# snap-stanford/KGWAS

Hardware: AMD Instinct MI355X
Metric: edges aggregated/sec (full fast-mode KG minibatch training; epoch time in config) (higher is better)
Workload: dtype f32

## Files before the change

include/kgwas_hip.h:

```cpp
#ifndef KGWAS_HIP_H
#define KGWAS_HIP_H

#include <stdint.h>

#ifdef __cplusplus
extern "C" {
#endif

#define KGW_VERSION      125
#define KGW_MAX_TYPES    8
#define KGW_MAX_RELS     64
#define KGW_MAX_LAYERS   4
#define KGW_CHUNK        128
#define KGW_TILE         1024
#define KGW_C            128

#define KGW_F_RAW_WEIGHTS 1
#define KGW_F_DUV_PIECES  4
#define KGW_F_RELU_INPUT  2

#define KGW_OK           0
#define KGW_E_NULL      -1
#define KGW_E_RANGE     -2
#define KGW_E_UNSUPPORTED -3
// ... 186 lines not shown

int64_t kgw_scatter_relu_rows_workspace_floats(int64_t n_rows);
int kgw_scatter_relu_rows(const float* g, const int32_t* g2l, const float* h, int64_t n_rows, float* dz,
                          float* colsum, float* workspace, kgw_stream_t stream);

int kgw_edge_alpha(const KgwLayerArgs* args, float* alpha_out, kgw_stream_t stream);

enum { KGW_GRAD_DIRECT = 0, KGW_GRAD_TN = 1, KGW_GRAD_TN_COLSUM = 2, KGW_GRAD_MLP2_W = 3, KGW_GRAD_MLP2_B = 4, KGW_GRAD_G3T = 5 };
typedef struct KgwGradSrc {
    const float* ws;
    int32_t kind, nblk;
    int32_t M, N, MT, NT, gy, gz;
    int32_t K1, c_transposed;
    void* packed;
    int32_t flip, pad_;
} KgwGradSrc;

int64_t kgw_tn_gemm_workspace_floats(int64_t rows, int32_t M, int32_t N);
typedef struct KgwTnJob {
    const float* A; int64_t lda; const float* B; int64_t ldb;
    int64_t rows;
    float* C; int64_t ldc;
    float* colsum_a; int64_t colsum_ld;
    float* workspace; int64_t workspace_floats;
    const int32_t* rows_dev;
    int32_t M, N, c_transposed, colsum_repeat;
} KgwTnJob;
int kgw_tn_gemm_multi(int32_t n_jobs, const KgwTnJob* jobs, kgw_stream_t stream);
int kgw_tn_gemm(const float* A, int64_t lda, int32_t M, const float* B, int64_t ldb, int32_t N,
                int64_t rows, float* C, int64_t ldc, float* colsum_a, float* workspace,
                int64_t workspace_floats, kgw_stream_t stream);
int kgw_tn_gemm_ex(const float* A, int64_t lda, int32_t M, const float* B, int64_t ldb, int32_t N,
                   int64_t rows, float* C, int64_t ldc, int32_t c_transposed, float* colsum_a,
                   int32_t colsum_repeat, int64_t colsum_ld, float* workspace, int64_t workspace_floats,
                   const int32_t* rows_dev, kgw_stream_t stream);

int kgw_tn_gemm_partial(const float* A, int64_t lda, int32_t M, const float* B, int64_t ldb, int32_t N,
                        int64_t rows, float* C, int64_t ldc, int32_t c_transposed, float* colsum_a,
                        float* workspace, int64_t workspace_floats, const int32_t* rows_dev, KgwGradSrc* src,
                        kgw_stream_t stream);
int kgw_tn_gemm_multi_partial(int32_t n_jobs, const KgwTnJob* jobs, KgwGradSrc* src, kgw_stream_t stream);
int kgw_tn_split(int on);
int64_t kgw_tn_direct_rows(int64_t rows);

typedef struct KgwReadoutFold {
    const float* scratch; const double* terms; float* dw_lin; float* db_lin; double* loss;
    int32_t nb, n;
} KgwReadoutFold;

typedef struct KgwTnReducePlan { int32_t valid; int32_t blocks ; int32_t reserved[2]; int64_t opaque[96]; } KgwTnReducePlan;
int kgw_tn_reduce_launch(const KgwTnReducePlan* plan, kgw_stream_t stream);
int kgw_tn_gemm_partial_ride(const float* A, int64_t lda, int32_t M, const float* B, int64_t ldb, int32_t N, int64_t rows,
                             float* C, int64_t ldc, int32_t c_transposed, float* colsum_a, float* workspace,
                             int64_t workspace_floats, const int32_t* rows_dev, KgwGradSrc* src, const KgwTnReducePlan* ride_in,
                             kgw_stream_t stream);

int kgw_linear(const float* X, int64_t ldx, const float* W, int64_t ldw, const float* bias,
               const float* mask, int64_t ldm, float* Y, int64_t ldy, int64_t rows, int32_t K, int32_t N,
               int32_t relu, int32_t w_is_kn, const int32_t* rows_dev, kgw_stream_t stream);

int kgw_mlp2_fwd(const float* X, int64_t ldx, int32_t K1, const float* W1, int64_t ldw1, const float* b1, const float* W2,
                 int64_t ldw2, const float* b2, float* H1, int64_t ldh1, float* H2, int64_t ldh2, int64_t rows,
                 const int32_t* rows_dev, const int32_t* ids, float* Xg, int64_t ldxg, kgw_stream_t stream);

int kgw_mlp2w_fwd(int32_t n_jobs, const float* const* src, const int32_t* const* ids, const int64_t* n_rows, int64_t ldx,
                  const float* W1, int64_t ldw1, const float* b1, const float* W2, int64_t ldw2, const float* b2, float* Xg,
                  float* H1, float* H2, int64_t ldo, kgw_stream_t stream);

int64_t kgw_mlp2_bwd_first_workspace_floats(int64_t rows);
int kgw_mlp2_bwd_first(const float* dH2, int64_t ldd, const float* W2, int64_t ldw2, const float* H1, int64_t ldh1,
                       const float* X, int64_t ldx, int32_t K1, int64_t rows, const int32_t* rows_dev, float* dW1,
                       int64_t ldw1, float* db1, float* workspace, int64_t workspace_floats, const int32_t* in_ids, float* dZ,
                       int64_t ldz, kgw_stream_t stream);

int kgw_mlp2_bwd_first_partial(const float* dH2, int64_t ldd, const float* W2, int64_t ldw2, const float* H1, int64_t ldh1,
                               const float* X, int64_t ldx, int32_t K1, int64_t rows, const int32_t* rows_dev, float* dW1,
                               int64_t ldw1, float* db1, float* workspace, int64_t workspace_floats, const int32_t* in_ids,
                               float* dZ, int64_t ldz, KgwGradSrc* src, kgw_stream_t stream);
int kgw_mlp2_bwd_first_packed(const float* dH2, int64_t ldd, const float* W2, int64_t ldw2, const float* H1, int64_t ldh1,
                              const float* X, int64_t ldx, int32_t K1, int64_t rows, float* dW1, int64_t ldw1, float* db1,
                              float* workspace, int64_t workspace_floats, const int32_t* in_ids, float* dZ, int64_t ldz,
                              void* packed, int32_t flip, KgwGradSrc* src, kgw_stream_t stream);

int64_t kgw_gemm3_packed_bytes(int64_t K);
int64_t kgw_gemm3_workspace_floats(int64_t M, int64_t K);
int kgw_gemm3_pack(const float* S, int64_t lds, int64_t K, int64_t k_valid, int32_t s_is_kn, void* packed, kgw_stream_t stream);
int kgw_gemm3(const float* A, int64_t lda, int64_t M, int64_t K, const void* packed, float* workspace, int64_t workspace_floats,
              const float* bias, int32_t relu, float* out, int64_t ldo, int32_t transpose_out, const int32_t* row_map,
              float* out_rows, int64_t ld_rows, int64_t out_rows_n, const int32_t* out_rows_real, kgw_stream_t stream);

int64_t kgw_linear_splitk_workspace_floats(int64_t rows, int32_t K, int32_t N);
int kgw_linear_splitk(const float* X, int64_t ldx, const float* W, int64_t ldw, const float* bias, float* Y,
                      int64_t ldy, int64_t rows, int32_t K, int32_t N, int32_t relu, int32_t w_is_kn,
                      float* workspace, int64_t workspace_floats, const int32_t* rows_dev, kgw_stream_t stream);
int kgw_linear_splitk_ind(const float* X, int64_t ldx, const float* W, int64_t ldw, const float* bias, float* Y,
                          int64_t ldy, int64_t rows, int32_t K, int32_t relu, const float* seg_stat, const float* gamma,
                          float* workspace, int64_t workspace_floats, const int32_t* rows_dev, kgw_stream_t stream);
int kgw_ind_colsum(const float* seg_stat, const float* dY, int64_t ldy, int64_t rows, int32_t R, float* dgamma,
                   kgw_stream_t stream);
typedef struct KgwSplitKJob {
    const float* X; int64_t ldx;
    const float* W; int64_t ldw;
    const float* bias;
    float* Y; int64_t ldy;
    int64_t rows;
    const float* seg_stat;
    const float* gamma;
    float* dgamma;
    int32_t K, N, relu, w_is_kn;
} KgwSplitKJob;
int kgw_linear_splitk_multi(int32_t n_jobs, const KgwSplitKJob* jobs, kgw_stream_t stream);
int kgw_ind_colsum_multi(int32_t n_jobs, const KgwSplitKJob* jobs, kgw_stream_t stream);

int kgw_transform_bwd(int32_t n_tn, const KgwTnJob* tn_jobs, int32_t n_sk, const KgwSplitKJob* sk_jobs, int32_t n_cs,
                      const KgwSplitKJob* cs_jobs, kgw_stream_t stream);
int kgw_transform_bwd_ex(int32_t n_tn, const KgwTnJob* tn_jobs, int32_t n_sk, const KgwSplitKJob* sk_jobs, int32_t n_cs,
                         const KgwSplitKJob* cs_jobs, const KgwTnReducePlan* ride_in, KgwTnReducePlan* defer_out,
                         const KgwReadoutFold* fold_in , kgw_stream_t stream);

int kgw_adam(int32_t n_tensors, float* const* params, const float* const* grads, float* const* exp_avg,
             float* const* exp_avg_sq, const int64_t* numel, int32_t* step_dev, float lr, float beta1,
             float beta2, float eps, float weight_decay, kgw_stream_t stream);
int kgw_adam_notick(int32_t n_tensors, float* const* params, const float* const* grads, float* const* exp_avg,
                    float* const* exp_avg_sq, const int64_t* numel, int32_t* step_dev, float lr, float beta1,
                    float beta2, float eps, float weight_decay, kgw_stream_t stream);

int kgw_gemm3_partial(const float* A, int64_t lda, int64_t M, int64_t K, const void* packed, float* workspace,
                      int64_t workspace_floats, float* out, int64_t ldo, KgwGradSrc* src, kgw_stream_t stream);
int kgw_gemm3_flip(void);

enum { KGW_ADAM_FUSED_MAX = 40, KGW_ADAM_FUSED_SRC = 12, KGW_ADAM_FUSED_COUNTERS = 65 * 32 };
int kgw_adam_fused(int32_t n_tensors, float* const* params, float* const* grads, float* const* exp_avg,
                   float* const* exp_avg_sq, const int64_t* numel, const KgwGradSrc* src, int32_t* step_dev, float lr,
                   float beta1, float beta2, float eps, float weight_decay, const KgwBatchMeta* meta_dev, int32_t n_layers,
                   int32_t n_hops, int64_t* stats, int32_t* done_counters, kgw_stream_t stream);

int kgw_grad_finish(int32_t n_tensors, float* const* dst, float* const* grads, const int64_t* numel, const KgwGradSrc* src,
                    kgw_stream_t stream);

int kgw_relvec_fwd(int32_t n_rels_total, const int32_t* live_of_rel, const int32_t* bip_pos, const float* w_src_t,
                   const float* w_dst_t, const float* att_src, const float* att_dst, float* U_full, float* V,
                   int32_t v_by_rel, int32_t n_live, const float* bias, const int32_t* blk_of_live, int32_t n_blk,
                   float* bias_sum, float* zero_buf, int64_t zero_floats, kgw_stream_t stream);
int kgw_relvec_bwd(int32_t n_live, const int32_t* rel_ids, const int32_t* bip_pos, const float* w_src_t,
                   const float* w_dst_t, const float* att_src, const float* att_dst, const float* dU_full,
                   const float* dV, float* dw_src_t, float* dw_dst_t, float* datt_src, float* datt_dst,
                   int32_t v_by_rel, kgw_stream_t stream);
typedef struct KgwRelvecJob {
    int32_t n_rels_total, n_live, n_blk;
    int32_t duv_pieces;
    const int32_t* live_of_rel; const int32_t* rel_ids; const int32_t* bip_pos;
    const float* w_src_t; const float* w_dst_t; const float* att_src; const float* att_dst;
    float* U_full; float* V; const float* bias; const int32_t* blk_of_live; float* bias_sum;
    float* zero_buf; int64_t zero_floats;
    const float* dU_full; const float* dV; const float* dw_src_acc;
    float* dw_src_t; float* dw_dst_t; float* datt_src; float* datt_dst;
} KgwRelvecJob;
int kgw_relvec_fwd_multi(int32_t n_jobs, const KgwRelvecJob* jobs, kgw_stream_t stream);
int kgw_relvec_bwd_multi(int32_t n_jobs, const KgwRelvecJob* jobs, kgw_stream_t stream);
int kgw_relvec_bwd_acc(int32_t n_live, const int32_t* rel_ids, const int32_t* bip_pos, const float* w_src_t,
                       const float* w_dst_t, const float* att_src, const float* att_dst, const float* dU_full,
                       const float* dV, const float* dw_src_acc, float* dw_src_t, float* dw_dst_t, float* datt_src,
                       float* datt_dst, int32_t v_by_rel, kgw_stream_t stream);

typedef struct KgwFoldArgs {
    int32_t n, n_rels, n_mlp;
// ... 55 lines not shown
```

kgwas_amd/_lib.py:

```python
from __future__ import annotations

import ctypes as C
import os

KGW_MAX_TYPES = 8
KGW_MAX_RELS = 64
KGW_MAX_LAYERS = 4
KGW_CHUNK = 128
KGW_TILE = 1024
KGW_C = 128
PART_STRIDE = 132

_HERE = os.path.dirname(os.path.abspath(__file__))
LIB_PATH = os.environ.get('KGW_LIB_PATH') or os.path.join(_HERE, 'csrc', 'libkgwas_hip.so')


class KgwGraph(C.Structure):
    _fields_ = [
        ('n_types', C.c_int32), ('n_rels', C.c_int32), ('n_layers', C.c_int32), ('n_hops', C.c_int32),
        ('n_nodes', C.c_int32 * KGW_MAX_TYPES),
        ('node_base', C.c_int32 * (KGW_MAX_TYPES + 1)),
        ('R_dst', C.c_int32 * KGW_MAX_TYPES),
        ('R_src', C.c_int32 * KGW_MAX_TYPES),
        ('rel_src', C.c_int32 * KGW_MAX_RELS),
# ... 57 lines not shown
    ]


class KgwLayerArgs(C.Structure):
    _fields_ = [
        ('layer', C.c_int32), ('n_chunks', C.c_int32), ('n_multi_hops', C.c_int32), ('n_src_rows', C.c_int32),
        ('neg_slope', C.c_float), ('inv_temp', C.c_float), ('flags', C.c_int32), ('pad_', C.c_int32),
        ('graph_host', C.c_void_p), ('meta_host', C.c_void_p), ('meta_dev', C.c_void_p),
        ('chunks', C.c_void_p), ('multi', C.c_void_p), ('multi_cap', C.c_int64),
        ('col_local', C.c_void_p), ('H', C.c_void_p), ('a_dst', C.c_void_p), ('V', C.c_void_p), ('U', C.c_void_p),
        ('Z', C.c_void_p), ('stat', C.c_void_p), ('e_edge', C.c_void_p), ('part', C.c_void_p),
        ('dZ', C.c_void_p), ('adp', C.c_void_p), ('da_dst', C.c_void_p), ('part_da', C.c_void_p),
        ('t_ptr', C.c_void_p), ('t_edge', C.c_void_p), ('t_zrow', C.c_void_p),
        ('dH', C.c_void_p), ('ev_before', C.c_void_p), ('ev_after', C.c_void_p), ('da_src', C.c_void_p),
        ('logit_bias', C.c_void_p), ('partial_rels', C.c_uint64),
        ('t_rel', C.c_void_p), ('oct_flags', C.c_void_p), ('rel_sums', C.c_void_p),
        ('part_du', C.c_void_p), ('seg_chptr', C.c_void_p), ('duv_ws', C.c_void_p), ('dU', C.c_void_p), ('dV', C.c_void_p),
    ]


class KgwTnJob(C.Structure):
    _fields_ = [('A', C.c_void_p), ('lda', C.c_int64), ('B', C.c_void_p), ('ldb', C.c_int64), ('rows', C.c_int64),
                ('C', C.c_void_p), ('ldc', C.c_int64), ('colsum_a', C.c_void_p), ('colsum_ld', C.c_int64),
                ('workspace', C.c_void_p), ('workspace_floats', C.c_int64), ('rows_dev', C.c_void_p),
                ('M', C.c_int32), ('N', C.c_int32), ('c_transposed', C.c_int32), ('colsum_repeat', C.c_int32)]


class KgwGradSrc(C.Structure):
    _fields_ = [('ws', C.c_void_p), ('kind', C.c_int32), ('nblk', C.c_int32), ('M', C.c_int32), ('N', C.c_int32), ('MT', C.c_int32),
                ('NT', C.c_int32), ('gy', C.c_int32), ('gz', C.c_int32), ('K1', C.c_int32), ('c_transposed', C.c_int32),
                ('packed', C.c_void_p), ('flip', C.c_int32), ('pad_', C.c_int32)]


KGW_SEGCOPY_MAX = 40


class KgwSegCopy(C.Structure):
    _fields_ = [('n', C.c_int32), ('to_slot', C.c_int32), ('ptr', C.c_void_p * KGW_SEGCOPY_MAX), ('units', C.c_int64 * KGW_SEGCOPY_MAX),
                ('slot_off', C.c_int64 * KGW_SEGCOPY_MAX), ('slots', C.c_void_p), ('slot_stride', C.c_int64), ('slot_index', C.c_void_p)]


ADAM_FUSED_MAX, ADAM_FUSED_SRC, ADAM_FUSED_COUNTERS = 40, 12, 65 * 32


class KgwReadoutFold(C.Structure):
    _fields_ = [('scratch', C.c_void_p), ('terms', C.c_void_p), ('dw_lin', C.c_void_p), ('db_lin', C.c_void_p), ('loss', C.c_void_p),
                ('nb', C.c_int32), ('n', C.c_int32)]


class KgwTnReducePlan(C.Structure):
    _fields_ = [('valid', C.c_int32), ('blocks', C.c_int32), ('reserved', C.c_int32 * 2), ('opaque', C.c_int64 * 96)]


class KgwSplitKJob(C.Structure):
    _fields_ = [('X', C.c_void_p), ('ldx', C.c_int64), ('W', C.c_void_p), ('ldw', C.c_int64), ('bias', C.c_void_p),
                ('Y', C.c_void_p), ('ldy', C.c_int64), ('rows', C.c_int64), ('seg_stat', C.c_void_p), ('gamma', C.c_void_p),
                ('dgamma', C.c_void_p), ('K', C.c_int32), ('N', C.c_int32), ('relu', C.c_int32), ('w_is_kn', C.c_int32)]


class KgwRelvecJob(C.Structure):
    _fields_ = [('n_rels_total', C.c_int32), ('n_live', C.c_int32), ('n_blk', C.c_int32), ('duv_pieces', C.c_int32),
                ('live_of_rel', C.c_void_p), ('rel_ids', C.c_void_p), ('bip_pos', C.c_void_p),
                ('w_src_t', C.c_void_p), ('w_dst_t', C.c_void_p), ('att_src', C.c_void_p), ('att_dst', C.c_void_p),
                ('U_full', C.c_void_p), ('V', C.c_void_p), ('bias', C.c_void_p), ('blk_of_live', C.c_void_p), ('bias_sum', C.c_void_p),
                ('zero_buf', C.c_void_p), ('zero_floats', C.c_int64),
                ('dU_full', C.c_void_p), ('dV', C.c_void_p), ('dw_src_acc', C.c_void_p),
                ('dw_src_t', C.c_void_p), ('dw_dst_t', C.c_void_p), ('datt_src', C.c_void_p), ('datt_dst', C.c_void_p)]


class KgwFoldArgs(C.Structure):
    _fields_ = [('n', C.c_int32), ('n_rels', C.c_int32), ('n_mlp', C.c_int32), ('duv_pieces', C.c_int32),
                ('rel_ids_host', C.c_void_p), ('src_mlp_host', C.c_void_p), ('dst_mlp_host', C.c_void_p),
                ('w_src_t', C.c_void_p), ('fc_weight', C.c_void_p * 4), ('fc_bias', C.c_void_p * 4),
                ('U', C.c_void_p), ('V', C.c_void_p),
                ('Up', C.c_void_p), ('Vp', C.c_void_p), ('kappa', C.c_void_p), ('Wp', C.c_void_p), ('gamma', C.c_void_p),
                ('dUp', C.c_void_p), ('dVp', C.c_void_p), ('dkappa', C.c_void_p), ('dWp', C.c_void_p), ('dgamma', C.c_void_p),
                ('dU', C.c_void_p), ('dV', C.c_void_p), ('dws', C.c_void_p),
                ('d_fc_weight', C.c_void_p * 4), ('d_fc_bias', C.c_void_p * 4)]


EXPORTS = ['kgw_version', 'kgw_status_string', 'kgw_struct_sizes', 'kgw_sample_batch', 'kgw_sample_batch_parts', 'kgw_sample_batch_fanout', 'kgw_sampler_scan_ints', 'kgw_segments_copy',
           'kgw_softmax_pack', 'kgw_softmax_merge', 'kgw_scatter_rows', 'kgw_linear_splitk', 'kgw_linear_splitk_workspace_floats', 'kgw_linear_splitk_ind', 'kgw_ind_colsum', 'kgw_linear_splitk_multi', 'kgw_ind_colsum_multi', 'kgw_fold_fwd', 'kgw_fold_bwd', 'kgw_relation_sums',
           'kgw_gat_aggregate_fwd', 'kgw_gat_aggregate_bwd_dst', 'kgw_gat_aggregate_bwd_src',
           'kgw_gather_rows', 'kgw_gather_rows_multi', 'kgw_scatter_relu_rows', 'kgw_scatter_relu_rows_workspace_floats', 'kgw_edge_alpha', 'kgw_debug_reduce', 'kgw_debug_reduce8', 'kgw_tn_gemm', 'kgw_tn_gemm_ex', 'kgw_tn_gemm_multi', 'kgw_tn_gemm_workspace_floats', 'kgw_tn_gemm_partial', 'kgw_tn_gemm_multi_partial', 'kgw_tn_split', 'kgw_tn_direct_rows', 'kgw_param_tail', 'kgw_tn_reduce_launch', 'kgw_tn_gemm_partial_ride', 'kgw_transform_bwd_ex', 'kgw_mlp2_bwd_first_partial', 'kgw_mlp2_bwd_first_packed', 'kgw_adam_fused', 'kgw_gemm3_partial', 'kgw_gemm3_flip', 'kgw_transform_bwd', 'kgw_grad_finish',
           'kgw_linear', 'kgw_mlp2_fwd', 'kgw_mlp2w_fwd', 'kgw_mlp2_bwd_first', 'kgw_mlp2_bwd_first_workspace_floats', 'kgw_gemm3', 'kgw_gemm3_riders', 'kgw_gemm3_rider_blocks', 'kgw_gemm3_pack', 'kgw_gemm3_packed_bytes', 'kgw_gemm3_workspace_floats', 'kgw_adam', 'kgw_adam_notick', 'kgw_relvec_fwd', 'kgw_relvec_bwd', 'kgw_relvec_bwd_acc', 'kgw_relvec_fwd_multi', 'kgw_relvec_bwd_multi', 'kgw_wmse_fwd', 'kgw_wmse_bwd', 'kgw_readout_wmse_fwd', 'kgw_readout_wmse_bwd', 'kgw_readout_wmse_train', 'kgw_readout_wmse_train_parts', 'kgw_readout_train_fold', 'kgw_accumulate_stats', 'kgw_accumulate_stats_tick']

_lib = None


class KgwasHipError(RuntimeError):
    pass


def lib():
    global _lib
    if _lib is not None:
        return _lib
    if not os.path.exists(LIB_PATH):
        raise KgwasHipError(
            f'{LIB_PATH} not found: build it with `python -c "import __graft_entry__ as g; g.build()"` '
            '(hipcc --offload-arch=gfx950).  kgwas_amd has no CPU fallback.')
    L = C.CDLL(LIB_PATH)
    L.kgw_version.restype = C.c_int
    L.kgw_status_string.restype = C.c_char_p
    L.kgw_status_string.argtypes = [C.c_int]
    L.kgw_struct_sizes.argtypes = [C.POINTER(C.c_int64), C.c_int]
    sizes = (C.c_int64 * 7)()
    L.kgw_struct_sizes(sizes, 7)
    mine = [C.sizeof(KgwGraph), C.sizeof(KgwBatchMeta), C.sizeof(KgwChunk), C.sizeof(KgwBatchBuf),
            C.sizeof(KgwLayerArgs), C.sizeof(KgwTnJob), C.sizeof(KgwGradSrc)]
    if list(sizes) != mine:
        raise KgwasHipError(f'ABI struct size mismatch: library {list(sizes)} vs binding {mine}')
    L.kgw_sample_batch.argtypes = [C.POINTER(KgwGraph), C.POINTER(KgwBatchBuf), C.c_void_p, C.c_int32,
                                   C.c_int32, C.c_int32, C.c_void_p]
    L.kgw_sample_batch_parts.argtypes = [C.POINTER(KgwGraph), C.POINTER(KgwBatchBuf), C.c_void_p, C.c_int32,
                                         C.c_int32, C.c_int32, C.c_int32, C.c_int32, C.c_void_p]
    if hasattr(L, 'kgw_sample_batch_fanout'):
        L.kgw_sample_batch_fanout.argtypes = [C.POINTER(KgwGraph), C.POINTER(KgwBatchBuf), C.c_void_p, C.c_int32, C.c_int32,
                                              C.POINTER(C.c_int32), C.c_void_p, C.c_void_p]
    L.kgw_sampler_scan_ints.argtypes = [C.c_int64, C.c_int64, C.c_int64]
    L.kgw_sampler_scan_ints.restype = C.c_int64
    L.kgw_segments_copy.argtypes = [C.POINTER(KgwSegCopy), C.c_int32, C.c_void_p]
    L.kgw_softmax_pack.argtypes = [C.c_void_p, C.c_void_p, C.c_void_p, C.c_int64, C.c_void_p, C.c_void_p]
    L.kgw_softmax_merge.argtypes = [C.c_void_p, C.c_int32, C.c_void_p, C.c_int64, C.c_void_p, C.c_void_p, C.c_void_p]
    L.kgw_scatter_rows.argtypes = [C.c_void_p, C.c_void_p, C.c_int64, C.c_int32, C.c_void_p, C.c_void_p]
    for name in ('kgw_gat_aggregate_fwd', 'kgw_gat_aggregate_bwd_dst', 'kgw_gat_aggregate_bwd_src'):
        getattr(L, name).argtypes = [C.POINTER(KgwLayerArgs), C.c_void_p]
    L.kgw_gather_rows.argtypes = [C.c_void_p, C.c_void_p, C.c_int64, C.c_int32, C.c_void_p, C.c_void_p]
    L.kgw_tn_gemm_multi.argtypes = [C.c_int32, C.POINTER(KgwTnJob), C.c_void_p]
    L.kgw_scatter_relu_rows_workspace_floats.restype = C.c_int64
    L.kgw_scatter_relu_rows_workspace_floats.argtypes = [C.c_int64]
    L.kgw_scatter_relu_rows.argtypes = [C.c_void_p, C.c_void_p, C.c_void_p, C.c_int64, C.c_void_p, C.c_void_p, C.c_void_p, C.c_void_p]
    L.kgw_gather_rows_multi.argtypes = [C.c_int32, C.POINTER(C.c_void_p), C.POINTER(C.c_void_p), C.POINTER(C.c_int64), C.c_int32,
                                        C.POINTER(C.c_void_p), C.c_void_p]
    L.kgw_edge_alpha.argtypes = [C.POINTER(KgwLayerArgs), C.c_void_p, C.c_void_p]
    L.kgw_debug_reduce.argtypes = [C.c_void_p] * 5
    L.kgw_debug_reduce8.argtypes = [C.c_void_p] * 3
    L.kgw_tn_gemm_workspace_floats.restype = C.c_int64
    L.kgw_tn_gemm_workspace_floats.argtypes = [C.c_int64, C.c_int32, C.c_int32]
    L.kgw_linear.argtypes = [C.c_void_p, C.c_int64, C.c_void_p, C.c_int64, C.c_void_p, C.c_void_p, C.c_int64,
                             C.c_void_p, C.c_int64, C.c_int64, C.c_int32, C.c_int32, C.c_int32, C.c_int32, C.c_void_p,
                             C.c_void_p]
    L.kgw_mlp2_fwd.argtypes = [C.c_void_p, C.c_int64, C.c_int32, C.c_void_p, C.c_int64, C.c_void_p, C.c_void_p, C.c_int64, C.c_void_p,
                               C.c_void_p, C.c_int64, C.c_void_p, C.c_int64, C.c_int64, C.c_void_p, C.c_void_p, C.c_void_p, C.c_int64,
                               C.c_void_p]
    L.kgw_mlp2w_fwd.argtypes = [C.c_int32, C.c_void_p, C.c_void_p, C.c_void_p, C.c_int64, C.c_void_p, C.c_int64, C.c_void_p, C.c_void_p,
                                C.c_int64, C.c_void_p, C.c_void_p, C.c_void_p, C.c_void_p, C.c_int64, C.c_void_p]
    L.kgw_gemm3_packed_bytes.restype = C.c_int64
    L.kgw_gemm3_packed_bytes.argtypes = [C.c_int64]
    L.kgw_gemm3_workspace_floats.restype = C.c_int64
    L.kgw_gemm3_workspace_floats.argtypes = [C.c_int64, C.c_int64]
    L.kgw_gemm3_pack.argtypes = [C.c_void_p, C.c_int64, C.c_int64, C.c_int64, C.c_int32, C.c_void_p, C.c_void_p]
    L.kgw_gemm3.argtypes = [C.c_void_p, C.c_int64, C.c_int64, C.c_int64, C.c_void_p, C.c_void_p, C.c_int64, C.c_void_p, C.c_int32,
                            C.c_void_p, C.c_int64, C.c_int32, C.c_void_p, C.c_void_p, C.c_int64, C.c_int64, C.c_void_p, C.c_void_p]
    L.kgw_gemm3_riders.argtypes = L.kgw_gemm3.argtypes[:-1] + [C.c_int32, C.c_void_p, C.c_void_p, C.c_int32, C.c_void_p]
    L.kgw_gemm3_rider_blocks.argtypes = [C.c_int64, C.c_int64]
    L.kgw_mlp2_bwd_first_workspace_floats.restype = C.c_int64
    L.kgw_mlp2_bwd_first_workspace_floats.argtypes = [C.c_int64]
    L.kgw_mlp2_bwd_first.argtypes = [C.c_void_p, C.c_int64, C.c_void_p, C.c_int64, C.c_void_p, C.c_int64, C.c_void_p, C.c_int64, C.c_int32,
                                     C.c_int64, C.c_void_p, C.c_void_p, C.c_int64, C.c_void_p, C.c_void_p, C.c_int64, C.c_void_p, C.c_void_p,
                                     C.c_int64, C.c_void_p]
    L.kgw_linear_splitk_workspace_floats.restype = C.c_int64
    L.kgw_linear_splitk_workspace_floats.argtypes = [C.c_int64, C.c_int32, C.c_int32]
    L.kgw_linear_splitk.argtypes = [C.c_void_p, C.c_int64, C.c_void_p, C.c_int64, C.c_void_p, C.c_void_p, C.c_int64, C.c_int64,
                                    C.c_int32, C.c_int32, C.c_int32, C.c_int32, C.c_void_p, C.c_int64, C.c_void_p, C.c_void_p]
    L.kgw_linear_splitk_ind.argtypes = [C.c_void_p, C.c_int64, C.c_void_p, C.c_int64, C.c_void_p, C.c_void_p, C.c_int64, C.c_int64,
                                        C.c_int32, C.c_int32, C.c_void_p, C.c_void_p, C.c_void_p, C.c_int64, C.c_void_p, C.c_void_p]
    L.kgw_ind_colsum.argtypes = [C.c_void_p, C.c_void_p, C.c_int64, C.c_int64, C.c_int32, C.c_void_p, C.c_void_p]
    L.kgw_linear_splitk_multi.argtypes = [C.c_int32, C.POINTER(KgwSplitKJob), C.c_void_p]
    L.kgw_ind_colsum_multi.argtypes = [C.c_int32, C.POINTER(KgwSplitKJob), C.c_void_p]
    L.kgw_relation_sums.argtypes = [C.POINTER(KgwLayerArgs), C.c_void_p, C.c_void_p, C.c_void_p]
    L.kgw_fold_fwd.argtypes = [C.POINTER(KgwFoldArgs), C.c_void_p]
    L.kgw_fold_bwd.argtypes = [C.POINTER(KgwFoldArgs), C.c_void_p]
    L.kgw_adam.argtypes = [C.c_int32, C.c_void_p, C.c_void_p, C.c_void_p, C.c_void_p, C.c_void_p, C.c_void_p,
                           C.c_float, C.c_float, C.c_float, C.c_float, C.c_float, C.c_void_p]
    L.kgw_adam_notick.argtypes = L.kgw_adam.argtypes
    L.kgw_relvec_fwd.argtypes = [C.c_int32] + [C.c_void_p] * 8 + [C.c_int32, C.c_int32, C.c_void_p, C.c_void_p, C.c_int32,
                                 C.c_void_p, C.c_void_p, C.c_int64, C.c_void_p]
    L.kgw_relvec_fwd_multi.argtypes = [C.c_int32, C.POINTER(KgwRelvecJob), C.c_void_p]
    L.kgw_relvec_bwd_multi.argtypes = [C.c_int32, C.POINTER(KgwRelvecJob), C.c_void_p]
    L.kgw_relvec_bwd.argtypes = [C.c_int32] + [C.c_void_p] * 12 + [C.c_int32, C.c_void_p]
    L.kgw_relvec_bwd_acc.argtypes = [C.c_int32] + [C.c_void_p] * 13 + [C.c_int32, C.c_void_p]
    L.kgw_tn_gemm.argtypes = [C.c_void_p, C.c_int64, C.c_int32, C.c_void_p, C.c_int64, C.c_int32, C.c_int64,
                              C.c_void_p, C.c_int64, C.c_void_p, C.c_void_p, C.c_int64, C.c_void_p]
    L.kgw_tn_gemm_ex.argtypes = [C.c_void_p, C.c_int64, C.c_int32, C.c_void_p, C.c_int64, C.c_int32, C.c_int64,
                                 C.c_void_p, C.c_int64, C.c_int32, C.c_void_p, C.c_int32, C.c_int64, C.c_void_p,
                                 C.c_int64, C.c_void_p, C.c_void_p]
    L.kgw_tn_gemm_partial.argtypes = [C.c_void_p, C.c_int64, C.c_int32, C.c_void_p, C.c_int64, C.c_int32, C.c_int64,
                                      C.c_void_p, C.c_int64, C.c_int32, C.c_void_p, C.c_void_p, C.c_int64, C.c_void_p,
                                      C.POINTER(KgwGradSrc), C.c_void_p]
    L.kgw_tn_gemm_multi_partial.argtypes = [C.c_int32, C.POINTER(KgwTnJob), C.POINTER(KgwGradSrc), C.c_void_p]
    L.kgw_param_tail.argtypes = [C.c_int32, C.c_void_p, C.c_void_p, C.c_void_p, C.c_int32, C.c_void_p, C.c_int32, C.c_void_p]
    L.kgw_mlp2_bwd_first_partial.argtypes = L.kgw_mlp2_bwd_first.argtypes[:-1] + [C.POINTER(KgwGradSrc), C.c_void_p]
    L.kgw_mlp2_bwd_first_packed.argtypes = [C.c_void_p, C.c_int64, C.c_void_p, C.c_int64, C.c_void_p, C.c_int64, C.c_void_p, C.c_int64, C.c_int32,
                                            C.c_int64, C.c_void_p, C.c_int64, C.c_void_p, C.c_void_p, C.c_int64, C.c_void_p, C.c_void_p,
                                            C.c_int64, C.c_void_p, C.c_int32, C.c_void_p, C.c_void_p]
    L.kgw_adam_fused.argtypes = [C.c_int32, C.c_void_p, C.c_void_p, C.c_void_p, C.c_void_p, C.c_void_p, C.POINTER(KgwGradSrc), C.c_void_p,
                                 C.c_float, C.c_float, C.c_float, C.c_float, C.c_float, C.c_void_p, C.c_int32, C.c_int32, C.c_void_p,
                                 C.c_void_p, C.c_void_p]
    L.kgw_gemm3_partial.argtypes = [C.c_void_p, C.c_int64, C.c_int64, C.c_int64, C.c_void_p, C.c_void_p, C.c_int64, C.c_void_p, C.c_int64,
                                    C.POINTER(KgwGradSrc), C.c_void_p]
    L.kgw_gemm3_flip.restype = C.c_int
    L.kgw_grad_finish.argtypes = [C.c_int32, C.c_void_p, C.c_void_p, C.c_void_p, C.POINTER(KgwGradSrc), C.c_void_p]
    L.kgw_transform_bwd.argtypes = [C.c_int32, C.POINTER(KgwTnJob), C.c_int32, C.POINTER(KgwSplitKJob), C.c_int32, C.POINTER(KgwSplitKJob),
                                    C.c_void_p]
    L.kgw_transform_bwd_ex.argtypes = L.kgw_transform_bwd.argtypes[:-1] + [C.c_void_p, C.c_void_p, C.c_void_p, C.c_void_p]
    L.kgw_tn_reduce_launch.argtypes = [C.c_void_p, C.c_void_p]
    L.kgw_tn_direct_rows.restype = C.c_int64
    L.kgw_tn_direct_rows.argtypes = [C.c_int64]
    L.kgw_tn_gemm_partial_ride.argtypes = L.kgw_tn_gemm_partial.argtypes[:-1] + [C.c_void_p, C.c_void_p]
    L.kgw_wmse_fwd.argtypes = [C.c_void_p] * 4 + [C.c_int32, C.c_void_p, C.c_void_p]
    L.kgw_wmse_bwd.argtypes = [C.c_void_p] * 4 + [C.c_int32, C.c_void_p, C.c_void_p, C.c_void_p]
    L.kgw_readout_wmse_fwd.argtypes = [C.c_void_p] * 6 + [C.c_int32, C.c_int32] + [C.c_void_p] * 4
    L.kgw_readout_wmse_bwd.argtypes = [C.c_void_p] * 6 + [C.c_int32, C.c_int64, C.c_int32] + [C.c_void_p] * 6
    L.kgw_readout_wmse_train.argtypes = [C.c_void_p] * 6 + [C.c_int32, C.c_int64, C.c_int32] + [C.c_void_p] * 8
    L.kgw_readout_wmse_train_parts.argtypes = [C.c_void_p] * 6 + [C.c_int32, C.c_int64, C.c_int32] + [C.c_void_p] * 9
    L.kgw_readout_train_fold.argtypes = [C.c_void_p, C.c_void_p]
    L.kgw_accumulate_stats.argtypes = [C.c_void_p, C.c_int32, C.c_int32, C.c_void_p, C.c_void_p]
    L.kgw_accumulate_stats_tick.argtypes = [C.c_void_p, C.c_int32, C.c_int32, C.c_void_p, C.c_void_p, C.c_void_p]
    _lib = L
    return L


KGW_E_UNSUPPORTED = -3


def check(status: int, what: str):
    if status != 0:
        msg = lib().kgw_status_string(int(status))
        raise KgwasHipError(f'{what} failed: status {status} ({msg.decode() if msg else "?"})')


def stream_ptr():
    import torch
    return C.c_void_p(torch.cuda.current_stream().cuda_stream)
```

kgwas_amd/csrc/kgw_dense_linear.h:

```cpp
#pragma once

namespace {

constexpr int LBM = 128, LBN = 128, LBK = 32, LPAD = 33;

struct LinArgs {
    const float* X; int64_t ldx;
    const float* W; int64_t ldw;
    const float* bias;
    const float* mask;
    int64_t ldm;
    float* Y; int64_t ldy;
    int64_t rows; int K, N;
    int relu, w_kn;
    const int32_t* rows_dev;
};

__device__ __forceinline__ int64_t lin_rows_eff(const LinArgs& a) {
    if (!a.rows_dev) return a.rows;
    const int64_t r = *a.rows_dev;
    return r < 0 ? 0 : (r < a.rows ? r : a.rows);
}

__device__ __forceinline__ void lin_zero_padding(const LinArgs& a, int64_t rows_eff, int64_t tid, int64_t nthreads) {
// ... 38 lines not shown
            {
                const int row = idx >> 3, kq = (idx & 7) * 4;
                const int64_t r = r0 + row;
                const bool ok = (r < a.rows) && (k0 + kq < a.K);
                const float* p = a.X + (ok ? r : 0) * a.ldx + (ok ? k0 + kq : 0);
                const float4 v = *(const float4*)p;
                xr[j] = ok ? v : make_float4(0.f, 0.f, 0.f, 0.f);
            }
            if (!a.w_kn) {
                const int n = idx >> 3, kq = (idx & 7) * 4;
                const bool ok = (n0 + n < a.N) && (k0 + kq < a.K);
                const float* p = a.W + (int64_t)(ok ? n0 + n : 0) * a.ldw + (ok ? k0 + kq : 0);
                const float4 v = *(const float4*)p;
                wr[j] = ok ? v : make_float4(0.f, 0.f, 0.f, 0.f);
            } else {
                const int k = idx >> 5, nq = (idx & 31) * 4;
                const bool ok = (k0 + k < a.K) && (n0 + nq < a.N);
                const float* p = a.W + (int64_t)(ok ? k0 + k : 0) * a.ldw + (ok ? n0 + nq : 0);
                const float4 v = *(const float4*)p;
                wr[j] = ok ? v : make_float4(0.f, 0.f, 0.f, 0.f);
            }
        }
    };
    auto stage = [&]() {
#pragma unroll
        for (int j = 0; j < 4; ++j) {
            const int idx = tid + 256 * j;
            {
                const int row = idx >> 3, kq = (idx & 7) * 4;
                float* d = Xs + row * LPAD + kq;
                d[0] = xr[j].x; d[1] = xr[j].y; d[2] = xr[j].z; d[3] = xr[j].w;
            }
            if (!a.w_kn) {
                const int n = idx >> 3, kq = (idx & 7) * 4;
                float* d = Ws + n * LPAD + kq;
                d[0] = wr[j].x; d[1] = wr[j].y; d[2] = wr[j].z; d[3] = wr[j].w;
            } else {
                const int k = idx >> 5, nq = (idx & 31) * 4;
                Ws[(nq + 0) * LPAD + k] = wr[j].x; Ws[(nq + 1) * LPAD + k] = wr[j].y;
                Ws[(nq + 2) * LPAD + k] = wr[j].z; Ws[(nq + 3) * LPAD + k] = wr[j].w;
            }
        }
    };

    fetch(0);
    for (int k0 = 0; k0 < a.K; k0 += LBK) {
        __syncthreads();
        stage();
        __syncthreads();
        if (k0 + LBK < a.K) fetch(k0 + LBK);
        const float* xa = Xs + (wave * 32 + li) * LPAD + lk;
        const float* wb = Ws + li * LPAD + lk;
#pragma unroll
        for (int kp = 0; kp < LBK / 2; ++kp) {
            const float av = xa[2 * kp];
#pragma unroll
            for (int t = 0; t < 4; ++t)
                acc[t] = __builtin_amdgcn_mfma_f32_32x32x2f32(av, wb[t * 32 * LPAD + 2 * kp], acc[t], 0, 0, 0);
        }
    }
#pragma unroll
    for (int t = 0; t < 4; ++t) {
        const int col = n0 + t * 32 + li;
        if (col >= a.N) continue;
        const float bv = a.bias ? a.bias[col] : 0.f;
#pragma unroll
        for (int e = 0; e < 16; ++e) {
            const int64_t r = r0 + wave * 32 + (e & 3) + 8 * (e >> 2) + 4 * lk;
            if (r >= a.rows) continue;
            float v = acc[t][e] + bv;
            if (a.relu) v = fmaxf(v, 0.f);
            if (a.mask) v = (a.mask[r * a.ldm + col] > 0.f) ? v : 0.f;
            a.Y[r * a.ldy + col] = v;
        }
    }
}

}

namespace {

constexpr int WST = 132;

typedef float f32x4 __attribute__((ext_vector_type(4)));

template <int KC, bool WKN, int RT>
__global__ void __launch_bounds__(512) __attribute__((amdgpu_waves_per_eu(2, 2))) k_linear_wres(LinArgs a_) {
    extern __shared__ __attribute__((aligned(16))) float lds[];
    LinArgs a = a_;
    {
        const int64_t re = lin_rows_eff(a_);
        lin_zero_padding(a_, re, (int64_t)blockIdx.x * 512 + threadIdx.x, (int64_t)gridDim.x * 512);
        a.rows = re;
        if ((int64_t)blockIdx.x * RT >= re) return;
    }
    constexpr int XST = KC + 4;
    float* Wl = lds;
    float* Xs = lds + 128 * WST;
    constexpr int WRG = RT / 32, WCG = 8 / WRG, CT = 4 / WCG;
    const int tid = threadIdx.x, lane = tid & 63, wave = tid >> 6;
    const int li = lane & 31, lk = lane >> 5;
    const int nch = (a.K + KC - 1) / KC;
    const int64_t ntiles = (a.rows + RT - 1) / RT;
    constexpr int F4 = RT * KC / 4 / 512;
    f32x4 xr[F4];
#define KGW_FETCH(TILE, CH)                                                                            \
    _Pragma("unroll") for (int j = 0; j < F4; ++j) {                                                   \
        const int idx = tid + 512 * j;                                                                 \
        const int row = idx / (KC / 4), kq = (idx % (KC / 4)) * 4;                                     \
        int64_t r = (TILE) * RT + row;                                                                 \
        if (r >= a.rows) r = a.rows - 1;                      \
        int k = (CH) * KC + kq;                                                                        \
        if (k > a.K - 4) k = a.K - 4;                       \
        xr[j] = *(const f32x4*)(a.X + r * a.ldx + k);                                                   \
    }
    int64_t tile = blockIdx.x;
    if (tile < ntiles) { KGW_FETCH(tile, 0) }
    {
        f32x4 wv[8];
#pragma unroll
        for (int it = 0; it < 8; ++it) {
            const int idx = tid + 512 * it;
            wv[it] = f32x4{0.f, 0.f, 0.f, 0.f};
            if (!WKN) {
                const int n = idx >> 5, k4 = (idx & 31) * 4;
                if (n < a.N && k4 < a.K) wv[it] = *(const f32x4*)(a.W + (int64_t)n * a.ldw + k4);
            } else {
                const int k = idx >> 5, n4 = (idx & 31) * 4;
                if (k < a.K && n4 < a.N) wv[it] = *(const f32x4*)(a.W + (int64_t)k * a.ldw + n4);
            }
        }
#pragma unroll
        for (int it = 0; it < 8; ++it) {
            const int idx = tid + 512 * it;
            if (!WKN) {
                *(f32x4*)(Wl + (idx >> 5) * WST + (idx & 31) * 4) = wv[it];
            } else {
                const int k = idx >> 5, n4 = (idx & 31) * 4;
                Wl[(n4 + 0) * WST + k] = wv[it].x; Wl[(n4 + 1) * WST + k] = wv[it].y;
                Wl[(n4 + 2) * WST + k] = wv[it].z; Wl[(n4 + 3) * WST + k] = wv[it].w;
            }
        }
    }
    const int rg = wave % WRG, cg = wave / WRG;
    const float* wb = Wl + (cg * CT * 32 + li) * WST + lk * (KC / 2);
    float* slice = Xs + rg * 32 * XST;
    const float* xa = slice + li * XST + lk * (KC / 2);
    constexpr int Q = KC / 8;
    const float relu_lo = a.relu ? 0.f : -__builtin_inff();
    for (; tile < ntiles; tile += gridDim.x) {
        f32x16 acc[CT];
#pragma unroll
        for (int t = 0; t < CT; ++t)
#pragma unroll
            for (int e = 0; e < 16; ++e) acc[t][e] = 0.f;
        for (int ch = 0; ch < nch; ++ch) {
            __syncthreads();
#pragma unroll
            for (int j = 0; j < F4; ++j) {
                const int idx = tid + 512 * j;
                *(f32x4*)(Xs + (idx / (KC / 4)) * XST + (idx % (KC / 4)) * 4) = xr[j];
            }
            __syncthreads();
            {
                const bool same = ch + 1 < nch;
                const int64_t nt = same ? tile : tile + gridDim.x;
                const int nc = same ? ch + 1 : 0;
// ... 163 lines not shown
        }
        const int64_t row = (int64_t)tile * 32 + li;
        const bool live = row < a.rows;
        const float* mp = nullptr;
        if (MASK) mp = a.mask + (live ? row : a.rows - 1) * a.ldm + 4 * lk;
        unsigned mb[2] = {0xffffffffu, 0xffffffffu};
        f32x4 mv[2][4];
        f32x4 b3n = *(const f32x4*)w3;
#define KGW_MASK_FETCH(T)                                                                                 \
        _Pragma("unroll") for (int g = 0; g < 4; ++g) mv[(T) & 1][g] = *(const f32x4*)(mp + (T) * 32 + 8 * g);
#define KGW_MASK_BITS(T)                                                                                  \
        _Pragma("unroll") for (int g = 0; g < 4; ++g) {                                                  \
            const int b0 = ((T) & 1) * 16 + 4 * g;                                                        \
            if (!(mv[(T) & 1][g].x > 0.f)) mb[(T) >> 1] &= ~(1u << (b0 + 0));                             \
            if (!(mv[(T) & 1][g].y > 0.f)) mb[(T) >> 1] &= ~(1u << (b0 + 1));                             \
            if (!(mv[(T) & 1][g].z > 0.f)) mb[(T) >> 1] &= ~(1u << (b0 + 2));                             \
            if (!(mv[(T) & 1][g].w > 0.f)) mb[(T) >> 1] &= ~(1u << (b0 + 3));                             \
        }
#pragma unroll
        for (int q = 0; q < 16; ++q) {
            if (MASK) {
                if (q == 0) { KGW_MASK_FETCH(0) }
                if (q == 1) { KGW_MASK_FETCH(1) }
                if (q == 5) { KGW_MASK_BITS(0) }
                if (q == 6) { KGW_MASK_BITS(1) KGW_MASK_FETCH(2) }
                if (q == 7) { KGW_MASK_FETCH(3) }
                if (q == 11) { KGW_MASK_BITS(2) }
                if (q == 12) { KGW_MASK_BITS(3) }
            }
            const f32x4 b3 = b3n;
            if (q + 1 < 16) b3n = *(const f32x4*)(w3 + 4 * (q + 1));
#define KGW_WREG_STEP(C)                                                                                  \
            _Pragma("unroll") for (int t = 0; t < 3; ++t)                                                \
                acc[t] = __builtin_amdgcn_mfma_f32_32x32x2f32(bw[t][q].C, xa[q].C, acc[t], 0, 0, 0);      \
            acc[3] = __builtin_amdgcn_mfma_f32_32x32x2f32(b3.C, xa[q].C, acc[3], 0, 0, 0);
            KGW_WREG_STEP(x) KGW_WREG_STEP(y) KGW_WREG_STEP(z) KGW_WREG_STEP(w)
#undef KGW_WREG_STEP
            if (q == 7) {
                __builtin_amdgcn_sched_barrier(0);
#pragma unroll
                for (int qq = 0; qq < 8; ++qq) xa[qq] = *(const f32x4*)(xn + 4 * qq);
                __builtin_amdgcn_sched_barrier(0);
            }
        }
#undef KGW_MASK_FETCH
#undef KGW_MASK_BITS
        if (live) {
            float* yp = a.Y + row * a.ldy + 4 * lk;
#pragma unroll
            for (int t = 0; t < 4; ++t) {
#pragma unroll
                for (int g = 0; g < 4; ++g) {
                    const f32x4 b4 = *(const f32x4*)(bl + t * 32 + 8 * g);
                    f32x4 v;
                    v.x = acc[t][4 * g + 0] + b4.x; v.y = acc[t][4 * g + 1] + b4.y;
                    v.z = acc[t][4 * g + 2] + b4.z; v.w = acc[t][4 * g + 3] + b4.w;
                    v.x = fmaxf(v.x, lo); v.y = fmaxf(v.y, lo); v.z = fmaxf(v.z, lo); v.w = fmaxf(v.w, lo);
                    if (MASK) {
                        const unsigned m4 = mb[t >> 1] >> (((t & 1) << 4) + 4 * g);
                        v.x = (m4 & 1u) ? v.x : 0.f; v.y = (m4 & 2u) ? v.y : 0.f;
                        v.z = (m4 & 4u) ? v.z : 0.f; v.w = (m4 & 8u) ? v.w : 0.f;
                    }
                    *(f32x4*)(yp + t * 32 + 8 * g) = v;
                }
            }
        }
        __builtin_amdgcn_sched_barrier(0);
#pragma unroll
        for (int qq = 8; qq < 16; ++qq) xa[qq] = *(const f32x4*)(xn + 4 * qq);
        __builtin_amdgcn_sched_barrier(0);
    }
}

struct Mlp2Args {
    const float* X; int64_t ldx;
    const float* W1; int64_t ldw1; const float* b1;
    const float* W2; int64_t ldw2; const float* b2;
    float* H1; int64_t ldh1;
    float* H2; int64_t ldh2;
    int64_t rows; int K1;
    const int32_t* rows_dev;
    const int32_t* ids;
    float* Xg; int64_t ldxg;
};

__global__ void __launch_bounds__(256) __attribute__((amdgpu_waves_per_eu(1, 1))) k_mlp2_fwd(Mlp2Args a) {
    extern __shared__ __attribute__((aligned(16))) float lds[];
    float* Wl = lds;
    float* W1l = lds + 128 * WST + 128;
    const int tid = threadIdx.x, lane = tid & 63, wave = tid >> 6;
    const int li = lane & 31, lk = lane >> 5;
    int64_t rows = a.rows;
    if (a.rows_dev) { const int64_t r = *a.rows_dev; rows = r < 0 ? 0 : (r < a.rows ? r : a.rows); }
    {
        const int64_t npad = a.rows - rows;
        for (int64_t q = (int64_t)blockIdx.x * 256 + tid; q < npad * 32; q += (int64_t)gridDim.x * 256) {
            const int64_t r = rows + q / 32; const int c4 = (int)(q % 32) * 4;
            *(float4*)(a.H2 + r * a.ldh2 + c4) = make_float4(0.f, 0.f, 0.f, 0.f);
            if (a.H1) *(float4*)(a.H1 + r * a.ldh1 + c4) = make_float4(0.f, 0.f, 0.f, 0.f);
        }
        if ((int64_t)blockIdx.x * 4 * 32 >= rows) return;
    }
    const int ntiles = (int)((rows + 31) / 32);
    const int nw = (int)gridDim.x * 4;
    int tile = (int)blockIdx.x * 4 + wave;
    const int K1 = a.K1;
    auto fetch_x = [&](int t, f32x4 (&x)[3]) {
        int64_t r = (int64_t)(t < ntiles ? t : ntiles - 1) * 32 + li;
        if (r >= rows) r = rows - 1;
        const float* xp = a.X + (a.ids ? (int64_t)a.ids[r] : r) * a.ldx;
#pragma unroll
        for (int c = 0; c < 3; ++c) {
            const int k4 = 12 * lk + 4 * c;
            if (k4 + 4 <= K1) x[c] = *(const f32x4*)(xp + k4);
            else x[c] = f32x4{k4 == K1 ? 1.f : 0.f, 0.f, 0.f, 0.f};
        }
    };
    f32x4 xn[3];
    fetch_x(tile, xn);
    {
        f32x4 wv[16];
#pragma unroll
        for (int it = 0; it < 16; ++it) {
            const int idx = tid + 256 * it;
            wv[it] = *(const f32x4*)(a.W2 + (int64_t)(idx >> 5) * a.ldw2 + (idx & 31) * 4);
        }
#pragma unroll
        for (int it = 0; it < 16; ++it) {
            const int idx = tid + 256 * it;
            *(f32x4*)(Wl + (idx >> 5) * WST + (idx & 31) * 4) = wv[it];
        }
        for (int idx = tid; idx < 128 * 24; idx += 256) {
            const int n = idx / 24, k = idx % 24;
            W1l[idx] = k < K1 ? a.W1[(int64_t)n * a.ldw1 + k] : (k == K1 ? (a.b1 ? a.b1[n] : 0.f) : 0.f);
        }
    }
    if (tid < 128) Wl[128 * WST + tid] = a.b2 ? a.b2[tid] : 0.f;
    __syncthreads();
    f32x4 bw[3][16];
#pragma unroll
    for (int t = 0; t < 3; ++t)
#pragma unroll
        for (int q = 0; q < 16; ++q) bw[t][q] = *(const f32x4*)(Wl + (t * 32 + li) * WST + 32 * (q >> 2) + 8 * (q & 3) + 4 * lk);
    const float* w3 = Wl + (96 + li) * WST + 4 * lk;
    f32x4 w1[4][3];
#pragma unroll
    for (int t = 0; t < 4; ++t)
#pragma unroll
        for (int c = 0; c < 3; ++c) w1[t][c] = *(const f32x4*)(W1l + (t * 32 + li) * 24 + 12 * lk + 4 * c);
    const float* bl = Wl + 128 * WST + 4 * lk;
    for (; tile < ntiles; tile += nw) {
        f32x4 x[3] = {xn[0], xn[1], xn[2]};
        fetch_x(tile + nw, xn);
        f32x16 acc[4];
#pragma unroll
        for (int t = 0; t < 4; ++t)
#pragma unroll
            for (int e = 0; e < 16; ++e) acc[t][e] = 0.f;
#pragma unroll
        for (int c = 0; c < 3; ++c) {
#define KGW_MLP_STEP(C)                                                                                   \
            _Pragma("unroll") for (int t = 0; t < 4; ++t)                                                \
                acc[t] = __builtin_amdgcn_mfma_f32_32x32x2f32(w1[t][c].C, x[c].C, acc[t], 0, 0, 0);
            KGW_MLP_STEP(x) KGW_MLP_STEP(y) KGW_MLP_STEP(z) KGW_MLP_STEP(w)
#undef KGW_MLP_STEP
        }
        const int64_t row = (int64_t)tile * 32 + li;
        const bool live = row < rows;
        if (a.Xg && live) {
#pragma unroll
            for (int c = 0; c < 3; ++c)
                if (12 * lk + 4 * c + 4 <= K1) *(f32x4*)(a.Xg + row * a.ldxg + 12 * lk + 4 * c) = x[c];
        }
        f32x4 xa[16];
#pragma unroll
        for (int t = 0; t < 4; ++t)
#pragma unroll
            for (int g = 0; g < 4; ++g) {
                f32x4 v;
                v.x = fmaxf(acc[t][4 * g + 0], 0.f); v.y = fmaxf(acc[t][4 * g + 1], 0.f);
                v.z = fmaxf(acc[t][4 * g + 2], 0.f); v.w = fmaxf(acc[t][4 * g + 3], 0.f);
                xa[4 * t + g] = v;
            }
        if (a.H1 && live) {
            float* hp = a.H1 + row * a.ldh1 + 4 * lk;
#pragma unroll
            for (int q = 0; q < 16; ++q) *(f32x4*)(hp + 32 * (q >> 2) + 8 * (q & 3)) = xa[q];
        }
#pragma unroll
        for (int t = 0; t < 4; ++t)
#pragma unroll
            for (int e = 0; e < 16; ++e) acc[t][e] = 0.f;
        f32x4 b3n = *(const f32x4*)w3;
#pragma unroll
        for (int q = 0; q < 16; ++q) {
            const f32x4 b3 = b3n;
            if (q + 1 < 16) b3n = *(const f32x4*)(w3 + 32 * ((q + 1) >> 2) + 8 * ((q + 1) & 3));
#define KGW_MLP_STEP(C)                                                                                   \
            _Pragma("unroll") for (int t = 0; t < 3; ++t)                                                \
                acc[t] = __builtin_amdgcn_mfma_f32_32x32x2f32(bw[t][q].C, xa[q].C, acc[t], 0, 0, 0);      \
            acc[3] = __builtin_amdgcn_mfma_f32_32x32x2f32(b3.C, xa[q].C, acc[3], 0, 0, 0);
            KGW_MLP_STEP(x) KGW_MLP_STEP(y) KGW_MLP_STEP(z) KGW_MLP_STEP(w)
#undef KGW_MLP_STEP
        }
        if (live) {
            float* yp = a.H2 + row * a.ldh2 + 4 * lk;
#pragma unroll
            for (int t = 0; t < 4; ++t) {
#pragma unroll
                for (int g = 0; g < 4; ++g) {
                    const f32x4 b4 = *(const f32x4*)(bl + t * 32 + 8 * g);
                    f32x4 v;
                    v.x = fmaxf(acc[t][4 * g + 0] + b4.x, 0.f); v.y = fmaxf(acc[t][4 * g + 1] + b4.y, 0.f);
                    v.z = fmaxf(acc[t][4 * g + 2] + b4.z, 0.f); v.w = fmaxf(acc[t][4 * g + 3] + b4.w, 0.f);
                    *(f32x4*)(yp + t * 32 + 8 * g) = v;
                }
            }
        }
    }
}

static constexpr int M3_W2_U4 = 8 * 3 * 4 * 64;

__global__ void __launch_bounds__(512, 1) k_mlp2_fwd3(Mlp2Args a) {
    extern __shared__ __attribute__((aligned(16))) float lds[];
    uint4* W2p = (uint4*)lds;
    float* W1l = lds + M3_W2_U4 * 4;
    float* bl = W1l + 128 * 24;
    const int tid = threadIdx.x, lane = tid & 63, wave = tid >> 6;
    const int li = lane & 31, lk = lane >> 5;
    int64_t rows = a.rows;
    if (a.rows_dev) { const int64_t r = *a.rows_dev; rows = r < 0 ? 0 : (r < a.rows ? r : a.rows); }
    {
        const int64_t npad = a.rows - rows;
        for (int64_t q = (int64_t)blockIdx.x * 512 + tid; q < npad * 32; q += (int64_t)gridDim.x * 512) {
            const int64_t r = rows + q / 32; const int c4 = (int)(q % 32) * 4;
            *(float4*)(a.H2 + r * a.ldh2 + c4) = make_float4(0.f, 0.f, 0.f, 0.f);
            if (a.H1) *(float4*)(a.H1 + r * a.ldh1 + c4) = make_float4(0.f, 0.f, 0.f, 0.f);
        }
        if ((int64_t)blockIdx.x * 8 * 32 >= rows) return;
    }
    const int ntiles = (int)((rows + 31) / 32);
    const int nw = (int)gridDim.x * 8;
    int tile = (int)blockIdx.x * 8 + wave;
    const int K1 = a.K1;
    auto fetch_x = [&](int t, f32x4 (&x)[3]) {
        int64_t r = (int64_t)(t < ntiles ? t : ntiles - 1) * 32 + li;
        if (r >= rows) r = rows - 1;
        const float* xp = a.X + (a.ids ? (int64_t)a.ids[r] : r) * a.ldx;
#pragma unroll
        for (int c = 0; c < 3; ++c) {
            const int k4 = 12 * lk + 4 * c;
            if (k4 + 4 <= K1) x[c] = *(const f32x4*)(xp + k4);
            else x[c] = f32x4{k4 == K1 ? 1.f : 0.f, 0.f, 0.f, 0.f};
        }
    };
    f32x4 xn[3];
    fetch_x(tile, xn);
    for (int idx = tid; idx < 8 * 4 * 64; idx += 512) {
        const int ln = idx & 63, ot = (idx >> 6) & 3, s_ = idx >> 8;
        const float* wp = a.W2 + (int64_t)(32 * ot + (ln & 31)) * a.ldw2 + 32 * (s_ >> 1) + 16 * (s_ & 1) + 4 * (ln >> 5);
        const f32x4 u = *(const f32x4*)wp, v = *(const f32x4*)(wp + 8);
        const float x[8] = {u.x, u.y, u.z, u.w, v.x, v.y, v.z, v.w};
        uint4 p1, p2, p3;
        kgw_split3x8(x, p1, p2, p3);
        uint4* o = W2p + ((s_ * 3) * 4 + ot) * 64 + ln;
        o[0] = p1; o[4 * 64] = p2; o[8 * 64] = p3;
    }
    for (int idx = tid; idx < 128 * 24; idx += 512) {
        const int n = idx / 24, k = idx % 24;
        W1l[idx] = k < K1 ? a.W1[(int64_t)n * a.ldw1 + k] : (k == K1 ? (a.b1 ? a.b1[n] : 0.f) : 0.f);
    }
    if (tid < 128) bl[tid] = a.b2 ? a.b2[tid] : 0.f;
    __syncthreads();
    const float* w1p = W1l + li * 24 + 12 * lk;
    const uint4* w2p = W2p + lane;
    const float* blp = bl + 4 * lk;
    for (; tile < ntiles; tile += nw) {
        f32x4 x[3] = {xn[0], xn[1], xn[2]};
        fetch_x(tile + nw, xn);
        f32x16 acc[4];
#pragma unroll
        for (int t = 0; t < 4; ++t)
#pragma unroll
            for (int e = 0; e < 16; ++e) acc[t][e] = 0.f;
#pragma unroll
        for (int c = 0; c < 3; ++c) {
            f32x4 w[4];
#pragma unroll
            for (int t = 0; t < 4; ++t) w[t] = *(const f32x4*)(w1p + t * 32 * 24 + 4 * c);
#define KGW_MLP_STEP(C)                                                                                   \
            _Pragma("unroll") for (int t = 0; t < 4; ++t)                                                \
                acc[t] = __builtin_amdgcn_mfma_f32_32x32x2f32(w[t].C, x[c].C, acc[t], 0, 0, 0);
            KGW_MLP_STEP(x) KGW_MLP_STEP(y) KGW_MLP_STEP(z) KGW_MLP_STEP(w)
#undef KGW_MLP_STEP
        }
        const int64_t row = (int64_t)tile * 32 + li;
        const bool live = row < rows;
        if (a.Xg && live) {
#pragma unroll
            for (int c = 0; c < 3; ++c)
                if (12 * lk + 4 * c + 4 <= K1) *(f32x4*)(a.Xg + row * a.ldxg + 12 * lk + 4 * c) = x[c];
        }
        f32x4 xa[16];
#pragma unroll
        for (int t = 0; t < 4; ++t)
#pragma unroll
            for (int g = 0; g < 4; ++g) {
                f32x4 v;
                v.x = fmaxf(acc[t][4 * g + 0], 0.f); v.y = fmaxf(acc[t][4 * g + 1], 0.f);
                v.z = fmaxf(acc[t][4 * g + 2], 0.f); v.w = fmaxf(acc[t][4 * g + 3], 0.f);
                xa[4 * t + g] = v;
            }
        if (a.H1 && live) {
            float* hp = a.H1 + row * a.ldh1 + 4 * lk;
#pragma unroll
            for (int q = 0; q < 16; ++q) *(f32x4*)(hp + 32 * (q >> 2) + 8 * (q & 3)) = xa[q];
        }
#pragma unroll
        for (int t = 0; t < 4; ++t)
#pragma unroll
            for (int e = 0; e < 16; ++e) acc[t][e] = 0.f;
#pragma unroll
        for (int s_ = 0; s_ < 8; ++s_) {
            const f32x4 u = xa[2 * s_], v = xa[2 * s_ + 1];
            const float h[8] = {u.x, u.y, u.z, u.w, v.x, v.y, v.z, v.w};
            uint4 p1, p2, p3;
            kgw_split3x8(h, p1, p2, p3);
            const kgw_bf8 hb[3] = {__builtin_bit_cast(kgw_bf8, p1), __builtin_bit_cast(kgw_bf8, p2), __builtin_bit_cast(kgw_bf8, p3)};
            kgw_bf8 wa[3][4];
#pragma unroll
            for (int p = 0; p < 3; ++p)
#pragma unroll
                for (int ot = 0; ot < 4; ++ot) wa[p][ot] = __builtin_bit_cast(kgw_bf8, w2p[((s_ * 3 + p) * 4 + ot) * 64]);
            constexpr int TW[6] = {0, 2, 1, 0, 1, 0}, TH[6] = {2, 0, 1, 1, 0, 0};
#pragma unroll
            for (int t6 = 0; t6 < 6; ++t6)
#pragma unroll
                for (int ot = 0; ot < 4; ++ot)
                    acc[ot] = __builtin_amdgcn_mfma_f32_32x32x16_bf16(wa[TW[t6]][ot], hb[TH[t6]], acc[ot], 0, 0, 0);
        }
        if (live) {
            float* yp = a.H2 + row * a.ldh2 + 4 * lk;
#pragma unroll
            for (int t = 0; t < 4; ++t) {
#pragma unroll
                for (int g = 0; g < 4; ++g) {
                    const f32x4 b4 = *(const f32x4*)(blp + t * 32 + 8 * g);
                    f32x4 v;
                    v.x = fmaxf(acc[t][4 * g + 0] + b4.x, 0.f); v.y = fmaxf(acc[t][4 * g + 1] + b4.y, 0.f);
                    v.z = fmaxf(acc[t][4 * g + 2] + b4.z, 0.f); v.w = fmaxf(acc[t][4 * g + 3] + b4.w, 0.f);
                    *(f32x4*)(yp + t * 32 + 8 * g) = v;
                }
            }
        }
    }
}

struct Mlp2wArgs {
    const float* src[4]; const int32_t* ids[4]; int64_t row0[5];
    int n_jobs; int64_t ldx;
    const float* W1; int64_t ldw1; const float* b1;
    const float* W2; int64_t ldw2; const float* b2;
    float* Xg; float* H1; float* H2; int64_t ldo;
    int64_t rows;
};

__global__ void __launch_bounds__(256) __attribute__((amdgpu_waves_per_eu(1, 1))) k_mlp2w_fwd(Mlp2wArgs a) {
    extern __shared__ __attribute__((aligned(16))) float lds[];
    float* W1l = lds;
    float* W2l = lds + 128 * WST;
    float* bl = lds + 2 * 128 * WST;
    const int tid = threadIdx.x, lane = tid & 63, wave = tid >> 6;
    const int li = lane & 31, lk = lane >> 5;
    const int64_t tile = (int64_t)blockIdx.x * 2 + (wave >> 1);
    const int half = wave & 1, t0 = half * 2;
    const int64_t row = tile * 32 + li;
    const bool live = row < a.rows;
    const int64_t rc = live ? row : a.rows - 1;
    f32x4 xa[16];
    {
        int j = 0;
        while (j + 1 < a.n_jobs && rc >= a.row0[j + 1]) ++j;
        const float* xp = a.src[j] + (int64_t)a.ids[j][rc - a.row0[j]] * a.ldx + lk * 64;
#pragma unroll
        for (int q = 0; q < 16; ++q) xa[q] = *(const f32x4*)(xp + 4 * q);
    }
    {
        f32x4 wv[16];
#pragma unroll
        for (int it = 0; it < 16; ++it) {
            const int idx = tid + 256 * it;
            wv[it] = *(const f32x4*)(a.W1 + (int64_t)(idx >> 5) * a.ldw1 + (idx & 31) * 4);
        }
#pragma unroll
        for (int it = 0; it < 16; ++it) {
            const int idx = tid + 256 * it;
            *(f32x4*)(W1l + (idx >> 5) * WST + (idx & 31) * 4) = wv[it];
        }
#pragma unroll
        for (int it = 0; it < 16; ++it) {
// ... 38 lines not shown
#undef KGW_MLPW_STEP
    }
    f32x4 xh[8];
#pragma unroll
    for (int t = 0; t < 2; ++t)
#pragma unroll
        for (int g = 0; g < 4; ++g) {
            const f32x4 b4 = *(const f32x4*)(bl + (t0 + t) * 32 + 8 * g + 4 * lk);
            f32x4 v;
            v.x = fmaxf(acc[t][4 * g + 0] + b4.x, 0.f); v.y = fmaxf(acc[t][4 * g + 1] + b4.y, 0.f);
            v.z = fmaxf(acc[t][4 * g + 2] + b4.z, 0.f); v.w = fmaxf(acc[t][4 * g + 3] + b4.w, 0.f);
            xh[4 * t + g] = v;
        }
    if (live) {
        float* hp = a.H1 + row * a.ldo + 4 * lk;
#pragma unroll
        for (int q = 0; q < 8; ++q) *(f32x4*)(hp + 32 * (t0 + (q >> 2)) + 8 * (q & 3)) = xh[q];
    }
    __syncthreads();
    {
        f32x4* ex = (f32x4*)W1l;
#pragma unroll
        for (int q = 0; q < 8; ++q) ex[(wave * 8 + q) * 64 + lane] = xh[q];
    }
    __syncthreads();
    {
        const f32x4* ex = (const f32x4*)W1l + ((wave ^ 1) * 8) * 64 + lane;
#pragma unroll
        for (int q = 0; q < 8; ++q) {
            const f32x4 pq = ex[q * 64];
            xa[q] = half ? pq : xh[q];
            xa[8 + q] = half ? xh[q] : pq;
        }
    }
    f32x16 ac2[2];
#pragma unroll
    for (int t = 0; t < 2; ++t)
#pragma unroll
        for (int e = 0; e < 16; ++e) ac2[t][e] = 0.f;
    const float* w2p = W2l + (t0 * 32 + li) * WST + 4 * lk;
    f32x4 vn[2];
#pragma unroll
    for (int t = 0; t < 2; ++t) vn[t] = *(const f32x4*)(w2p + t * 32 * WST);
#pragma unroll
    for (int q = 0; q < 16; ++q) {
        f32x4 w[2];
#pragma unroll
        for (int t = 0; t < 2; ++t) w[t] = vn[t];
        if (q + 1 < 16) {
#pragma unroll
            for (int t = 0; t < 2; ++t) vn[t] = *(const f32x4*)(w2p + t * 32 * WST + 32 * ((q + 1) >> 2) + 8 * ((q + 1) & 3));
        }
#define KGW_MLPW_STEP(C)                                                                                  \
        _Pragma("unroll") for (int t = 0; t < 2; ++t)                                                    \
            ac2[t] = __builtin_amdgcn_mfma_f32_32x32x2f32(w[t].C, xa[q].C, ac2[t], 0, 0, 0);
        KGW_MLPW_STEP(x) KGW_MLPW_STEP(y) KGW_MLPW_STEP(z) KGW_MLPW_STEP(w)
#undef KGW_MLPW_STEP
    }
    if (live) {
        float* yp = a.H2 + row * a.ldo + 4 * lk;
#pragma unroll
        for (int t = 0; t < 2; ++t)
#pragma unroll
            for (int g = 0; g < 4; ++g) {
                const f32x4 b4 = *(const f32x4*)(bl + 128 + (t0 + t) * 32 + 8 * g + 4 * lk);
                f32x4 v;
                v.x = fmaxf(ac2[t][4 * g + 0] + b4.x, 0.f); v.y = fmaxf(ac2[t][4 * g + 1] + b4.y, 0.f);
                v.z = fmaxf(ac2[t][4 * g + 2] + b4.z, 0.f); v.w = fmaxf(ac2[t][4 * g + 3] + b4.w, 0.f);
                *(f32x4*)(yp + (t0 + t) * 32 + 8 * g) = v;
            }
    }
}

struct Mlp2BwdArgs {
    const float* dH2; int64_t ldd;
    const float* W2; int64_t ldw;
    const float* H1; int64_t ldm;
    const float* X; int64_t ldx;
    float* part;
    int64_t rows; int K1;
    const int32_t* rows_dev;
    const int32_t* in_ids;
    float* dZ; int64_t ldz;
    uint4* packed; int flip;
};

constexpr int TST = 132;

__global__ void __launch_bounds__(256) __attribute__((amdgpu_waves_per_eu(1, 1))) k_mlp2_bwd_first(Mlp2BwdArgs a) {
    extern __shared__ __attribute__((aligned(16))) float lds[];
    float* Wl = lds;
    float* Tl = lds + 128 * WST;
    const int tid = threadIdx.x, lane = tid & 63, wave = tid >> 6;
    const int li = lane & 31, lk = lane >> 5;
    int64_t rows = a.rows;
    if (a.rows_dev) { const int64_t r = *a.rows_dev; rows = r < 0 ? 0 : (r < a.rows ? r : a.rows); }
    const int ntiles = (int)((rows + 31) / 32);
    const int nw = (int)gridDim.x * 4;
    float* Tw = Tl + wave * 32 * TST;
    {
        f32x4 wv[16];
#pragma unroll
        for (int it = 0; it < 16; ++it) {
            const int idx = tid + 256 * it;
            wv[it] = *(const f32x4*)(a.W2 + (int64_t)(idx & 127) * a.ldw + (idx >> 7) * 4);
        }
#pragma unroll
        for (int it = 0; it < 16; ++it) {
            const int idx = tid + 256 * it;
            const int k = idx & 127, n4 = (idx >> 7) * 4;
            Wl[(n4 + 0) * WST + k] = wv[it].x; Wl[(n4 + 1) * WST + k] = wv[it].y;
            Wl[(n4 + 2) * WST + k] = wv[it].z; Wl[(n4 + 3) * WST + k] = wv[it].w;
        }
    }
    __syncthreads();
    f32x4 bw[2][16];
#pragma unroll
    for (int t = 0; t < 2; ++t)
#pragma unroll
        for (int q = 0; q < 16; ++q) bw[t][q] = *(const f32x4*)(Wl + (t * 32 + li) * WST + lk * 64 + 4 * q);
    const float* w2 = Wl + (64 + li) * WST + lk * 64;
    const float* w3 = Wl + (96 + li) * WST + lk * 64;
    f32x16 accw[4];
#pragma unroll
    for (int t = 0; t < 4; ++t)
#pragma unroll
        for (int e = 0; e < 16; ++e) accw[t][e] = 0.f;
    const int K1 = a.K1;
    int tile = (int)blockIdx.x * 4 + wave;
    f32x4 xa[16];
    int src_cur;
    {
        int64_t r = (int64_t)(tile < ntiles ? tile : ntiles - 1) * 32 + li;
        if (r >= rows) r = rows - 1;
        src_cur = a.in_ids ? a.in_ids[r] : 0;
        const float* xp = a.dH2 + (a.in_ids ? (int64_t)(src_cur < 0 ? 0 : src_cur) : r) * a.ldd + lk * 64;
#pragma unroll
        for (int q = 0; q < 16; ++q) xa[q] = *(const f32x4*)(xp + 4 * q);
    }
    for (; tile < ntiles; tile += nw) {
        const int64_t r0 = (int64_t)tile * 32;
        const int64_t row = r0 + li;
        const bool live = row < rows && src_cur >= 0;
        const int64_t rc = row < rows ? row : rows - 1;
        const float* xn;
        {
            int nt = tile + nw;
            if (nt >= ntiles) nt = ntiles - 1;
            int64_t r = (int64_t)nt * 32 + li;
            if (r >= rows) r = rows - 1;
            src_cur = a.in_ids ? a.in_ids[r] : 0;
            xn = a.dH2 + (a.in_ids ? (int64_t)(src_cur < 0 ? 0 : src_cur) : r) * a.ldd + lk * 64;
        }
        float xs[16];
#pragma unroll
        for (int s2 = 0; s2 < 16; ++s2) {
            const int64_t rr = r0 + 2 * s2 + lk;
            float v = 0.f;
            if (rr < rows) v = li < K1 ? a.X[rr * a.ldx + li] : (li == K1 ? 1.f : 0.f);
            xs[s2] = v;
        }
        const float* mp = a.H1 + rc * a.ldm + 4 * lk;
        unsigned mb[2] = {0u, 0u};
        f32x4 mv[4];
#define KGW_MLPB_MFETCH(T)                                                                                \
        _Pragma("unroll") for (int g = 0; g < 4; ++g) mv[g] = *(const f32x4*)(mp + (T) * 32 + 8 * g);
#define KGW_MLPB_MBITS(T)                                                                                 \
        _Pragma("unroll") for (int g = 0; g < 4; ++g) {                                                  \
            const int b0 = ((T) & 1) * 16 + 4 * g;                                                        \
            mb[(T) >> 1] |= (mv[g].x > 0.f ? 1u : 0u) << (b0 + 0);                                        \
            mb[(T) >> 1] |= (mv[g].y > 0.f ? 1u : 0u) << (b0 + 1);                                        \
            mb[(T) >> 1] |= (mv[g].z > 0.f ? 1u : 0u) << (b0 + 2);                                        \
            mb[(T) >> 1] |= (mv[g].w > 0.f ? 1u : 0u) << (b0 + 3);                                        \
        }
        f32x16 acc[4];
#pragma unroll
        for (int t = 0; t < 4; ++t)
#pragma unroll
            for (int e = 0; e < 16; ++e) acc[t][e] = 0.f;
        f32x4 b2n = *(const f32x4*)w2, b3n = *(const f32x4*)w3;
#pragma unroll
        for (int q = 0; q < 16; ++q) {
            if (q == 0) { KGW_MLPB_MFETCH(0) }
            if (q == 3) { KGW_MLPB_MBITS(0) KGW_MLPB_MFETCH(1) }
            if (q == 6) { KGW_MLPB_MBITS(1) KGW_MLPB_MFETCH(2) }
            if (q == 10) { KGW_MLPB_MBITS(2) KGW_MLPB_MFETCH(3) }
            if (q == 14) { KGW_MLPB_MBITS(3) }
            const f32x4 b2 = b2n, b3 = b3n;
            if (q + 1 < 16) { b2n = *(const f32x4*)(w2 + 4 * (q + 1)); b3n = *(const f32x4*)(w3 + 4 * (q + 1)); }
#define KGW_MLPB_STEP(C)                                                                                  \
            acc[0] = __builtin_amdgcn_mfma_f32_32x32x2f32(bw[0][q].C, xa[q].C, acc[0], 0, 0, 0);          \
            acc[1] = __builtin_amdgcn_mfma_f32_32x32x2f32(bw[1][q].C, xa[q].C, acc[1], 0, 0, 0);          \
            acc[2] = __builtin_amdgcn_mfma_f32_32x32x2f32(b2.C, xa[q].C, acc[2], 0, 0, 0);                \
            acc[3] = __builtin_amdgcn_mfma_f32_32x32x2f32(b3.C, xa[q].C, acc[3], 0, 0, 0);
            KGW_MLPB_STEP(x) KGW_MLPB_STEP(y) KGW_MLPB_STEP(z) KGW_MLPB_STEP(w)
#undef KGW_MLPB_STEP
            if (q == 7) {
                __builtin_amdgcn_sched_barrier(0);
#pragma unroll
                for (int qq = 0; qq < 8; ++qq) xa[qq] = *(const f32x4*)(xn + 4 * qq);
                __builtin_amdgcn_sched_barrier(0);
            }
        }
#undef KGW_MLPB_MFETCH
#undef KGW_MLPB_MBITS
        if (!live) { mb[0] = 0u; mb[1] = 0u; }
        __builtin_amdgcn_sched_barrier(0);
#pragma unroll
        for (int qq = 8; qq < 16; ++qq) xa[qq] = *(const f32x4*)(xn + 4 * qq);
        __builtin_amdgcn_sched_barrier(0);
#pragma unroll
        for (int t = 0; t < 4; ++t)
#pragma unroll
            for (int g = 0; g < 4; ++g) {
                const unsigned m4 = mb[t >> 1] >> (((t & 1) << 4) + 4 * g);
                f32x4 v;
                v.x = (m4 & 1u) ? acc[t][4 * g + 0] : 0.f; v.y = (m4 & 2u) ? acc[t][4 * g + 1] : 0.f;
                v.z = (m4 & 4u) ? acc[t][4 * g + 2] : 0.f; v.w = (m4 & 8u) ? acc[t][4 * g + 3] : 0.f;
                *(f32x4*)(Tw + li * TST + t * 32 + 8 * g + 4 * lk) = v;
                if (a.dZ && row < rows) *(f32x4*)(a.dZ + row * a.ldz + t * 32 + 8 * g + 4 * lk) = v;
            }
        __asm__ volatile("s_waitcnt lgkmcnt(0)" ::: "memory");
#pragma unroll
        for (int s2 = 0; s2 < 16; ++s2) {
            const float* tp = Tw + (2 * s2 + lk) * TST + li;
#pragma unroll
            for (int t = 0; t < 4; ++t)
                accw[t] = __builtin_amdgcn_mfma_f32_32x32x2f32(xs[s2], tp[t * 32], accw[t], 0, 0, 0);
        }
        __asm__ volatile("s_waitcnt lgkmcnt(0)" ::: "memory");
    }
    __syncthreads();
    float* R = Tl;
#pragma unroll
    for (int t = 0; t < 4; ++t)
#pragma unroll
        for (int e = 0; e < 16; ++e) R[wave * 4096 + (t * 16 + e) * 64 + lane] = accw[t][e];
    __syncthreads();
    for (int f = tid; f < 4096; f += 256)
        a.part[(int64_t)blockIdx.x * 4096 + f] = (R[f] + R[4096 + f]) + (R[2 * 4096 + f] + R[3 * 4096 + f]);
}

constexpr int TS2 = 68;

template <bool PACK>
__global__ void __launch_bounds__(256) __attribute__((amdgpu_waves_per_eu(1, 1))) k_mlp2_bwd_first3(Mlp2BwdArgs a) {
    extern __shared__ __attribute__((aligned(16))) float lds[];
    uint4* W2p = (uint4*)lds;
    float* Tl = lds + M3_W2_U4 * 4;
    const int tid = threadIdx.x, lane = tid & 63, wave = tid >> 6;
    const int li = lane & 31, lk = lane >> 5;
    const unsigned sgn = (li & 1) ? 0x80000000u : 0u;
    int64_t rows = a.rows;
    if (a.rows_dev) { const int64_t r = *a.rows_dev; rows = r < 0 ? 0 : (r < a.rows ? r : a.rows); }
    const int ntiles = (int)((rows + 31) / 32);
    const int nw = (int)gridDim.x * 4;
    float* Tw = Tl + wave * 32 * TS2;
    for (int idx = tid; idx < 8 * 4 * 64; idx += 256) {
        const int ln = idx & 63, jt = (idx >> 6) & 3, s_ = idx >> 8;
        const float* wp = a.W2 + (int64_t)(64 * (ln >> 5) + 8 * s_) * a.ldw + 32 * jt + (ln & 31);
        float x[8];
#pragma unroll
        for (int i = 0; i < 8; ++i) x[i] = wp[(int64_t)i * a.ldw];
        uint4 p1, p2, p3;
        kgw_split3x8(x, p1, p2, p3);
        uint4* o = W2p + ((s_ * 3) * 4 + jt) * 64 + ln;
        o[0] = p1; o[4 * 64] = p2; o[8 * 64] = p3;
    }
    __syncthreads();
    const uint4* w2p = W2p + lane;
    f32x16 accw[4];
#pragma unroll
    for (int t = 0; t < 4; ++t)
#pragma unroll
        for (int e = 0; e < 16; ++e) accw[t][e] = 0.f;
    const int K1 = a.K1;
    int tile = (int)blockIdx.x * 4 + wave;
    f32x4 xa[16];
    int src_cur;
    {
        int64_t r = (int64_t)(tile < ntiles ? tile : ntiles - 1) * 32 + li;
        if (r >= rows) r = rows - 1;
        src_cur = a.in_ids ? a.in_ids[r] : 0;
        const float* xp = a.dH2 + (a.in_ids ? (int64_t)(src_cur < 0 ? 0 : src_cur) : r) * a.ldd + lk * 64;
#pragma unroll
        for (int q = 0; q < 16; ++q) xa[q] = *(const f32x4*)(xp + 4 * q);
    }
#define KGW_MLPB_BITS(MV, MB)                                                                            \
    _Pragma("unroll") for (int t_ = 0; t_ < 4; ++t_) _Pragma("unroll") for (int g = 0; g < 4; ++g) {    \
        const int b0 = (t_ & 1) * 16 + 4 * g;                                                            \
        MB[t_ >> 1] |= (MV[t_][g].x > 0.f ? 1u : 0u) << (b0 + 0);                                        \
        MB[t_ >> 1] |= (MV[t_][g].y > 0.f ? 1u : 0u) << (b0 + 1);                                        \
        MB[t_ >> 1] |= (MV[t_][g].z > 0.f ? 1u : 0u) << (b0 + 2);                                        \
        MB[t_ >> 1] |= (MV[t_][g].w > 0.f ? 1u : 0u) << (b0 + 3);                                        \
    }
    unsigned mb[2] = {0u, 0u};
    {
        int64_t r = (int64_t)(tile < ntiles ? tile : ntiles - 1) * 32 + li;
        if (r >= rows) r = rows - 1;
        const float* mp = a.H1 + r * a.ldm + 4 * lk;
        f32x4 mv[4][4];
#pragma unroll
        for (int t_ = 0; t_ < 4; ++t_)
#pragma unroll
            for (int g = 0; g < 4; ++g) mv[t_][g] = *(const f32x4*)(mp + t_ * 32 + 8 * g);
        KGW_MLPB_BITS(mv, mb)
    }
    for (; tile < ntiles; tile += nw) {
        const int64_t r0 = (int64_t)tile * 32;
        const int64_t row = r0 + li;
        const bool live = row < rows && src_cur >= 0;
        const int64_t rc = row < rows ? row : rows - 1;
        const float* xn;
        {
            int nt = tile + nw;
            if (nt >= ntiles) nt = ntiles - 1;
            int64_t r = (int64_t)nt * 32 + li;
            if (r >= rows) r = rows - 1;
            src_cur = a.in_ids ? a.in_ids[r] : 0;
            xn = a.dH2 + (a.in_ids ? (int64_t)(src_cur < 0 ? 0 : src_cur) : r) * a.ldd + lk * 64;
        }
        float xs[16];
#pragma unroll
        for (int s2 = 0; s2 < 16; ++s2) {
            const int64_t rr = r0 + 2 * s2 + lk;
            float v = 0.f;
            if (rr < rows) v = li < K1 ? a.X[rr * a.ldx + li] : (li == K1 ? 1.f : 0.f);
            xs[s2] = v;
        }
        f32x4 mvn[4][4];
        {
            int nt = tile + nw;
            if (nt >= ntiles) nt = ntiles - 1;
            int64_t r = (int64_t)nt * 32 + li;
            if (r >= rows) r = rows - 1;
            const float* mpn = a.H1 + r * a.ldm + 4 * lk;
#pragma unroll
            for (int t_ = 0; t_ < 4; ++t_)
#pragma unroll
                for (int g = 0; g < 4; ++g) mvn[t_][g] = *(const f32x4*)(mpn + t_ * 32 + 8 * g);
        }
        f32x16 acc[4];
#pragma unroll
        for (int t = 0; t < 4; ++t)
#pragma unroll
            for (int e = 0; e < 16; ++e) acc[t][e] = 0.f;
#pragma unroll
        for (int s_ = 0; s_ < 8; ++s_) {
            const f32x4 u = xa[2 * s_], v = xa[2 * s_ + 1];
            const float h[8] = {kgw_fxor(u.x, sgn), kgw_fxor(u.y, sgn), kgw_fxor(u.z, sgn), kgw_fxor(u.w, sgn),
                                kgw_fxor(v.x, sgn), kgw_fxor(v.y, sgn), kgw_fxor(v.z, sgn), kgw_fxor(v.w, sgn)};
            uint4 p1, p2, p3;
            kgw_split3x8(h, p1, p2, p3);
            const kgw_bf8 hb[3] = {__builtin_bit_cast(kgw_bf8, p1), __builtin_bit_cast(kgw_bf8, p2), __builtin_bit_cast(kgw_bf8, p3)};
            kgw_bf8 wa[3][4];
#pragma unroll
            for (int p = 0; p < 3; ++p)
#pragma unroll
                for (int jt = 0; jt < 4; ++jt) wa[p][jt] = __builtin_bit_cast(kgw_bf8, w2p[((s_ * 3 + p) * 4 + jt) * 64]);
            constexpr int TW[6] = {0, 2, 1, 0, 1, 0}, TH[6] = {2, 0, 1, 1, 0, 0};
#pragma unroll
            for (int t6 = 0; t6 < 6; ++t6)
#pragma unroll
                for (int jt = 0; jt < 4; ++jt)
                    acc[jt] = __builtin_amdgcn_mfma_f32_32x32x16_bf16(wa[TW[t6]][jt], hb[TH[t6]], acc[jt], 0, 0, 0);
            if (s_ == 3) {
                __builtin_amdgcn_sched_barrier(0);
#pragma unroll
                for (int qq = 0; qq < 8; ++qq) xa[qq] = *(const f32x4*)(xn + 4 * qq);
                __builtin_amdgcn_sched_barrier(0);
            }
        }
        if (!live) { mb[0] = 0u; mb[1] = 0u; }
        __builtin_amdgcn_sched_barrier(0);
#pragma unroll
        for (int qq = 8; qq < 16; ++qq) xa[qq] = *(const f32x4*)(xn + 4 * qq);
        __builtin_amdgcn_sched_barrier(0);
#pragma unroll
        for (int hh = 0; hh < 2; ++hh) {
#pragma unroll
            for (int t = 2 * hh; t < 2 * hh + 2; ++t)
#pragma unroll
                for (int g = 0; g < 4; ++g) {
                    const unsigned m4 = mb[t >> 1] >> (((t & 1) << 4) + 4 * g);
                    f32x4 v;
                    v.x = (m4 & 1u) ? kgw_fxor(acc[t][4 * g + 0], sgn) : 0.f; v.y = (m4 & 2u) ? kgw_fxor(acc[t][4 * g + 1], sgn) : 0.f;
                    v.z = (m4 & 4u) ? kgw_fxor(acc[t][4 * g + 2], sgn) : 0.f; v.w = (m4 & 8u) ? kgw_fxor(acc[t][4 * g + 3], sgn) : 0.f;
                    *(f32x4*)(Tw + li * TS2 + (t - 2 * hh) * 32 + 8 * g + 4 * lk) = v;
                    if (a.dZ && row < rows) *(f32x4*)(a.dZ + row * a.ldz + t * 32 + 8 * g + 4 * lk) = v;
                }
            __asm__ volatile("s_waitcnt lgkmcnt(0)" ::: "memory");
            if (PACK) {
                const bool neg = a.flip && ((tile / a.flip) & 1);
#pragma unroll
                for (int it = 0; it < 4; ++it) {
                    const int ntl = it & 1, j = it >> 1;
                    const float* tp = Tw + (16 * j + 8 * lk) * TS2 + 32 * ntl + li;
                    float x[8];
#pragma unroll
                    for (int i = 0; i < 8; ++i) x[i] = neg ? -tp[i * TS2] : tp[i * TS2];
                    uint4 p1, p2, p3;
                    kgw_split3x8(x, p1, p2, p3);
                    uint4* o = a.packed + (((int64_t)tile * 2 + j) * 3 * 4 + (2 * hh + ntl)) * 64 + lane;
                    o[0] = p1; o[4 * 64] = p2; o[8 * 64] = p3;
                }
            }
#pragma unroll
            for (int s2 = 0; s2 < 16; ++s2) {
                const float* tp = Tw + (2 * s2 + lk) * TS2 + li;
#pragma unroll
                for (int t = 0; t < 2; ++t)
                    accw[2 * hh + t] = __builtin_amdgcn_mfma_f32_32x32x2f32(xs[s2], tp[t * 32], accw[2 * hh + t], 0, 0, 0);
            }
            __asm__ volatile("s_waitcnt lgkmcnt(0)" ::: "memory");
        }
        mb[0] = 0u; mb[1] = 0u;
        KGW_MLPB_BITS(mvn, mb)
    }
#undef KGW_MLPB_BITS
    __syncthreads();
    float* R = lds;
#pragma unroll
    for (int t = 0; t < 4; ++t)
#pragma unroll
        for (int e = 0; e < 16; ++e) R[wave * 4096 + (t * 16 + e) * 64 + lane] = accw[t][e];
    __syncthreads();
    for (int f = tid; f < 4096; f += 256)
        a.part[(int64_t)blockIdx.x * 4096 + f] = (R[f] + R[4096 + f]) + (R[2 * 4096 + f] + R[3 * 4096 + f]);
}

__global__ void __launch_bounds__(1024) k_mlp2_bwd_fold(const float* __restrict__ part, int nblk, int K1, float* __restrict__ dW1,
                                                        int64_t ldw, float* __restrict__ db1) {
    __shared__ float sm[1024];
    const int fl = threadIdx.x & 63, g = threadIdx.x >> 6;
    const int f = blockIdx.x * 64 + fl;
    float s4[4] = {0.f, 0.f, 0.f, 0.f};
    int q = 0;
    for (int b = g; b < nblk; b += 16, ++q) s4[q & 3] += part[(int64_t)b * 4096 + f];
    sm[threadIdx.x] = (s4[0] + s4[1]) + (s4[2] + s4[3]);
    __syncthreads();
    if (g == 0) {
        float sv = 0.f;
#pragma unroll
        for (int k = 0; k < 16; k += 4) sv += (sm[k * 64 + fl] + sm[(k + 1) * 64 + fl]) + (sm[(k + 2) * 64 + fl] + sm[(k + 3) * 64 + fl]);
        const int lane = f & 63, e = (f >> 6) & 15, t = f >> 10;
        const int k = (e & 3) + 8 * (e >> 2) + 4 * (lane >> 5), col = 32 * t + (lane & 31);
        if (k < K1) dW1[(int64_t)col * ldw + k] = sv;
        else if (k == K1) db1[col] = sv;
    }
}

template <bool WKN, bool MASK>
__global__ void __launch_bounds__(256) __attribute__((amdgpu_waves_per_eu(2, 2))) k_linear_wreg_half(LinArgs a_) {
    extern __shared__ __attribute__((aligned(16))) float lds[];
    LinArgs a = a_;
    {
        const int64_t re = lin_rows_eff(a_);
        lin_zero_padding(a_, re, (int64_t)blockIdx.x * 256 + threadIdx.x, (int64_t)gridDim.x * 256);
        a.rows = re;
        if ((int64_t)blockIdx.x * 2 * 32 >= re) return;
    }
    float* Wl = lds;
    const int tid = threadIdx.x, lane = tid & 63, wave = tid >> 6;
    const int li = lane & 31, lk = lane >> 5;
    const int64_t tile = (int64_t)blockIdx.x * 2 + (wave >> 1);
    const int t0 = (wave & 1) * 2;
    const int64_t row = tile * 32 + li;
    const bool live = row < a.rows;
    const int64_t rc = live ? row : a.rows - 1;
    f32x4 xa[16];
    {
        const float* xp = a.X + rc * a.ldx + lk * 64;
#pragma unroll
        for (int q = 0; q < 16; ++q) xa[q] = *(const f32x4*)(xp + 4 * q);
    }
    f32x4 mv[2][4];
    if (MASK) {
        const float* mp = a.mask + rc * a.ldm + 4 * lk;
#pragma unroll
        for (int t = 0; t < 2; ++t)
#pragma unroll
            for (int g = 0; g < 4; ++g) mv[t][g] = *(const f32x4*)(mp + (t0 + t) * 32 + 8 * g);
    }
    {
        f32x4 wv[16];
#pragma unroll
        for (int it = 0; it < 16; ++it) {
            const int idx = tid + 256 * it;
            if (!WKN) wv[it] = *(const f32x4*)(a.W + (int64_t)(idx >> 5) * a.ldw + (idx & 31) * 4);
            else wv[it] = *(const f32x4*)(a.W + (int64_t)(idx & 127) * a.ldw + (idx >> 7) * 4);
        }
#pragma unroll
        for (int it = 0; it < 16; ++it) {
            const int idx = tid + 256 * it;
            if (!WKN) {
                *(f32x4*)(Wl + (idx >> 5) * WST + (idx & 31) * 4) = wv[it];
            } else {
                const int k = idx & 127, n4 = (idx >> 7) * 4;
                Wl[(n4 + 0) * WST + k] = wv[it].x; Wl[(n4 + 1) * WST + k] = wv[it].y;
                Wl[(n4 + 2) * WST + k] = wv[it].z; Wl[(n4 + 3) * WST + k] = wv[it].w;
// ... 42 lines not shown
                *(f32x4*)(yp + (t0 + t) * 32 + 8 * g) = v;
            }
        }
    }
}

template <bool WKN>
int launch_wreg(const LinArgs& a, hipStream_t st) {
    const size_t lds = (size_t)(128 * WST + 128) * sizeof(float);
    static KgwPerDevice attr_once;
    if (attr_once.need()) {
        KGW_HIP(hipFuncSetAttribute((const void*)k_linear_wreg<WKN, false>, hipFuncAttributeMaxDynamicSharedMemorySize, (int)lds));
        KGW_HIP(hipFuncSetAttribute((const void*)k_linear_wreg<WKN, true>, hipFuncAttributeMaxDynamicSharedMemorySize, (int)lds));
    }
    const int64_t ntiles = (a.rows + 31) / 32;
    const int64_t half_max = 1024;
    if (ntiles <= half_max) {
        static KgwPerDevice attr_half;
        if (attr_half.need()) {
            KGW_HIP(hipFuncSetAttribute((const void*)k_linear_wreg_half<WKN, false>, hipFuncAttributeMaxDynamicSharedMemorySize, (int)lds));
            KGW_HIP(hipFuncSetAttribute((const void*)k_linear_wreg_half<WKN, true>, hipFuncAttributeMaxDynamicSharedMemorySize, (int)lds));
        }
        const int grid = (int)((ntiles + 1) / 2);
        if (a.mask) k_linear_wreg_half<WKN, true><<<grid, 256, lds, st>>>(a);
        else k_linear_wreg_half<WKN, false><<<grid, 256, lds, st>>>(a);
        KGW_LAUNCH_CHECK();
        return KGW_OK;
    }
    const int64_t nblk = (ntiles + 3) / 4;
    const int grid = (int)(nblk < 256 ? nblk : 256);
    if (a.mask) k_linear_wreg<WKN, true><<<grid, 256, lds, st>>>(a);
    else k_linear_wreg<WKN, false><<<grid, 256, lds, st>>>(a);
    KGW_LAUNCH_CHECK();
    return KGW_OK;
}

template <int KC, bool WKN, int RT>
int launch_wres(const LinArgs& a, hipStream_t st) {
    const size_t lds = (size_t)(128 * WST + RT * (KC + 4)) * sizeof(float);
    auto kern = k_linear_wres<KC, WKN, RT>;
    static KgwPerDevice attr_once;
    if (attr_once.need()) {
        KGW_HIP(hipFuncSetAttribute((const void*)kern, hipFuncAttributeMaxDynamicSharedMemorySize, (int)lds));
    }
    int64_t ntiles = (a.rows + RT - 1) / RT;
    int grid = (int)(ntiles < 256 ? ntiles : 256);
    kern<<<grid, 512, lds, st>>>(a);
    KGW_LAUNCH_CHECK();
    return KGW_OK;
}

}

extern "C" int kgw_linear(const float* X, int64_t ldx, const float* W, int64_t ldw, const float* bias,
                          const float* mask, int64_t ldm, float* Y, int64_t ldy, int64_t rows, int32_t K,
                          int32_t N, int32_t relu, int32_t w_is_kn, const int32_t* rows_dev, kgw_stream_t stream_) {
    if (rows == 0) return KGW_OK;
    if (!X || !W || !Y) return KGW_E_NULL;
    if (rows < 0 || K <= 0 || N <= 0) return KGW_E_RANGE;
    if ((K & 3) || (ldx & 3) || (ldw & 3) || !aligned16(X) || !aligned16(W)) return KGW_E_UNSUPPORTED;
    if (w_is_kn && (N & 3)) return KGW_E_UNSUPPORTED;
    LinArgs a{X, ldx, W, ldw, bias, mask, ldm, Y, ldy, rows, K, N, relu, w_is_kn, rows_dev};
    const int64_t wres_min = 4096;
    const int64_t wres_tall = 32768;
    if (K <= 128 && N <= 128 && rows >= wres_min && (N & 3) == 0 && (ldy & 3) == 0 && aligned16(Y) && aligned16(bias) &&
        (!mask || ((ldm & 3) == 0 && aligned16(mask)))) {
        hipStream_t st = (hipStream_t)stream_;
        const int64_t wreg_min = 4096;
        if (K == 128 && N == 128 && rows >= wreg_min)
            return w_is_kn ? launch_wreg<true>(a, st) : launch_wreg<false>(a, st);
        if (rows >= wres_tall) {
            if (w_is_kn) return K <= 32 ? launch_wres<32, true, 256>(a, st) : launch_wres<64, true, 256>(a, st);
            return K <= 32 ? launch_wres<32, false, 256>(a, st) : launch_wres<64, false, 256>(a, st);
        }
        if (w_is_kn) return K <= 32 ? launch_wres<32, true, 64>(a, st) : launch_wres<64, true, 64>(a, st);
        return K <= 32 ? launch_wres<32, false, 64>(a, st) : launch_wres<64, false, 64>(a, st);
    }
    dim3 grid((unsigned)((rows + LBM - 1) / LBM), (unsigned)((N + LBN - 1) / LBN));
    k_linear<<<grid, 256, 0, (hipStream_t)stream_>>>(a);
    KGW_LAUNCH_CHECK();
    return KGW_OK;
}

extern "C" int kgw_mlp2_fwd(const float* X, int64_t ldx, int32_t K1, const float* W1, int64_t ldw1, const float* b1,
                            const float* W2, int64_t ldw2, const float* b2, float* H1, int64_t ldh1, float* H2, int64_t ldh2,
                            int64_t rows, const int32_t* rows_dev, const int32_t* ids, float* Xg, int64_t ldxg,
                            kgw_stream_t stream_) {
    if (rows == 0) return KGW_OK;
    if (!X || !W1 || !W2 || !H2) return KGW_E_NULL;
    if (Xg && ((ldxg & 3) || !aligned16(Xg))) return KGW_E_UNSUPPORTED;
    if (rows < 0 || K1 <= 0) return KGW_E_RANGE;
    if (K1 > 20 || (K1 & 3) || (ldx & 3) || (ldw2 & 3) || (ldh2 & 3) || (H1 && (ldh1 & 3)) || !aligned16(X) || !aligned16(W2) ||
        !aligned16(H2) || (H1 && !aligned16(H1)))
        return KGW_E_UNSUPPORTED;
    Mlp2Args a{X, ldx, W1, ldw1, b1, W2, ldw2, b2, H1, ldh1, H2, ldh2, rows, K1, rows_dev, ids, Xg, ldxg};
    const size_t lds = (size_t)(128 * WST + 128 + 128 * 24) * sizeof(float);
    static KgwPerDevice attr_once;
    if (attr_once.need()) {
        KGW_HIP(hipFuncSetAttribute((const void*)k_mlp2_fwd, hipFuncAttributeMaxDynamicSharedMemorySize, (int)lds));
    }
    static const bool split3 = !(getenv("KGW_MLP2_SPLIT") && getenv("KGW_MLP2_SPLIT")[0] == '0');
    if (split3) {
        const size_t lds3 = (size_t)M3_W2_U4 * 16 + (size_t)(128 * 24 + 128) * sizeof(float);
        static KgwPerDevice attr3_set;
        if (attr3_set.need()) {
            KGW_HIP(hipFuncSetAttribute((const void*)k_mlp2_fwd3, hipFuncAttributeMaxDynamicSharedMemorySize, (int)lds3));
        }
        const int64_t nblk3 = ((rows + 31) / 32 + 7) / 8;
        k_mlp2_fwd3<<<(int)(nblk3 < 256 ? nblk3 : 256), 512, lds3, (hipStream_t)stream_>>>(a);
        KGW_LAUNCH_CHECK();
        return KGW_OK;
    }
    const int64_t nblk = ((rows + 31) / 32 + 3) / 4;
    k_mlp2_fwd<<<(int)(nblk < 256 ? nblk : 256), 256, lds, (hipStream_t)stream_>>>(a);
    KGW_LAUNCH_CHECK();
    return KGW_OK;
}

extern "C" int kgw_mlp2w_fwd(int32_t n_jobs, const float* const* src, const int32_t* const* ids, const int64_t* n_rows,
                             int64_t ldx, const float* W1, int64_t ldw1, const float* b1, const float* W2, int64_t ldw2,
                             const float* b2, float* Xg, float* H1, float* H2, int64_t ldo, kgw_stream_t stream_) {
    if (n_jobs <= 0) return KGW_OK;
    if (n_jobs > 4) return KGW_E_RANGE;
    if (!src || !ids || !n_rows || !W1 || !W2 || !Xg || !H1 || !H2) return KGW_E_NULL;
    if ((ldx & 3) || (ldw1 & 3) || (ldw2 & 3) || (ldo & 3) || !aligned16(W1) || !aligned16(W2) || !aligned16(Xg) || !aligned16(H1) ||
        !aligned16(H2))
        return KGW_E_UNSUPPORTED;
    Mlp2wArgs a{};
    a.n_jobs = n_jobs; a.ldx = ldx;
    a.row0[0] = 0;
    for (int j = 0; j < n_jobs; ++j) {
        if (!src[j] || !ids[j] || n_rows[j] < 0) return KGW_E_NULL;
        if (!aligned16(src[j])) return KGW_E_UNSUPPORTED;
        a.src[j] = src[j]; a.ids[j] = ids[j]; a.row0[j + 1] = a.row0[j] + n_rows[j];
    }
    a.rows = a.row0[n_jobs];
    if (a.rows == 0) return KGW_OK;
    a.W1 = W1; a.ldw1 = ldw1; a.b1 = b1; a.W2 = W2; a.ldw2 = ldw2; a.b2 = b2;
    a.Xg = Xg; a.H1 = H1; a.H2 = H2; a.ldo = ldo;
    const size_t lds = (size_t)(2 * 128 * WST + 256) * sizeof(float);
    static KgwPerDevice attr_once;
    if (attr_once.need()) {
        KGW_HIP(hipFuncSetAttribute((const void*)k_mlp2w_fwd, hipFuncAttributeMaxDynamicSharedMemorySize, (int)lds));
    }
    const int64_t ntiles = (a.rows + 31) / 32;
    k_mlp2w_fwd<<<(unsigned)((ntiles + 1) / 2), 256, lds, (hipStream_t)stream_>>>(a);
    KGW_LAUNCH_CHECK();
    return KGW_OK;
}

extern "C" int64_t kgw_mlp2_bwd_first_workspace_floats(int64_t rows) {
    int64_t nblk = ((rows + 31) / 32 + 3) / 4;
    if (nblk > 256) nblk = 256;
    if (nblk < 1) nblk = 1;
    return nblk * 4096;
}

static int mlp2_bwd_first(const float* dH2, int64_t ldd, const float* W2, int64_t ldw2, const float* H1, int64_t ldh1,
                          const float* X, int64_t ldx, int32_t K1, int64_t rows, const int32_t* rows_dev, float* dW1,
                          int64_t ldw1, float* db1, float* workspace, int64_t workspace_floats, const int32_t* in_ids,
                          float* dZ, int64_t ldz, kgw_stream_t stream_, KgwGradSrc* defer, void* packed = nullptr, int flip = 0) {
    if (!dH2 || !W2 || !H1 || !db1 || !workspace) return KGW_E_NULL;
    if (defer && K1 > 0 && ldw1 != K1) return KGW_E_UNSUPPORTED;
    if (rows <= 0 || K1 < 0) return KGW_E_RANGE;
    if (K1 > 0 && (!X || !dW1)) return KGW_E_NULL;
    if (dZ && ((ldz & 3) || !aligned16(dZ))) return KGW_E_UNSUPPORTED;
    if (K1 > 31 || (ldd & 3) || (ldw2 & 3) || (ldh1 & 3) || !aligned16(dH2) || !aligned16(W2) || !aligned16(H1)) return KGW_E_UNSUPPORTED;
    int64_t nblk = ((rows + 31) / 32 + 3) / 4;
    if (nblk > 256) nblk = 256;
    if (workspace_floats < nblk * 4096) return KGW_E_RANGE;
    Mlp2BwdArgs a{dH2, ldd, W2, ldw2, H1, ldh1, X, ldx, workspace, rows, K1, rows_dev, in_ids, dZ, ldz, (uint4*)packed, flip};
    const size_t lds = (size_t)(128 * WST + 4 * 32 * TST) * sizeof(float);
    static KgwPerDevice attr_once;
    if (attr_once.need()) {
        KGW_HIP(hipFuncSetAttribute((const void*)k_mlp2_bwd_first, hipFuncAttributeMaxDynamicSharedMemorySize, (int)lds));
    }
    hipStream_t st = (hipStream_t)stream_;
    static const bool split3 = !(getenv("KGW_MLP2_SPLIT") && getenv("KGW_MLP2_SPLIT")[0] == '0');
    if (packed && (!split3 || rows_dev || ((uintptr_t)packed & 15))) return KGW_E_UNSUPPORTED;
    if (split3) {
        const size_t lds3 = (size_t)M3_W2_U4 * 16 + (size_t)(4 * 32 * TS2) * sizeof(float);
        static KgwPerDevice attr3_set;
        if (attr3_set.need()) {
            KGW_HIP(hipFuncSetAttribute((const void*)k_mlp2_bwd_first3<false>, hipFuncAttributeMaxDynamicSharedMemorySize, (int)lds3));
            KGW_HIP(hipFuncSetAttribute((const void*)k_mlp2_bwd_first3<true>, hipFuncAttributeMaxDynamicSharedMemorySize, (int)lds3));
        }
        if (packed) k_mlp2_bwd_first3<true><<<(int)nblk, 256, lds3, st>>>(a);
        else k_mlp2_bwd_first3<false><<<(int)nblk, 256, lds3, st>>>(a);
    } else {
        k_mlp2_bwd_first<<<(int)nblk, 256, lds, st>>>(a);
    }
    KGW_LAUNCH_CHECK();
    if (defer) {
        defer[0] = KgwGradSrc{};
        defer[1] = KgwGradSrc{};
        if (K1 > 0) { defer[0].ws = workspace; defer[0].kind = KGW_GRAD_MLP2_W; defer[0].nblk = (int)nblk; defer[0].K1 = K1; }
        defer[1].ws = workspace; defer[1].kind = KGW_GRAD_MLP2_B; defer[1].nblk = (int)nblk; defer[1].K1 = K1;
        return KGW_OK;
    }
    k_mlp2_bwd_fold<<<4096 / 64, 1024, 0, st>>>(workspace, (int)nblk, K1, dW1, ldw1, db1);
    KGW_LAUNCH_CHECK();
    return KGW_OK;
}

extern "C" int kgw_mlp2_bwd_first(const float* dH2, int64_t ldd, const float* W2, int64_t ldw2, const float* H1, int64_t ldh1,
                                  const float* X, int64_t ldx, int32_t K1, int64_t rows, const int32_t* rows_dev, float* dW1,
                                  int64_t ldw1, float* db1, float* workspace, int64_t workspace_floats, const int32_t* in_ids,
                                  float* dZ, int64_t ldz, kgw_stream_t stream_) {
    return mlp2_bwd_first(dH2, ldd, W2, ldw2, H1, ldh1, X, ldx, K1, rows, rows_dev, dW1, ldw1, db1, workspace, workspace_floats,
                          in_ids, dZ, ldz, stream_, nullptr);
}

extern "C" int kgw_mlp2_bwd_first_partial(const float* dH2, int64_t ldd, const float* W2, int64_t ldw2, const float* H1,
                                          int64_t ldh1, const float* X, int64_t ldx, int32_t K1, int64_t rows,
                                          const int32_t* rows_dev, float* dW1, int64_t ldw1, float* db1, float* workspace,
                                          int64_t workspace_floats, const int32_t* in_ids, float* dZ, int64_t ldz, KgwGradSrc* src,
                                          kgw_stream_t stream_) {
    if (!src) return KGW_E_NULL;
    return mlp2_bwd_first(dH2, ldd, W2, ldw2, H1, ldh1, X, ldx, K1, rows, rows_dev, dW1, ldw1, db1, workspace, workspace_floats,
                          in_ids, dZ, ldz, stream_, src);
}

extern "C" int kgw_mlp2_bwd_first_packed(const float* dH2, int64_t ldd, const float* W2, int64_t ldw2, const float* H1,
                                         int64_t ldh1, const float* X, int64_t ldx, int32_t K1, int64_t rows, float* dW1,
                                         int64_t ldw1, float* db1, float* workspace, int64_t workspace_floats,
                                         const int32_t* in_ids, float* dZ, int64_t ldz, void* packed, int32_t flip, KgwGradSrc* src,
                                         kgw_stream_t stream_) {
    if (!packed) return KGW_E_NULL;
    if (flip < 0 || (flip & (flip - 1))) return KGW_E_RANGE;
    return mlp2_bwd_first(dH2, ldd, W2, ldw2, H1, ldh1, X, ldx, K1, rows, nullptr, dW1, ldw1, db1, workspace, workspace_floats,
                          in_ids, dZ, ldz, stream_, src, packed, flip);
}
```

kgwas_amd/csrc/kgw_dense_tn.h:

```cpp
#pragma once

namespace {

typedef float f32x16 __attribute__((ext_vector_type(16)));

template <int V> struct VecLoad;
template <> struct VecLoad<1> {
    static __device__ __forceinline__ void ld(const float* p, bool ok, float (&o)[1]) { float v = *p; o[0] = ok ? v : 0.f; }
};
template <> struct VecLoad<2> {
    static __device__ __forceinline__ void ld(const float* p, bool ok, float (&o)[2]) {
        float2 v = *(const float2*)p; o[0] = ok ? v.x : 0.f; o[1] = ok ? v.y : 0.f; }
};
template <> struct VecLoad<4> {
    static __device__ __forceinline__ void ld(const float* p, bool ok, float (&o)[4]) {
        float4 v = *(const float4*)p;
        o[0] = ok ? v.x : 0.f; o[1] = ok ? v.y : 0.f; o[2] = ok ? v.z : 0.f; o[3] = ok ? v.w : 0.f; }
};

constexpr int TN_U = 4;

template <int MT, int NT>
struct Stage { float a[TN_U][MT]; float b[TN_U][NT]; };

template <int MT, int NT>
__device__ __forceinline__ void tn_load(Stage<MT, NT>& s, const float* pa, int64_t lda2, const float* pb, int64_t ldb2) {
#pragma unroll
    for (int u = 0; u < TN_U; ++u) {
        VecLoad<MT>::ld(pa + u * lda2, true, s.a[u]);
        VecLoad<NT>::ld(pb + u * ldb2, true, s.b[u]);
    }
}

template <int MT, int NT>
__device__ __forceinline__ void tn_mma(const Stage<MT, NT>& s, f32x16 (&acc)[MT][NT], float (&sa)[MT]) {
#pragma unroll
    for (int u = 0; u < TN_U; ++u) {
#pragma unroll
        for (int a = 0; a < MT; ++a) {
            sa[a] += s.a[u][a];
#pragma unroll
            for (int b = 0; b < NT; ++b)
                acc[a][b] = __builtin_amdgcn_mfma_f32_32x32x2f32(s.a[u][a], s.b[u][b], acc[a][b], 0, 0, 0);
        }
    }
}

static int g_tn_split = -1;
static bool tn_split_on() {
    if (g_tn_split < 0) g_tn_split = !(getenv("KGW_TN_SPLIT") && getenv("KGW_TN_SPLIT")[0] == '0');
    return g_tn_split != 0;
}

static int64_t g_tn_direct = -1;
static int64_t tn_direct_rows() {
    if (g_tn_direct < 0) g_tn_direct = getenv("KGW_TN_DIRECT_ROWS") ? atoll(getenv("KGW_TN_DIRECT_ROWS")) : 0;
    return g_tn_direct;
}

constexpr int TN_MAX_JOBS = 4;
struct TnJob {
    const float* A; const float* B; float* C; float* colsum; float* ws; float* ws_cs; const int32_t* rows_dev;
    int64_t lda, ldb, rows, rpw, c_rs, c_cs, cs_ld;
    int M, N, nblk, blk0, gy, gz, cs_rep, pad_;
};
struct TnJobs { TnJob j[TN_MAX_JOBS]; int n; };

struct TnStage3 { float2 a[8], b[8]; };
__device__ __forceinline__ void tn_mma3(const TnStage3& s, const unsigned sgn, f32x16 (&acc)[2][2], float (&sa)[2]) {
    float xa0[8], xa1[8], xb0[8], xb1[8];
#pragma unroll
    for (int j = 0; j < 8; ++j) {
        sa[0] += s.a[j].x; sa[1] += s.a[j].y;
        xa0[j] = kgw_fxor(s.a[j].x, sgn); xa1[j] = kgw_fxor(s.a[j].y, sgn);
        xb0[j] = s.b[j].x; xb1[j] = s.b[j].y;
    }
    uint4 pa0[3], pa1[3], pb0[3], pb1[3];
    kgw_split3x8(xa0, pa0[0], pa0[1], pa0[2]);
    kgw_split3x8(xa1, pa1[0], pa1[1], pa1[2]);
    kgw_split3x8(xb0, pb0[0], pb0[1], pb0[2]);
    kgw_split3x8(xb1, pb1[0], pb1[1], pb1[2]);
    constexpr int TA[6] = {0, 2, 1, 0, 1, 0}, TB[6] = {2, 0, 1, 1, 0, 0};
#pragma unroll
    for (int t6 = 0; t6 < 6; ++t6) {
        const kgw_bf8 a0 = __builtin_bit_cast(kgw_bf8, pa0[TA[t6]]), a1 = __builtin_bit_cast(kgw_bf8, pa1[TA[t6]]);
        const kgw_bf8 b0 = __builtin_bit_cast(kgw_bf8, pb0[TB[t6]]), b1 = __builtin_bit_cast(kgw_bf8, pb1[TB[t6]]);
        acc[0][0] = __builtin_amdgcn_mfma_f32_32x32x16_bf16(a0, b0, acc[0][0], 0, 0, 0);
        acc[0][1] = __builtin_amdgcn_mfma_f32_32x32x16_bf16(a0, b1, acc[0][1], 0, 0, 0);
        acc[1][0] = __builtin_amdgcn_mfma_f32_32x32x16_bf16(a1, b0, acc[1][0], 0, 0, 0);
        acc[1][1] = __builtin_amdgcn_mfma_f32_32x32x16_bf16(a1, b1, acc[1][1], 0, 0, 0);
    }
}

constexpr int TN3_FLIP = 4;
__device__ __forceinline__ void tn3_flip(unsigned& sgn, f32x16 (&acc)[2][2]) {
    sgn ^= 0x80000000u;
#pragma unroll
    for (int a = 0; a < 2; ++a)
#pragma unroll
        for (int b = 0; b < 2; ++b)
#pragma unroll
            for (int e = 0; e < 16; ++e) acc[a][b][e] = -acc[a][b][e];
}
__device__ __forceinline__ void tn_rows_split3(const float* __restrict__ A, const int64_t lda, const int cas, const float* __restrict__ B,
                                               const int64_t ldb, const int cbs, const int64_t r0, const int64_t r1, const int kg,
                                               unsigned& sgn, f32x16 (&acc)[2][2], float (&sa)[2]) {
    const int64_t nfull = (r1 - r0) / 16;
    const float* pa = A + (r0 + 8 * kg) * lda + cas;
    const float* pb = B + (r0 + 8 * kg) * ldb + cbs;
    if (nfull > 0) {
        TnStage3 cur, nxt;
#pragma unroll
        for (int j = 0; j < 8; ++j) { cur.a[j] = *(const float2*)(pa + j * lda); cur.b[j] = *(const float2*)(pb + j * ldb); }
        for (int64_t it = 1; it < nfull; ++it) {
            pa += 16 * lda; pb += 16 * ldb;
#pragma unroll
            for (int j = 0; j < 8; ++j) { nxt.a[j] = *(const float2*)(pa + j * lda); nxt.b[j] = *(const float2*)(pb + j * ldb); }
            tn_mma3(cur, sgn, acc, sa);
            if ((it & (TN3_FLIP - 1)) == 0) tn3_flip(sgn, acc);
            cur = nxt;
        }
        tn_mma3(cur, sgn, acc, sa);
    }
    const int64_t rt = r0 + nfull * 16;
    if (rt < r1) {
        TnStage3 t;
#pragma unroll
        for (int j = 0; j < 8; ++j) {
            const int64_t row = rt + 8 * kg + j;
            const bool ok = row < r1;
            const int64_t rc = ok ? row : (r1 - 1);
            const float2 va = *(const float2*)(A + rc * lda + cas), vb = *(const float2*)(B + rc * ldb + cbs);
            t.a[j] = ok ? va : make_float2(0.f, 0.f);
            t.b[j] = ok ? vb : make_float2(0.f, 0.f);
        }
        tn_mma3(t, sgn, acc, sa);
    }
}

template <int MT, int NT>
__device__ __forceinline__ void tn_gemm_block(const TnJob& T, const int bx, const int by, const int bz, float* lds) {
    const float* __restrict__ A = T.A;
    const float* __restrict__ B = T.B;
    const int64_t lda = T.lda, ldb = T.ldb;
    const int M = T.M, N = T.N;
    int64_t rows = T.rows, rows_per_wave = T.rpw;
    float* __restrict__ ws = T.ws;
    float* __restrict__ ws_colsum = T.ws_cs;
    const int nbx = T.nblk;
    const int lane = threadIdx.x & 63, wave = threadIdx.x >> 6;
    const int k = lane >> 5, i = lane & 31;
    const int m0 = by * 32 * MT, n0 = bz * 32 * NT;
    const int ca = m0 + MT * i, cb = n0 + NT * i;
    const int cas = ca < M ? ca : 0, cbs = cb < N ? cb : 0;
    const int64_t wg = (int64_t)bx * 4 + wave;
    if (T.rows_dev) {
        const int64_t re = min(rows, (int64_t)max(*T.rows_dev, 0));
        rows = re;
        rows_per_wave = ((re + (int64_t)nbx * 4 - 1) / ((int64_t)nbx * 4) + 1) & ~(int64_t)1;
    }
    const int64_t r0 = min(rows, wg * rows_per_wave);
    const int64_t r1 = min(rows, r0 + rows_per_wave);

    f32x16 acc[MT][NT];
#pragma unroll
    for (int a = 0; a < MT; ++a)
#pragma unroll
        for (int b = 0; b < NT; ++b)
#pragma unroll
            for (int e = 0; e < 16; ++e) acc[a][b][e] = 0.f;
    float sa[MT];
#pragma unroll
    for (int a = 0; a < MT; ++a) sa[a] = 0.f;

    unsigned flipm = 0u;
    bool split3 = false;
    if constexpr (MT == 2 && NT == 2) split3 = T.pad_ != 0;
    if (split3) {
        if constexpr (MT == 2 && NT == 2) {
            flipm = (wg & 1) ? 0x80000000u : 0u;
            if (r0 < r1) tn_rows_split3(A, lda, cas, B, ldb, cbs, r0, r1, k, flipm, acc, sa);
        }
    } else if (r0 < r1) {
        constexpr int STEP = 2 * TN_U;
        const int64_t nfull = (r1 - r0) / STEP;
        const float* pa = A + (r0 + k) * lda + cas;
        const float* pb = B + (r0 + k) * ldb + cbs;
        const int64_t lda2 = 2 * lda, ldb2 = 2 * ldb;
        if (nfull > 0) {
            Stage<MT, NT> cur, nxt;
            tn_load<MT, NT>(cur, pa, lda2, pb, ldb2);
            for (int64_t it = 1; it < nfull; ++it) {
                pa += STEP * lda; pb += STEP * ldb;
                tn_load<MT, NT>(nxt, pa, lda2, pb, ldb2);
                tn_mma<MT, NT>(cur, acc, sa);
                cur = nxt;
            }
            tn_mma<MT, NT>(cur, acc, sa);
            pa += STEP * lda; pb += STEP * ldb;
        }
        const int64_t rt = r0 + nfull * STEP;
        if (rt < r1) {
            Stage<MT, NT> t;
#pragma unroll
            for (int u = 0; u < TN_U; ++u) {
                const int64_t row = rt + 2 * u + k;
                const bool ok = row < r1;
                const int64_t rc = ok ? row : (r1 - 1);
                VecLoad<MT>::ld(A + rc * lda + cas, ok, t.a[u]);
                VecLoad<NT>::ld(B + rc * ldb + cbs, ok, t.b[u]);
            }
            tn_mma<MT, NT>(t, acc, sa);
        }
    }

    constexpr int FRAG = MT * NT * 16 * 64;
    float* reg0 = lds;
    float* reg1 = lds + FRAG;
    float* cs = lds + 2 * FRAG;
#pragma unroll
    for (int a = 0; a < MT; ++a) {
        const float t = sa[a] + kgw_xhalf(sa[a]);
        if (k == 0) cs[wave * 32 * MT + MT * i + a] = t;
    }
    if (wave >= 2) {
        float* dst = (wave == 2) ? reg0 : reg1;
#pragma unroll
        for (int a = 0; a < MT; ++a)
#pragma unroll
            for (int b = 0; b < NT; ++b) {
#pragma unroll
                for (int e = 0; e < 16; ++e) dst[((a * NT + b) * 16 + e) * 64 + lane] = kgw_fxor(acc[a][b][e], flipm);
                __builtin_amdgcn_sched_barrier(0);
            }
    }
    __syncthreads();
    if (wave < 2) {
        float* dst = (wave == 0) ? reg0 : reg1;
#pragma unroll
        for (int a = 0; a < MT; ++a)
#pragma unroll
            for (int b = 0; b < NT; ++b) {
#pragma unroll
                for (int e = 0; e < 16; ++e) {
                    const int idx = ((a * NT + b) * 16 + e) * 64 + lane;
                    dst[idx] = kgw_fxor(acc[a][b][e], flipm) + dst[idx];
                }
                __builtin_amdgcn_sched_barrier(0);
            }
    }
    __syncthreads();
    if (nbx == 1) {
        float* __restrict__ Cq = T.C;
        for (int f = threadIdx.x * 4; f < FRAG; f += 256 * 4) {
            const float4 x = *(const float4*)(reg0 + f), y = *(const float4*)(reg1 + f);
            const float v[4] = {x.x + y.x, x.y + y.y, x.z + y.z, x.w + y.w};
            const int e = (f >> 6) & 15, tb = (f >> 10) % NT, ta = (f >> 10) / NT;
#pragma unroll
            for (int q = 0; q < 4; ++q) {
                const int ln = (f & 63) + q;
                const int ti = (e & 3) + 8 * (e >> 2) + 4 * (ln >> 5), tj = ln & 31;
                const int m = m0 + MT * ti + ta, n = n0 + NT * tj + tb;
                if (m < M && n < N) Cq[(int64_t)m * T.c_rs + (int64_t)n * T.c_cs] = v[q];
            }
// ... 37 lines not shown
    if (by >= T.gy || bz >= T.gz) return;
    if (T.nblk == 1) return;
    const float* __restrict__ ws = T.ws;
    const float* __restrict__ ws_colsum = T.ws_cs;
    const int nblk = T.nblk, gy = T.gy, M = T.M, N = T.N, cs_rep = T.cs_rep;
    float* __restrict__ C = T.C;
    float* __restrict__ colsum = T.colsum;
    const int64_t c_rs = T.c_rs, c_cs = T.c_cs, cs_ld = T.cs_ld;
    const int m0 = by * 32 * MT, n0 = bz * 32 * NT;
    const int fl = threadIdx.x & 63, g = threadIdx.x >> 6;
    const int f = bx_ * 64 + fl;
    {
        const float* p = ws + ((int64_t)bz * gy + by) * nblk * FRAG + f;
        float s8[8] = {0.f, 0.f, 0.f, 0.f, 0.f, 0.f, 0.f, 0.f};
        int b = g;
        for (; b + 28 < nblk; b += 32) {
#pragma unroll
            for (int q = 0; q < 8; ++q) s8[q] += p[(int64_t)(b + 4 * q) * FRAG];
        }
        for (int q = 0; b < nblk; b += 4, ++q) s8[q & 7] += p[(int64_t)b * FRAG];
        sm[threadIdx.x] = ((s8[0] + s8[1]) + (s8[2] + s8[3])) + ((s8[4] + s8[5]) + (s8[6] + s8[7]));
    }
    __syncthreads();
    if (g == 0) {
        const float s = (sm[fl] + sm[64 + fl]) + (sm[128 + fl] + sm[192 + fl]);
        const int lane = f & 63, e = (f >> 6) & 15, tb = (f >> 10) % NT, ta = (f >> 10) / NT;
        const int ti = (e & 3) + 8 * (e >> 2) + 4 * (lane >> 5);
        const int tj = lane & 31;
        const int m = m0 + MT * ti + ta, n = n0 + NT * tj + tb;
        if (m < M && n < N) C[(int64_t)m * c_rs + (int64_t)n * c_cs] = s;
    }
    if (colsum && bz == 0 && bx_ == 0) {
        constexpr int NC = 32 * MT, NG = 256 / NC;
        __syncthreads();
        const int c = threadIdx.x % NC, gq = threadIdx.x / NC;
        const float* p = ws_colsum + (int64_t)by * nblk * NC + c;
        float s4[4] = {0.f, 0.f, 0.f, 0.f};
        int b = gq;
        for (; b + 3 * NG < nblk; b += 4 * NG) {
#pragma unroll
            for (int q = 0; q < 4; ++q) s4[q] += p[(int64_t)(b + q * NG) * NC];
        }
        for (int q = 0; b < nblk; b += NG, ++q) s4[q & 3] += p[(int64_t)b * NC];
        sm[threadIdx.x] = (s4[0] + s4[1]) + (s4[2] + s4[3]);
        __syncthreads();
        if (gq == 0) {
            float t = 0.f;
            for (int q = 0; q < NG; ++q) t += sm[q * NC + c];
            if (m0 + c < M)
                for (int q = 0; q < cs_rep; ++q) colsum[(int64_t)q * cs_ld + m0 + c] = t;
        }
    }
}

template <int MT, int NT>
__global__ void __launch_bounds__(256) k_tn_reduce(TnJobs J, int gz_max) {
    __shared__ float sm[256];
    tn_reduce_block<MT, NT>(J, gz_max, (int)blockIdx.x, (int)blockIdx.y, (int)blockIdx.z, sm);
}

struct TnReducePlan { int32_t valid, blocks, gy_max, gz_max; int32_t n, pad_[3]; TnJobs J; };
static_assert(sizeof(TnReducePlan) <= sizeof(KgwTnReducePlan), "KgwTnReducePlan holds a TnReducePlan");
constexpr int TN22_FRAG = 2 * 2 * 16 * 64;
inline int tn_reduce_plan_blocks(const TnReducePlan& R) { return R.valid ? (TN22_FRAG / 64) * R.gy_max * R.gz_max * R.n : 0; }
__device__ __forceinline__ void tn_reduce_plan_block(const TnJobs& J, int gy_max, int gz_max, int b, float* sm) {
    constexpr int NX = TN22_FRAG / 64;
    tn_reduce_block<2, 2>(J, gz_max, b % NX, (b / NX) % gy_max, b / (NX * gy_max), sm);
}

struct TnRideIdx { int n_rd, rd_gy, rd_gz, blk, gy_max, gz_max; };
__global__ void __launch_bounds__(256, 1) k_tn_gemm_ride(TnJobs J, TnJobs JR, TnRideIdx X) {
    extern __shared__ __attribute__((aligned(16))) float lds[];
    const int b = (int)blockIdx.x;
    if (b < X.n_rd) { tn_reduce_plan_block(JR, X.rd_gy, X.rd_gz, b, lds); return; }
    const int l = b - X.n_rd;
    const int bx = l % X.blk, by = (l / X.blk) % X.gy_max, bz = l / (X.blk * X.gy_max);
    int jq = 0;
    while (jq + 1 < J.n && bx >= J.j[jq + 1].blk0) ++jq;
    const TnJob& T = J.j[jq];
    if (by >= T.gy || bz >= T.gz) return;
    tn_gemm_block<2, 2>(T, bx - T.blk0, by, bz, lds);
}

struct TnDesc {
    const float* A; int64_t lda; int M; const float* B; int64_t ldb; int N; int64_t rows; float* C; int64_t ldc; bool c_t;
    float* colsum; int cs_rep; int64_t cs_ld; float* ws; int64_t ws_floats; const int32_t* rows_dev;
};

struct TnPlan { TnJobs J; int blk, gy_max, gz_max; bool all_direct; };
template <int MT, int NT>
int launch_tn_jobs(const TnDesc* d, int n, hipStream_t st, KgwGradSrc* defer = nullptr, TnPlan* plan = nullptr,
                   const TnReducePlan* ride = nullptr) {
    constexpr int FRAG = MT * NT * 16 * 64;
    TnJobs J{};
    J.n = n;
    int blk = 0, gy_max = 0, gz_max = 0;
    bool all_direct = true;
    for (int q = 0; q < n; ++q) {
        const TnDesc& D = d[q];
        TnJob& T = J.j[q];
        const int gy = (D.M + 32 * MT - 1) / (32 * MT), gz = (D.N + 32 * NT - 1) / (32 * NT);
        int64_t nblk = (D.rows + 4 * 64 - 1) / (4 * 64);
        const int64_t cap_small = 512;
        int64_t cap = ((MT * NT <= 4) ? cap_small : 256) / ((int64_t)gy * gz);
        if (cap < 1) cap = 1;
        if (nblk > cap) nblk = cap;
        if (nblk < 1) nblk = 1;
        const int64_t direct_max = tn_direct_rows();
        if (D.rows <= direct_max && (int64_t)gy * gz >= 16) nblk = 1;
        all_direct = all_direct && nblk == 1;
        int64_t rpw = (D.rows + nblk * 4 - 1) / (nblk * 4);
        rpw = (rpw + 1) & ~(int64_t)1;
        const int64_t need = nblk * gy * gz * FRAG + nblk * gy * 32 * MT;
        if (need > D.ws_floats) return KGW_E_RANGE;
        T.A = D.A; T.B = D.B; T.C = D.C; T.colsum = D.colsum; T.ws = D.ws;
        T.ws_cs = D.colsum ? D.ws + nblk * gy * gz * FRAG : nullptr;
        T.rows_dev = D.rows_dev;
        T.lda = D.lda; T.ldb = D.ldb; T.rows = D.rows; T.rpw = rpw;
        T.c_rs = D.c_t ? 1 : D.ldc; T.c_cs = D.c_t ? D.ldc : 1; T.cs_ld = D.cs_ld;
        T.M = D.M; T.N = D.N; T.nblk = (int)nblk; T.blk0 = blk; T.gy = gy; T.gz = gz; T.cs_rep = D.cs_rep;
        T.pad_ = (MT == 2 && NT == 2 && tn_split_on() && (D.lda & 1) == 0 && (D.ldb & 1) == 0) ? 1 : 0;
        if (defer) {
            if (D.ldc != (D.c_t ? D.M : D.N) || (D.colsum && D.cs_rep != 1)) return KGW_E_UNSUPPORTED;
            KgwGradSrc& W = defer[2 * q];
            KgwGradSrc& Bc = defer[2 * q + 1];
            W = KgwGradSrc{};
            Bc = KgwGradSrc{};
            if (nblk > 1) {
                W.kind = KGW_GRAD_TN; W.nblk = (int)nblk; W.ws = D.ws; W.M = D.M; W.N = D.N; W.MT = MT; W.NT = NT; W.gy = gy; W.gz = gz;
                W.c_transposed = D.c_t ? 1 : 0;
                if (D.colsum) {
                    Bc = W;
                    Bc.kind = KGW_GRAD_TN_COLSUM; Bc.ws = T.ws_cs;
                }
            }
        }
        blk += (int)nblk;
        gy_max = gy > gy_max ? gy : gy_max;
        gz_max = gz > gz_max ? gz : gz_max;
    }
    if (plan) { plan->J = J; plan->blk = blk; plan->gy_max = gy_max; plan->gz_max = gz_max; plan->all_direct = all_direct; return KGW_OK; }
    const size_t lds_bytes = (size_t)(2 * FRAG + 4 * 32 * MT) * sizeof(float);
    auto kern = k_tn_gemm<MT, NT>;
    static KgwPerDevice attr_once;
    if (lds_bytes > 64 * 1024 && attr_once.need()) {
        KGW_HIP(hipFuncSetAttribute((const void*)kern, hipFuncAttributeMaxDynamicSharedMemorySize, (int)lds_bytes));
    }
    if (ride && !ride->valid) ride = nullptr;
    bool rode = false;
    if constexpr (MT == 2 && NT == 2) {
        if (ride) {
            const TnRideIdx X{tn_reduce_plan_blocks(*ride), ride->gy_max, ride->gz_max, blk, gy_max, gz_max};
            static KgwPerDevice attr_ride;
            if (lds_bytes > 64 * 1024 && attr_ride.need()) {
                KGW_HIP(hipFuncSetAttribute((const void*)k_tn_gemm_ride, hipFuncAttributeMaxDynamicSharedMemorySize, (int)lds_bytes));
            }
            k_tn_gemm_ride<<<X.n_rd + blk * gy_max * gz_max, 256, lds_bytes, st>>>(J, ride->J, X);
            KGW_LAUNCH_CHECK();
            rode = true;
        }
    }
    if (!rode) {
        if (ride) {
            k_tn_reduce<2, 2><<<dim3(TN22_FRAG / 64, ride->gy_max, ride->gz_max * ride->n), 256, 0, st>>>(ride->J, ride->gz_max);
            KGW_LAUNCH_CHECK();
        }
        kern<<<dim3((unsigned)blk, gy_max, gz_max), 256, lds_bytes, st>>>(J);
        KGW_LAUNCH_CHECK();
    }
    if (all_direct || defer) return KGW_OK;
    k_tn_reduce<MT, NT><<<dim3(FRAG / 64, gy_max, gz_max * n), 256, 0, st>>>(J, gz_max);
    KGW_LAUNCH_CHECK();
    return KGW_OK;
}

template <int MT, int NT>
int launch_tn(const float* A, int64_t lda, int M, const float* B, int64_t ldb, int N, int64_t rows, float* C,
              int64_t ldc, bool c_t, float* colsum, int cs_rep, int64_t cs_ld, float* ws, int64_t ws_floats,
              const int32_t* rows_dev, hipStream_t st, KgwGradSrc* defer = nullptr, const TnReducePlan* ride = nullptr) {
    const TnDesc d{A, lda, M, B, ldb, N, rows, C, ldc, c_t, colsum, cs_rep, cs_ld, ws, ws_floats, rows_dev};
    return launch_tn_jobs<MT, NT>(&d, 1, st, defer, nullptr, ride);
}

inline bool aligned16(const void* p) { return ((uintptr_t)p & 15) == 0; }

}

extern "C" int64_t kgw_tn_direct_rows(int64_t rows) {
    const int64_t was = tn_direct_rows();
    if (rows >= 0) g_tn_direct = rows;
    return was;
}

extern "C" int kgw_tn_split(int on) {
    const int was = tn_split_on() ? 1 : 0;
    if (on >= 0) g_tn_split = on ? 1 : 0;
    return was;
}

extern "C" int64_t kgw_tn_gemm_workspace_floats(int64_t rows, int M, int N) {
    const int64_t gy1 = 4 * ((M + 127) / 128), gz1 = 4 * ((N + 127) / 128);
    int64_t nblk = (rows + 255) / 256;
    if (nblk > 1024) nblk = 1024;
    if (nblk < 1) nblk = 1;
    return nblk * gy1 * gz1 * 1024 + nblk * gy1 * 32 + 4096;
}

static int tn_gemm_ex(const float* A, int64_t lda, int32_t M, const float* B, int64_t ldb, int32_t N,
                      int64_t rows, float* C, int64_t ldc, int32_t c_transposed, float* colsum_a,
                      int32_t colsum_repeat, int64_t colsum_ld, float* workspace, int64_t workspace_floats,
                      const int32_t* rows_dev, kgw_stream_t stream_, KgwGradSrc* defer, const TnReducePlan* ride = nullptr) {
    if (!A || !B || !C || !workspace) return KGW_E_NULL;
    if (M <= 0 || N <= 0 || rows <= 0 || lda < M || ldb < N || ldc < (c_transposed ? M : N)) return KGW_E_RANGE;
    if (colsum_a && (colsum_repeat < 1 || (colsum_repeat > 1 && colsum_ld < M))) return KGW_E_RANGE;
    hipStream_t st = (hipStream_t)stream_;
    const bool ct = c_transposed != 0;
    const int rep = colsum_a ? colsum_repeat : 0;
    auto aligned8 = [](const void* p) { return ((uintptr_t)p & 7) == 0; };
    const bool a2 = (M % 2 == 0) && (lda % 2 == 0) && aligned8(A) && M >= 64;
    const bool b2 = (N % 2 == 0) && (ldb % 2 == 0) && aligned8(B) && N >= 64;
    const bool b4 = (N % 4 == 0) && (ldb % 4 == 0) && aligned16(B) && N >= 128;
#define KGW_TN_ARGS A, lda, M, B, ldb, N, rows, C, ldc, ct, colsum_a, rep, colsum_ld, workspace, workspace_floats, rows_dev, st, defer, ride
    if (a2 && b2) return launch_tn<2, 2>(KGW_TN_ARGS);
    if (a2)       return launch_tn<2, 1>(KGW_TN_ARGS);
    if (b4)       return launch_tn<1, 4>(KGW_TN_ARGS);
    if (b2)       return launch_tn<1, 2>(KGW_TN_ARGS);
    return launch_tn<1, 1>(KGW_TN_ARGS);
#undef KGW_TN_ARGS
}

extern "C" int kgw_tn_gemm_ex(const float* A, int64_t lda, int32_t M, const float* B, int64_t ldb, int32_t N,
                              int64_t rows, float* C, int64_t ldc, int32_t c_transposed, float* colsum_a,
                              int32_t colsum_repeat, int64_t colsum_ld, float* workspace, int64_t workspace_floats,
                              const int32_t* rows_dev, kgw_stream_t stream_) {
    return tn_gemm_ex(A, lda, M, B, ldb, N, rows, C, ldc, c_transposed, colsum_a, colsum_repeat, colsum_ld, workspace,
                      workspace_floats, rows_dev, stream_, nullptr);
}

extern "C" int kgw_tn_gemm_partial(const float* A, int64_t lda, int32_t M, const float* B, int64_t ldb, int32_t N,
                                   int64_t rows, float* C, int64_t ldc, int32_t c_transposed, float* colsum_a,
                                   float* workspace, int64_t workspace_floats, const int32_t* rows_dev, KgwGradSrc* src,
                                   kgw_stream_t stream_) {
    if (!src) return KGW_E_NULL;
    return tn_gemm_ex(A, lda, M, B, ldb, N, rows, C, ldc, c_transposed, colsum_a, 1, M, workspace, workspace_floats, rows_dev,
                      stream_, src);
}

extern "C" int kgw_tn_gemm_partial_ride(const float* A, int64_t lda, int32_t M, const float* B, int64_t ldb, int32_t N,
                                        int64_t rows, float* C, int64_t ldc, int32_t c_transposed, float* colsum_a,
                                        float* workspace, int64_t workspace_floats, const int32_t* rows_dev, KgwGradSrc* src,
                                        const KgwTnReducePlan* ride_in, kgw_stream_t stream_) {
    if (!src) return KGW_E_NULL;
    return tn_gemm_ex(A, lda, M, B, ldb, N, rows, C, ldc, c_transposed, colsum_a, 1, M, workspace, workspace_floats, rows_dev,
                      stream_, src, (const TnReducePlan*)ride_in);
}

static int tn_gemm_multi(int32_t n_jobs, const KgwTnJob* jobs, kgw_stream_t stream_, KgwGradSrc* defer) {
    if (n_jobs == 0) return KGW_OK;
    if (!jobs) return KGW_E_NULL;
    if (n_jobs < 0 || n_jobs > TN_MAX_JOBS) return KGW_E_RANGE;
    TnDesc d[TN_MAX_JOBS];
    auto aligned8 = [](const void* p) { return ((uintptr_t)p & 7) == 0; };
    for (int q = 0; q < n_jobs; ++q) {
        const KgwTnJob& j = jobs[q];
        if (!j.A || !j.B || !j.C || !j.workspace) return KGW_E_NULL;
        if (j.M <= 0 || j.N <= 0 || j.rows <= 0 || j.lda < j.M || j.ldb < j.N || j.ldc < (j.c_transposed ? j.M : j.N)) return KGW_E_RANGE;
        if (j.colsum_a && (j.colsum_repeat < 1 || (j.colsum_repeat > 1 && j.colsum_ld < j.M))) return KGW_E_RANGE;
        if ((j.M & 1) || (j.lda & 1) || !aligned8(j.A) || (j.N & 1) || (j.ldb & 1) || !aligned8(j.B)) return KGW_E_UNSUPPORTED;
        d[q] = TnDesc{j.A, j.lda, j.M, j.B, j.ldb, j.N, j.rows, j.C, j.ldc, j.c_transposed != 0, j.colsum_a,
                      j.colsum_a ? j.colsum_repeat : 0, j.colsum_ld, j.workspace, j.workspace_floats, j.rows_dev};
    }
    return launch_tn_jobs<2, 2>(d, n_jobs, (hipStream_t)stream_, defer);
}

extern "C" int kgw_tn_gemm_multi(int32_t n_jobs, const KgwTnJob* jobs, kgw_stream_t stream_) {
    return tn_gemm_multi(n_jobs, jobs, stream_, nullptr);
}

extern "C" int kgw_tn_gemm_multi_partial(int32_t n_jobs, const KgwTnJob* jobs, KgwGradSrc* src, kgw_stream_t stream_) {
    if (n_jobs > 0 && !src) return KGW_E_NULL;
    return tn_gemm_multi(n_jobs, jobs, stream_, src);
}

extern "C" int kgw_tn_gemm(const float* A, int64_t lda, int32_t M, const float* B, int64_t ldb, int32_t N,
                           int64_t rows, float* C, int64_t ldc, float* colsum_a, float* workspace,
                           int64_t workspace_floats, kgw_stream_t stream_) {
    return kgw_tn_gemm_ex(A, lda, M, B, ldb, N, rows, C, ldc, 0, colsum_a, 1, M, workspace, workspace_floats, nullptr, stream_);
}
```

kgwas_amd/ops.py:

```python
from __future__ import annotations

import ctypes as C
import os
import weakref
import sys

import torch

from . import _lib
from ._lib import KGW_C, PART_STRIDE, KgwLayerArgs


def _p(t):
    return t.data_ptr() if t is not None else 0


class _TunedLibraryGemm:

    def __init__(self):
        self.on = os.environ.get('KGW_TUNABLE_GEMM', '1') == '1'
        self._ready = False

    def __enter__(self):
        if not self.on:
# ... 462 lines not shown
    return torch.empty(zr * (KGW_C + 3) + (-(zr * (KGW_C + 3))) % 4, device=device)


def gat_aggregate(batch, layer: int, H: torch.Tensor, U: torch.Tensor, V: torch.Tensor,
                  neg_slope: float = 0.2, temperature: float = 1.0, raw_weights: bool = False,
                  relu_input: bool = False, zbuf: torch.Tensor = None, logit_bias: torch.Tensor = None):
    stat, e_edge, Z = _GatAggregate.apply(H, U, V, batch, layer, float(neg_slope), 1.0 / float(temperature), raw_weights,
                                          relu_input, zbuf, logit_bias)
    xchg = getattr(batch, 'exchange', None)
    if xchg is not None and xchg.staged and xchg.mask[layer] and Z.requires_grad:
        Zx = Z.detach().requires_grad_()
        xchg.cuts.append((layer, Z, Zx))
        Z = Zx
    return Z, stat, e_edge


gat_aggregate_flat = gat_aggregate


def edge_alpha(batch, layer: int, stat: torch.Tensor, e_edge: torch.Tensor, temperature: float = 1.0):
    a = _layer_args(batch, layer, 0.2, 1.0 / float(temperature))
    n_edges = int(batch.meta.n_edges[layer - 1])
    out = torch.zeros(max(n_edges, 1), device=e_edge.device)
    a.stat, a.e_edge = _p(stat), _p(e_edge)
    _lib.check(_lib.lib().kgw_edge_alpha(C.byref(a), C.c_void_p(out.data_ptr()), _lib.stream_ptr()), 'kgw_edge_alpha')
    return out[:n_edges]


_TN_MIN_ROWS = 1024


def tn_gemm(A: torch.Tensor, B: torch.Tensor, colsum: bool = False, out: torch.Tensor = None,
            transpose_out: bool = False, colsum_out: torch.Tensor = None, rows_dev: torch.Tensor = None, defer: bool = False):
    assert A.dim() == 2 and B.dim() == 2 and A.shape[0] == B.shape[0]
    assert A.dtype == torch.float32 and B.dtype == torch.float32
    if A.stride(1) != 1:
        A = A.contiguous()
    if B.stride(1) != 1:
        B = B.contiguous()
    rows, M = A.shape
    N = B.shape[1]
    dev = A.device
    if out is None:
        out = torch.empty((N, M) if transpose_out else (M, N), device=dev)
    assert out.shape == ((N, M) if transpose_out else (M, N)) and out.stride(1) == 1
    cs = None
    rep, cs_ld = 1, M
    if colsum_out is not None:
        assert colsum_out.dim() == 2 and colsum_out.shape[1] == M and colsum_out.stride(1) == 1
        cs, rep, cs_ld = colsum_out, colsum_out.shape[0], colsum_out.stride(0)
    elif colsum:
        cs = torch.empty(M, device=dev)
    if rows == 0:
        out.zero_()
        if cs is not None:
            cs.zero_()
        return (out, cs) if (colsum or colsum_out is not None) else out
    L = _lib.lib()
    nws = int(L.kgw_tn_gemm_workspace_floats(rows, M, N))
    ws = torch.empty(nws, device=dev)
    sink = GRAD_SINK
    if defer and sink is not None and colsum_out is None and out.is_contiguous():
        src = (_lib.KgwGradSrc * 2)()
        ride = sink.take_reduce()
        if ride is not None:
            _lib.check(L.kgw_tn_gemm_partial_ride(_p(A), A.stride(0), M, _p(B), B.stride(0), N, rows, _p(out), out.stride(0),
                                                  1 if transpose_out else 0, _p(cs), _p(ws), nws, _p(rows_dev), src, C.byref(ride[0]),
                                                  _lib.stream_ptr()), 'kgw_tn_gemm_partial_ride')
            sink.reduces_ridden += 1
        else:
            _lib.check(L.kgw_tn_gemm_partial(_p(A), A.stride(0), M, _p(B), B.stride(0), N, rows, _p(out), out.stride(0),
                                             1 if transpose_out else 0, _p(cs), _p(ws), nws, _p(rows_dev), src, _lib.stream_ptr()),
                       'kgw_tn_gemm_partial')
        sink.add(out, src[0], ws)
        if cs is not None:
            sink.add(cs, src[1], ws)
        return (out, cs) if colsum else out
    _lib.check(L.kgw_tn_gemm_ex(_p(A), A.stride(0), M, _p(B), B.stride(0), N, rows, _p(out), out.stride(0),
                                1 if transpose_out else 0, _p(cs), rep, cs_ld, _p(ws), nws, _p(rows_dev), _lib.stream_ptr()),
               'kgw_tn_gemm_ex')
    return (out, cs) if (colsum or colsum_out is not None) else out


def _tn_gemm_group(jobs) -> bool:
    if not (2 <= len(jobs) <= 4):
        return False
    for A, B, out, cs in jobs:
        if not (A.dtype == torch.float32 and B.dtype == torch.float32 and A.stride(1) == 1 and B.stride(1) == 1 and out.stride(1) == 1 and
                cs.stride(1) == 1 and A.shape[0] == B.shape[0] and A.shape[0] > 0 and A.shape[1] % 2 == 0 and B.shape[1] % 2 == 0 and
                A.shape[1] >= 64 and B.shape[1] >= 64 and A.stride(0) % 2 == 0 and B.stride(0) % 2 == 0 and A.data_ptr() % 8 == 0 and
                B.data_ptr() % 8 == 0 and out.shape == (B.shape[1], A.shape[1]) and cs.shape[1] == A.shape[1]):
            return False
    L = _lib.lib()
    arr = (_lib.KgwTnJob * len(jobs))()
    keep = []
    for q, (A, B, out, cs) in enumerate(jobs):
        rows, M = A.shape
        N = B.shape[1]
        nws = int(L.kgw_tn_gemm_workspace_floats(rows, M, N))
        ws = torch.empty(nws, device=A.device)
        keep.append(ws)
        j = arr[q]
        j.A, j.lda, j.B, j.ldb, j.rows = _p(A), A.stride(0), _p(B), B.stride(0), rows
        j.C, j.ldc, j.colsum_a, j.colsum_ld = _p(out), out.stride(0), _p(cs), cs.stride(0)
        j.workspace, j.workspace_floats, j.rows_dev = _p(ws), nws, None
        j.M, j.N, j.c_transposed, j.colsum_repeat = M, N, 1, cs.shape[0]
    _lib.check(L.kgw_tn_gemm_multi(len(jobs), arr, _lib.stream_ptr()), 'kgw_tn_gemm_multi')
    return True


def weight_grads(pairs, rows_dev: torch.Tensor = None):
    pairs = [(dY if dY.stride(1) == 1 else dY.contiguous(), X if X.stride(1) == 1 else X.contiguous()) for dY, X in pairs]
    if GRAD_SINK is not None and _DEFER_PRODUCTS:
        return [linear_weight_grad(dY, X, rows_dev=rows_dev) for dY, X in pairs]
    ok = 1 < len(pairs) <= 4 and all(_TN_MIN_ROWS <= X.shape[0] < 32768 and X.shape[1] <= 1024 and X.shape[1] % 2 == 0 and dY.shape[1] % 2 == 0 and
                                     X.stride(0) % 2 == 0 and dY.stride(0) % 2 == 0 and X.data_ptr() % 8 == 0 and dY.data_ptr() % 8 == 0
                                     for dY, X in pairs)
    if not ok:
        return [linear_weight_grad(dY, X, rows_dev=rows_dev) for dY, X in pairs]
    L = _lib.lib()
    jobs = (_lib.KgwTnJob * len(pairs))()
    outs, keep = [], []
    for q, (dY, X) in enumerate(pairs):
        rows, M = dY.shape
        N = X.shape[1]
        dW = torch.empty(M, N, device=dY.device)
        db = torch.empty(M, device=dY.device)
        nws = int(L.kgw_tn_gemm_workspace_floats(rows, M, N))
        ws = torch.empty(nws, device=dY.device)
        keep.append(ws)
        j = jobs[q]
        j.A, j.lda, j.B, j.ldb, j.rows = _p(dY), dY.stride(0), _p(X), X.stride(0), rows
        j.C, j.ldc, j.colsum_a, j.colsum_ld = _p(dW), N, _p(db), M
        j.workspace, j.workspace_floats, j.rows_dev = _p(ws), nws, _p(rows_dev)
        j.M, j.N, j.c_transposed, j.colsum_repeat = M, N, 0, 1
        outs.append((dW, db))
    sink = GRAD_SINK
    if sink is not None:
        src = (_lib.KgwGradSrc * (2 * len(pairs)))()
        _lib.check(L.kgw_tn_gemm_multi_partial(len(pairs), jobs, src, _lib.stream_ptr()), 'kgw_tn_gemm_multi_partial')
        for q, (dW, db) in enumerate(outs):
            sink.add(dW, src[2 * q], keep[q])
            sink.add(db, src[2 * q + 1], keep[q])
        return outs
    _lib.check(L.kgw_tn_gemm_multi(len(pairs), jobs, _lib.stream_ptr()), 'kgw_tn_gemm_multi')
    return outs


def _library_linear(X, W, bias, relu, mask, w_kn, out, fixed_shape):
    LIBRARY_GEMM.note('linear', X.shape[0], X.shape[1], W.shape[1] if w_kn else W.shape[0])
    Wop = W if w_kn else W.t()
    if fixed_shape and mask is None and out is None:
        with _TUNED:
            if bias is not None and relu:
                return torch._addmm_activation(bias, X, Wop)
            Y = torch.addmm(bias, X, Wop) if bias is not None else X @ Wop
        return torch.relu_(Y) if relu else Y
    if bias is not None and relu and X.is_cuda:
        Y = torch._addmm_activation(bias, X, Wop, out=out) if (out is not None and mask is None) else \
            torch._addmm_activation(bias, X, Wop)
        if mask is None:
            return Y
        relu = False
    elif mask is None and out is not None:
        Y = torch.addmm(bias, X, Wop, out=out) if bias is not None else torch.mm(X, Wop, out=out)
        return torch.relu_(Y) if relu else Y
# ... 430 lines not shown
        b = self.buf
        t = torch.empty(0, dtype=b.dtype, device=b.device)
        return t.set_(b.untyped_storage(), b.storage_offset() + self.lo * b.stride(0), (self.n,) + tuple(b.shape[1:]),
                      b.stride())


class _JoinBlocks(torch.autograd.Function):

    @staticmethod
    def forward(ctx, holder, spans, *parts):
        buf = holder.buf
        for (lo, n), p in zip(spans, parts):
            dst = buf[lo:lo + n]
            if p.data_ptr() != dst.data_ptr() or p.stride(0) != buf.stride(0):
                dst.copy_(p)
        ctx.spans = spans
        return holder.view()

    @staticmethod
    def backward(ctx, dH):
        return (None, None) + tuple(dH[lo:lo + n] for lo, n in ctx.spans)


class _SplitRows(torch.autograd.Function):

    @staticmethod
    def forward(ctx, y, sizes):
        ctx.sizes = sizes
        ctx.set_materialize_grads(False)
        outs, off = [], 0
        for n in sizes:
            outs.append(RowBlock(y, off, n).view())
            off += n
        return tuple(outs)

    @staticmethod
    def backward(ctx, *gs):
        sizes = ctx.sizes
        if all(g is not None for g in gs):
            g0 = gs[0]
            adj, ptr = g0.is_contiguous(), g0.data_ptr()
            for g, n in zip(gs, sizes):
                adj = adj and g.is_contiguous() and g.data_ptr() == ptr and g.untyped_storage().data_ptr() == g0.untyped_storage().data_ptr()
                ptr += n * g.shape[1] * g.element_size()
            if adj:
                total = sum(sizes)
                t = torch.empty(0, dtype=g0.dtype, device=g0.device)
                return t.set_(g0.untyped_storage(), g0.storage_offset(), (total, g0.shape[1]), (g0.shape[1], 1)), None
        first = next(g for g in gs if g is not None)
        parts = [g if g is not None else torch.zeros(n, first.shape[1], device=first.device) for g, n in zip(gs, sizes)]
        return torch.cat(parts, 0), None


def split_rows(y: torch.Tensor, sizes):
    return _SplitRows.apply(y, tuple(int(n) for n in sizes))


def join_blocks(buf: torch.Tensor, spans, parts):
    return _JoinBlocks.apply(RowBlock(buf, 0, buf.shape[0]), tuple(spans), *parts)


class _MLP3(torch.autograd.Function):

    @staticmethod
    def forward(ctx, x, W1, b1, W2, b2, W3, b3, out, rows_dev):
        h1 = linear(x, W1, b1, relu=True, rows_dev=rows_dev)
        h2 = linear(h1, W2, b2, relu=True, rows_dev=rows_dev)
        y = linear(h2, W3, b3, out=out.view() if out is not None else None, rows_dev=rows_dev)
        ctx.save_for_backward(x, h1, h2, W2, W3)
        ctx.rows_dev = rows_dev
        return y

    @staticmethod
    def backward(ctx, dy):
        x, h1, h2, W2, W3 = ctx.saved_tensors
        rd = ctx.rows_dev
        dy = dy.contiguous()
        dh2 = linear(dy, W3, mask=h2, w_kn=True, rows_dev=rd)
        dh1 = linear(dh2, W2, mask=h1, w_kn=True, rows_dev=rd)
        (dW3, db3), (dW2, db2), (dW1, db1) = weight_grads([(dy, h2), (dh2, h1), (dh1, x)], rows_dev=rd)
        return None, dW1, db1, dW2, db2, dW3, db3, None, None


class _MLP2(torch.autograd.Function):

    @staticmethod
    def forward(ctx, x, W1, b1, W2, b2, out, rows_dev, ids=None):
        rows, K1 = (x.shape if ids is None else (ids.numel(), x.shape[1]))
        h2 = out.view() if out is not None else None
        if (rows >= 16384 and K1 <= 20 and K1 % 4 == 0 and W1.shape[0] == KGW_C and W2.shape == (KGW_C, KGW_C)
                and x.dtype == torch.float32 and x.stride(1) == 1 and x.stride(0) % 4 == 0 and x.data_ptr() % 16 == 0
                and W1.stride(1) == 1 and W2.stride(1) == 1 and W2.stride(0) % 4 == 0 and W2.data_ptr() % 16 == 0
                and b1 is not None and b2 is not None and (ids is None or ids.dtype == torch.int32)
                and (h2 is None or (h2.stride(1) == 1 and h2.stride(0) % 4 == 0 and h2.data_ptr() % 16 == 0))):
            if h2 is None:
                h2 = torch.empty(rows, KGW_C, device=x.device)
            h1 = torch.empty(rows, KGW_C, device=x.device)
            xg = torch.empty(rows, K1, device=x.device) if ids is not None else None
            _lib.check(_lib.lib().kgw_mlp2_fwd(_p(x), x.stride(0), K1, _p(W1), W1.stride(0), _p(b1), _p(W2), W2.stride(0), _p(b2),
                                               _p(h1), h1.stride(0), _p(h2), h2.stride(0), rows, _p(rows_dev), _p(ids), _p(xg),
                                               K1, _lib.stream_ptr()), 'kgw_mlp2_fwd')
            ctx.save_for_backward(x if ids is None else xg, h1, W2)
            ctx.rows_dev = rows_dev
            return h2
        if ids is not None:
            from .sampler import gather_rows
            x = gather_rows(x, ids)
        h1 = linear(x, W1, b1, relu=True, rows_dev=rows_dev)
        h2 = linear(h1, W2, b2, relu=True, out=h2, rows_dev=rows_dev)
        ctx.save_for_backward(x, h1, W2)
        ctx.rows_dev = rows_dev
        return h2

    @staticmethod
    def backward(ctx, dh2):
        x, h1, W2 = ctx.saved_tensors
        rd = ctx.rows_dev
        dh2 = dh2.contiguous()
        rows, K1 = x.shape
        if (rows >= 16384 and K1 <= 31 and h1.shape[1] == KGW_C and W2.shape == (KGW_C, KGW_C) and x.stride(1) == 1
                and h1.stride(1) == 1 and dh2.stride(0) % 4 == 0 and h1.stride(0) % 4 == 0 and W2.stride(0) % 4 == 0
                and dh2.data_ptr() % 16 == 0 and h1.data_ptr() % 16 == 0 and W2.data_ptr() % 16 == 0):
            L = _lib.lib()
            dW1 = torch.empty(KGW_C, K1, device=x.device)
            db1 = torch.empty(KGW_C, device=x.device)
            nws = int(L.kgw_mlp2_bwd_first_workspace_floats(rows))
            ws = torch.empty(nws, device=x.device)
            sink = GRAD_SINK
            if sink is not None:
                src = (_lib.KgwGradSrc * 2)()
                _lib.check(L.kgw_mlp2_bwd_first_partial(_p(dh2), dh2.stride(0), _p(W2), W2.stride(0), _p(h1), h1.stride(0), _p(x), x.stride(0),
                                                        K1, rows, _p(rd), _p(dW1), K1, _p(db1), _p(ws), nws, None, None, 0, src,
                                                        _lib.stream_ptr()), 'kgw_mlp2_bwd_first_partial')
                sink.add(dW1, src[0], ws)
                sink.add(db1, src[1], ws)
            else:
                _lib.check(L.kgw_mlp2_bwd_first(_p(dh2), dh2.stride(0), _p(W2), W2.stride(0), _p(h1), h1.stride(0), _p(x), x.stride(0), K1,
                                                rows, _p(rd), _p(dW1), K1, _p(db1), _p(ws), nws, None, None, 0, _lib.stream_ptr()), 'kgw_mlp2_bwd_first')
            dW2, db2 = linear_weight_grad(dh2, h1, rows_dev=rd)
            return None, dW1, db1, dW2, db2, None, None, None
        dh1 = linear(dh2, W2, mask=h1, w_kn=True, rows_dev=rd)
        (dW2, db2), (dW1, db1) = weight_grads([(dh2, h1), (dh1, x)], rows_dev=rd)
        return None, dW1, db1, dW2, db2, None, None, None


def mlp2(x, W1, b1, W2, b2, out=None, rows_dev=None, ids=None):
    return _MLP2.apply(x, W1, b1, W2, b2, out, rows_dev, ids)


class _MLP2Gathered(torch.autograd.Function):

    @staticmethod
    def forward(ctx, W1, b1, W2, b2, out, *jobs):
        srcs, idss = jobs[0::2], jobs[1::2]
        n = len(srcs)
        rows = sum(int(i.numel()) for i in idss)
        dev = W1.device
        h2 = out.view() if out is not None else torch.empty(rows, KGW_C, device=dev)
        xg = torch.empty(rows, KGW_C, device=dev)
        h1 = torch.empty(rows, KGW_C, device=dev)
        S = (C.c_void_p * n)(*[_p(x) for x in srcs])
        I = (C.c_void_p * n)(*[_p(i) for i in idss])
        N = (C.c_int64 * n)(*[int(i.numel()) for i in idss])
        assert h2.stride(0) == KGW_C or rows == 0 or h2.stride(0) % 4 == 0
        if h2.stride(0) != KGW_C:
            h2c = torch.empty(rows, KGW_C, device=dev)
        else:
            h2c = h2
        _lib.check(_lib.lib().kgw_mlp2w_fwd(n, S, I, N, srcs[0].stride(0), _p(W1), W1.stride(0), _p(b1), _p(W2), W2.stride(0), _p(b2),
                                            _p(xg), _p(h1), _p(h2c), KGW_C, _lib.stream_ptr()), 'kgw_mlp2w_fwd')
        if h2c is not h2:
            h2.copy_(h2c)
        ctx.save_for_backward(xg, h1, W2)
        return h2

    @staticmethod
    def backward(ctx, dh2):
        x, h1, W2 = ctx.saved_tensors
        dh2 = dh2.contiguous()
        dh1 = linear(dh2, W2, mask=h1, w_kn=True)
        (dW2, db2), (dW1, db1) = weight_grads([(dh2, h1), (dh1, x)])
        return (dW1, db1, dW2, db2, None) + (None,) * (len(ctx.needs_input_grad) - 5)


def mlp2_gathered(jobs, W1, b1, W2, b2, out=None):
    flat = []
    for x, i in jobs:
        flat += [x, i]
    return _MLP2Gathered.apply(W1, b1, W2, b2, out, *flat)


def mlp2_gathered_ok(jobs, W1, W2) -> bool:
    return (1 <= len(jobs) <= 4 and W1.shape == (KGW_C, KGW_C) and W2.shape == (KGW_C, KGW_C)
            and all(x.dtype == torch.float32 and x.shape[1] == KGW_C and x.stride(1) == 1 and x.stride(0) % 4 == 0 and
                    x.data_ptr() % 16 == 0 and i.dtype == torch.int32 and x.stride(0) == jobs[0][0].stride(0) for x, i in jobs)
            and 0 < sum(int(i.numel()) for _, i in jobs) <= 16384)


class _MLPTail2(torch.autograd.Function):

    @staticmethod
# ... 779 lines not shown
```

Before: 1.077 billion.

## Recompute MLP hidden layer in backward and store ReLU masks as bits

Result: no change. 1.068 billion (-0.9%).

```diff
diff --git a/include/kgwas_hip.h b/include/kgwas_hip.h
--- a/include/kgwas_hip.h
+++ b/include/kgwas_hip.h
@@ -292,6 +292,18 @@
                               float* workspace, int64_t workspace_floats, const int32_t* in_ids, float* dZ, int64_t ldz,
                               void* packed, int32_t flip, KgwGradSrc* src, kgw_stream_t stream);
 
+int kgw_mlp2_fwd_bits(const float* X, int64_t ldx, int32_t K1, const float* W1, int64_t ldw1, const float* b1, const float* W2,
+                      int64_t ldw2, const float* b2, float* H1, int64_t ldh1, float* H2, int64_t ldh2, int64_t rows,
+                      const int32_t* rows_dev, const int32_t* ids, float* Xg, int64_t ldxg, uint32_t* bits, kgw_stream_t stream);
+int kgw_mlp2_bwd_first_bits(const float* dH2, int64_t ldd, const float* W2, int64_t ldw2, const uint32_t* bits, const float* X,
+                            int64_t ldx, int32_t K1, int64_t rows, const int32_t* rows_dev, float* dW1, int64_t ldw1,
+                            float* db1, float* workspace, int64_t workspace_floats, KgwGradSrc* src, kgw_stream_t stream);
+
+int kgw_tn_gemm_h1(const float* A, int64_t lda, int32_t M, const float* X, int64_t ldx, int32_t K1, const float* W1, int64_t ldw1,
+                   const float* b1, int64_t rows, float* C, int64_t ldc, int32_t c_transposed, float* colsum_a, float* workspace,
+                   int64_t workspace_floats, const int32_t* rows_dev, KgwGradSrc* src, const KgwTnReducePlan* ride_in,
+                   kgw_stream_t stream);
+
 int64_t kgw_gemm3_packed_bytes(int64_t K);
 int64_t kgw_gemm3_workspace_floats(int64_t M, int64_t K);
 int kgw_gemm3_pack(const float* S, int64_t lds, int64_t K, int64_t k_valid, int32_t s_is_kn, void* packed, kgw_stream_t stream);
diff --git a/kgwas_amd/_lib.py b/kgwas_amd/_lib.py
--- a/kgwas_amd/_lib.py
+++ b/kgwas_amd/_lib.py
@@ -163,7 +163,7 @@
 EXPORTS = ['kgw_version', 'kgw_status_string', 'kgw_struct_sizes', 'kgw_sample_batch', 'kgw_sample_batch_parts', 'kgw_sample_batch_fanout', 'kgw_sampler_scan_ints', 'kgw_segments_copy',
            'kgw_softmax_pack', 'kgw_softmax_merge', 'kgw_scatter_rows', 'kgw_linear_splitk', 'kgw_linear_splitk_workspace_floats', 'kgw_linear_splitk_ind', 'kgw_ind_colsum', 'kgw_linear_splitk_multi', 'kgw_ind_colsum_multi', 'kgw_fold_fwd', 'kgw_fold_bwd', 'kgw_relation_sums',
            'kgw_gat_aggregate_fwd', 'kgw_gat_aggregate_bwd_dst', 'kgw_gat_aggregate_bwd_src',
-           'kgw_gather_rows', 'kgw_gather_rows_multi', 'kgw_scatter_relu_rows', 'kgw_scatter_relu_rows_workspace_floats', 'kgw_edge_alpha', 'kgw_debug_reduce', 'kgw_debug_reduce8', 'kgw_tn_gemm', 'kgw_tn_gemm_ex', 'kgw_tn_gemm_multi', 'kgw_tn_gemm_workspace_floats', 'kgw_tn_gemm_partial', 'kgw_tn_gemm_multi_partial', 'kgw_tn_split', 'kgw_tn_direct_rows', 'kgw_param_tail', 'kgw_tn_reduce_launch', 'kgw_tn_gemm_partial_ride', 'kgw_transform_bwd_ex', 'kgw_mlp2_bwd_first_partial', 'kgw_mlp2_bwd_first_packed', 'kgw_adam_fused', 'kgw_gemm3_partial', 'kgw_gemm3_flip', 'kgw_transform_bwd', 'kgw_grad_finish',
+           'kgw_gather_rows', 'kgw_gather_rows_multi', 'kgw_scatter_relu_rows', 'kgw_scatter_relu_rows_workspace_floats', 'kgw_edge_alpha', 'kgw_debug_reduce', 'kgw_debug_reduce8', 'kgw_tn_gemm', 'kgw_tn_gemm_ex', 'kgw_tn_gemm_multi', 'kgw_tn_gemm_workspace_floats', 'kgw_tn_gemm_partial', 'kgw_tn_gemm_multi_partial', 'kgw_tn_split', 'kgw_tn_direct_rows', 'kgw_param_tail', 'kgw_tn_reduce_launch', 'kgw_tn_gemm_partial_ride', 'kgw_transform_bwd_ex', 'kgw_mlp2_bwd_first_partial', 'kgw_mlp2_bwd_first_packed', 'kgw_mlp2_fwd_bits', 'kgw_mlp2_bwd_first_bits', 'kgw_tn_gemm_h1', 'kgw_adam_fused', 'kgw_gemm3_partial', 'kgw_gemm3_flip', 'kgw_transform_bwd', 'kgw_grad_finish',
            'kgw_linear', 'kgw_mlp2_fwd', 'kgw_mlp2w_fwd', 'kgw_mlp2_bwd_first', 'kgw_mlp2_bwd_first_workspace_floats', 'kgw_gemm3', 'kgw_gemm3_riders', 'kgw_gemm3_rider_blocks', 'kgw_gemm3_pack', 'kgw_gemm3_packed_bytes', 'kgw_gemm3_workspace_floats', 'kgw_adam', 'kgw_adam_notick', 'kgw_relvec_fwd', 'kgw_relvec_bwd', 'kgw_relvec_bwd_acc', 'kgw_relvec_fwd_multi', 'kgw_relvec_bwd_multi', 'kgw_wmse_fwd', 'kgw_wmse_bwd', 'kgw_readout_wmse_fwd', 'kgw_readout_wmse_bwd', 'kgw_readout_wmse_train', 'kgw_readout_wmse_train_parts', 'kgw_readout_train_fold', 'kgw_accumulate_stats', 'kgw_accumulate_stats_tick']
 
 _lib = None
@@ -276,6 +276,13 @@
     L.kgw_mlp2_bwd_first_packed.argtypes = [C.c_void_p, C.c_int64, C.c_void_p, C.c_int64, C.c_void_p, C.c_int64, C.c_void_p, C.c_int64, C.c_int32,
                                             C.c_int64, C.c_void_p, C.c_int64, C.c_void_p, C.c_void_p, C.c_int64, C.c_void_p, C.c_void_p,
                                             C.c_int64, C.c_void_p, C.c_int32, C.c_void_p, C.c_void_p]
+    L.kgw_mlp2_fwd_bits.argtypes = L.kgw_mlp2_fwd.argtypes[:-1] + [C.c_void_p, C.c_void_p]
+    L.kgw_mlp2_bwd_first_bits.argtypes = [C.c_void_p, C.c_int64, C.c_void_p, C.c_int64, C.c_void_p, C.c_void_p, C.c_int64, C.c_int32,
+                                          C.c_int64, C.c_void_p, C.c_void_p, C.c_int64, C.c_void_p, C.c_void_p, C.c_int64,
+                                          C.POINTER(KgwGradSrc), C.c_void_p]
+    L.kgw_tn_gemm_h1.argtypes = [C.c_void_p, C.c_int64, C.c_int32, C.c_void_p, C.c_int64, C.c_int32, C.c_void_p, C.c_int64, C.c_void_p,
+                                 C.c_int64, C.c_void_p, C.c_int64, C.c_int32, C.c_void_p, C.c_void_p, C.c_int64, C.c_void_p,
+                                 C.POINTER(KgwGradSrc), C.c_void_p, C.c_void_p]
     L.kgw_adam_fused.argtypes = [C.c_int32, C.c_void_p, C.c_void_p, C.c_void_p, C.c_void_p, C.c_void_p, C.POINTER(KgwGradSrc), C.c_void_p,
                                  C.c_float, C.c_float, C.c_float, C.c_float, C.c_float, C.c_void_p, C.c_int32, C.c_int32, C.c_void_p,
                                  C.c_void_p, C.c_void_p]
diff --git a/kgwas_amd/csrc/kgw_dense_linear.h b/kgwas_amd/csrc/kgw_dense_linear.h
--- a/kgwas_amd/csrc/kgw_dense_linear.h
+++ b/kgwas_amd/csrc/kgw_dense_linear.h
@@ -144,7 +144,6 @@
 
 constexpr int WST = 132;
 
-typedef float f32x4 __attribute__((ext_vector_type(4)));
 
 template <int KC, bool WKN, int RT>
 __global__ void __launch_bounds__(512) __attribute__((amdgpu_waves_per_eu(2, 2))) k_linear_wres(LinArgs a_) {
@@ -474,7 +473,23 @@
     const int32_t* rows_dev;
     const int32_t* ids;
     float* Xg; int64_t ldxg;
+    uint32_t* mask;
 };
+
+__device__ __forceinline__ uint2 mlp2_mask_bits(const f32x4 (&xa)[16]) {
+    unsigned mb[2] = {0u, 0u};
+#pragma unroll
+    for (int t = 0; t < 4; ++t)
+#pragma unroll
+        for (int g = 0; g < 4; ++g) {
+            const int b0 = (t & 1) * 16 + 4 * g;
+            mb[t >> 1] |= (xa[4 * t + g].x > 0.f ? 1u : 0u) << (b0 + 0);
+            mb[t >> 1] |= (xa[4 * t + g].y > 0.f ? 1u : 0u) << (b0 + 1);
+            mb[t >> 1] |= (xa[4 * t + g].z > 0.f ? 1u : 0u) << (b0 + 2);
+            mb[t >> 1] |= (xa[4 * t + g].w > 0.f ? 1u : 0u) << (b0 + 3);
+        }
+    return make_uint2(mb[0], mb[1]);
+}
 
 __global__ void __launch_bounds__(256) __attribute__((amdgpu_waves_per_eu(1, 1))) k_mlp2_fwd(Mlp2Args a) {
     extern __shared__ __attribute__((aligned(16))) float lds[];
@@ -490,6 +505,7 @@
             const int64_t r = rows + q / 32; const int c4 = (int)(q % 32) * 4;
             *(float4*)(a.H2 + r * a.ldh2 + c4) = make_float4(0.f, 0.f, 0.f, 0.f);
             if (a.H1) *(float4*)(a.H1 + r * a.ldh1 + c4) = make_float4(0.f, 0.f, 0.f, 0.f);
+            if (a.mask && c4 == 0) *(uint4*)(a.mask + r * 4) = make_uint4(0u, 0u, 0u, 0u);
         }
         if ((int64_t)blockIdx.x * 4 * 32 >= rows) return;
     }
@@ -579,6 +595,7 @@
 #pragma unroll
             for (int q = 0; q < 16; ++q) *(f32x4*)(hp + 32 * (q >> 2) + 8 * (q & 3)) = xa[q];
         }
+        if (a.mask && live) *(uint2*)(a.mask + row * 4 + 2 * lk) = mlp2_mask_bits(xa);
 #pragma unroll
         for (int t = 0; t < 4; ++t)
 #pragma unroll
@@ -629,6 +646,7 @@
             const int64_t r = rows + q / 32; const int c4 = (int)(q % 32) * 4;
             *(float4*)(a.H2 + r * a.ldh2 + c4) = make_float4(0.f, 0.f, 0.f, 0.f);
             if (a.H1) *(float4*)(a.H1 + r * a.ldh1 + c4) = make_float4(0.f, 0.f, 0.f, 0.f);
+            if (a.mask && c4 == 0) *(uint4*)(a.mask + r * 4) = make_uint4(0u, 0u, 0u, 0u);
         }
         if ((int64_t)blockIdx.x * 8 * 32 >= rows) return;
     }
@@ -709,6 +727,7 @@
 #pragma unroll
             for (int q = 0; q < 16; ++q) *(f32x4*)(hp + 32 * (q >> 2) + 8 * (q & 3)) = xa[q];
         }
+        if (a.mask && live) *(uint2*)(a.mask + row * 4 + 2 * lk) = mlp2_mask_bits(xa);
 #pragma unroll
         for (int t = 0; t < 4; ++t)
 #pragma unroll
@@ -913,11 +932,13 @@
     const int32_t* rows_dev;
     const int32_t* in_ids;
     float* dZ; int64_t ldz;
+    const uint2* bits;
     uint4* packed; int flip;
 };
 
 constexpr int TST = 132;
 
+template <bool BITS>
 __global__ void __launch_bounds__(256) __attribute__((amdgpu_waves_per_eu(1, 1))) k_mlp2_bwd_first(Mlp2BwdArgs a) {
     extern __shared__ __attribute__((aligned(16))) float lds[];
     float* Wl = lds;
@@ -964,6 +985,7 @@
     {
         int64_t r = (int64_t)(tile < ntiles ? tile : ntiles - 1) * 32 + li;
         if (r >= rows) r = rows - 1;
+        if (r < 0) r = 0;
         src_cur = a.in_ids ? a.in_ids[r] : 0;
         const float* xp = a.dH2 + (a.in_ids ? (int64_t)(src_cur < 0 ? 0 : src_cur) : r) * a.ldd + lk * 64;
 #pragma unroll
@@ -991,8 +1013,10 @@
             if (rr < rows) v = li < K1 ? a.X[rr * a.ldx + li] : (li == K1 ? 1.f : 0.f);
             xs[s2] = v;
         }
-        const float* mp = a.H1 + rc * a.ldm + 4 * lk;
+        constexpr bool bits = BITS;
+        const float* mp = bits ? nullptr : a.H1 + rc * a.ldm + 4 * lk;
         unsigned mb[2] = {0u, 0u};
+        if (bits) { const uint2 m = a.bits[rc * 2 + lk]; mb[0] = m.x; mb[1] = m.y; }
         f32x4 mv[4];
 #define KGW_MLPB_MFETCH(T)                                                                                \
         _Pragma("unroll") for (int g = 0; g < 4; ++g) mv[g] = *(const f32x4*)(mp + (T) * 32 + 8 * g);
@@ -1012,11 +1036,13 @@
         f32x4 b2n = *(const f32x4*)w2, b3n = *(const f32x4*)w3;
 #pragma unroll
         for (int q = 0; q < 16; ++q) {
-            if (q == 0) { KGW_MLPB_MFETCH(0) }
-            if (q == 3) { KGW_MLPB_MBITS(0) KGW_MLPB_MFETCH(1) }
-            if (q == 6) { KGW_MLPB_MBITS(1) KGW_MLPB_MFETCH(2) }
-            if (q == 10) { KGW_MLPB_MBITS(2) KGW_MLPB_MFETCH(3) }
-            if (q == 14) { KGW_MLPB_MBITS(3) }
+            if (!bits) {
+                if (q == 0) { KGW_MLPB_MFETCH(0) }
+                if (q == 3) { KGW_MLPB_MBITS(0) KGW_MLPB_MFETCH(1) }
+                if (q == 6) { KGW_MLPB_MBITS(1) KGW_MLPB_MFETCH(2) }
+                if (q == 10) { KGW_MLPB_MBITS(2) KGW_MLPB_MFETCH(3) }
+                if (q == 14) { KGW_MLPB_MBITS(3) }
+            }
             const f32x4 b2 = b2n, b3 = b3n;
             if (q + 1 < 16) { b2n = *(const f32x4*)(w2 + 4 * (q + 1)); b3n = *(const f32x4*)(w3 + 4 * (q + 1)); }
 #define KGW_MLPB_STEP(C)                                                                                  \
@@ -1074,7 +1100,7 @@
 
 constexpr int TS2 = 68;
 
-template <bool PACK>
+template <bool PACK, bool BITS>
 __global__ void __launch_bounds__(256) __attribute__((amdgpu_waves_per_eu(1, 1))) k_mlp2_bwd_first3(Mlp2BwdArgs a) {
     extern __shared__ __attribute__((aligned(16))) float lds[];
     uint4* W2p = (uint4*)lds;
@@ -1112,6 +1138,7 @@
     {
         int64_t r = (int64_t)(tile < ntiles ? tile : ntiles - 1) * 32 + li;
         if (r >= rows) r = rows - 1;
+        if (r < 0) r = 0;
         src_cur = a.in_ids ? a.in_ids[r] : 0;
         const float* xp = a.dH2 + (a.in_ids ? (int64_t)(src_cur < 0 ? 0 : src_cur) : r) * a.ldd + lk * 64;
 #pragma unroll
@@ -1126,9 +1153,16 @@
         MB[t_ >> 1] |= (MV[t_][g].w > 0.f ? 1u : 0u) << (b0 + 3);                                        \
     }
     unsigned mb[2] = {0u, 0u};
-    {
+    if (BITS) {
         int64_t r = (int64_t)(tile < ntiles ? tile : ntiles - 1) * 32 + li;
         if (r >= rows) r = rows - 1;
+        if (r < 0) r = 0;
+        const uint2 m = a.bits[r * 2 + lk];
+        mb[0] = m.x; mb[1] = m.y;
+    } else {
+        int64_t r = (int64_t)(tile < ntiles ? tile : ntiles - 1) * 32 + li;
+        if (r >= rows) r = rows - 1;
+        if (r < 0) r = 0;
         const float* mp = a.H1 + r * a.ldm + 4 * lk;
         f32x4 mv[4][4];
 #pragma unroll
@@ -1159,8 +1193,15 @@
             if (rr < rows) v = li < K1 ? a.X[rr * a.ldx + li] : (li == K1 ? 1.f : 0.f);
             xs[s2] = v;
         }
-        f32x4 mvn[4][4];
-        {
+        f32x4 mvn[BITS ? 1 : 4][4];
+        uint2 mbn = make_uint2(0u, 0u);
+        if (BITS) {
+            int nt = tile + nw;
+            if (nt >= ntiles) nt = ntiles - 1;
+            int64_t r = (int64_t)nt * 32 + li;
+            if (r >= rows) r = rows - 1;
+            mbn = a.bits[r * 2 + lk];
+        } else {
             int nt = tile + nw;
             if (nt >= ntiles) nt = ntiles - 1;
             int64_t r = (int64_t)nt * 32 + li;
@@ -1245,8 +1286,12 @@
             }
             __asm__ volatile("s_waitcnt lgkmcnt(0)" ::: "memory");
         }
-        mb[0] = 0u; mb[1] = 0u;
-        KGW_MLPB_BITS(mvn, mb)
+        if (BITS) {
+            mb[0] = mbn.x; mb[1] = mbn.y;
+        } else {
+            mb[0] = 0u; mb[1] = 0u;
+            KGW_MLPB_BITS(mvn, mb)
+        }
     }
 #undef KGW_MLPB_BITS
     __syncthreads();
@@ -1455,18 +1500,19 @@
     return KGW_OK;
 }
 
-extern "C" int kgw_mlp2_fwd(const float* X, int64_t ldx, int32_t K1, const float* W1, int64_t ldw1, const float* b1,
-                            const float* W2, int64_t ldw2, const float* b2, float* H1, int64_t ldh1, float* H2, int64_t ldh2,
-                            int64_t rows, const int32_t* rows_dev, const int32_t* ids, float* Xg, int64_t ldxg,
-                            kgw_stream_t stream_) {
+static int mlp2_fwd(const float* X, int64_t ldx, int32_t K1, const float* W1, int64_t ldw1, const float* b1,
+                    const float* W2, int64_t ldw2, const float* b2, float* H1, int64_t ldh1, float* H2, int64_t ldh2,
+                    int64_t rows, const int32_t* rows_dev, const int32_t* ids, float* Xg, int64_t ldxg, uint32_t* mask,
+                    kgw_stream_t stream_) {
     if (rows == 0) return KGW_OK;
     if (!X || !W1 || !W2 || !H2) return KGW_E_NULL;
+    if (mask && !aligned16(mask)) return KGW_E_UNSUPPORTED;
     if (Xg && ((ldxg & 3) || !aligned16(Xg))) return KGW_E_UNSUPPORTED;
     if (rows < 0 || K1 <= 0) return KGW_E_RANGE;
     if (K1 > 20 || (K1 & 3) || (ldx & 3) || (ldw2 & 3) || (ldh2 & 3) || (H1 && (ldh1 & 3)) || !aligned16(X) || !aligned16(W2) ||
         !aligned16(H2) || (H1 && !aligned16(H1)))
         return KGW_E_UNSUPPORTED;
-    Mlp2Args a{X, ldx, W1, ldw1, b1, W2, ldw2, b2, H1, ldh1, H2, ldh2, rows, K1, rows_dev, ids, Xg, ldxg};
+    Mlp2Args a{X, ldx, W1, ldw1, b1, W2, ldw2, b2, H1, ldh1, H2, ldh2, rows, K1, rows_dev, ids, Xg, ldxg, mask};
     const size_t lds = (size_t)(128 * WST + 128 + 128 * 24) * sizeof(float);
     static KgwPerDevice attr_once;
     if (attr_once.need()) {
@@ -1488,6 +1534,21 @@
     k_mlp2_fwd<<<(int)(nblk < 256 ? nblk : 256), 256, lds, (hipStream_t)stream_>>>(a);
     KGW_LAUNCH_CHECK();
     return KGW_OK;
+}
+
+extern "C" int kgw_mlp2_fwd(const float* X, int64_t ldx, int32_t K1, const float* W1, int64_t ldw1, const float* b1,
+                            const float* W2, int64_t ldw2, const float* b2, float* H1, int64_t ldh1, float* H2, int64_t ldh2,
+                            int64_t rows, const int32_t* rows_dev, const int32_t* ids, float* Xg, int64_t ldxg,
+                            kgw_stream_t stream_) {
+    return mlp2_fwd(X, ldx, K1, W1, ldw1, b1, W2, ldw2, b2, H1, ldh1, H2, ldh2, rows, rows_dev, ids, Xg, ldxg, nullptr, stream_);
+}
+
+extern "C" int kgw_mlp2_fwd_bits(const float* X, int64_t ldx, int32_t K1, const float* W1, int64_t ldw1, const float* b1,
+                                 const float* W2, int64_t ldw2, const float* b2, float* H1, int64_t ldh1, float* H2, int64_t ldh2,
+                                 int64_t rows, const int32_t* rows_dev, const int32_t* ids, float* Xg, int64_t ldxg,
+                                 uint32_t* bits, kgw_stream_t stream_) {
+    if (rows != 0 && !bits) return KGW_E_NULL;
+    return mlp2_fwd(X, ldx, K1, W1, ldw1, b1, W2, ldw2, b2, H1, ldh1, H2, ldh2, rows, rows_dev, ids, Xg, ldxg, bits, stream_);
 }
 
 extern "C" int kgw_mlp2w_fwd(int32_t n_jobs, const float* const* src, const int32_t* const* ids, const int64_t* n_rows,
@@ -1532,21 +1593,24 @@
 static int mlp2_bwd_first(const float* dH2, int64_t ldd, const float* W2, int64_t ldw2, const float* H1, int64_t ldh1,
                           const float* X, int64_t ldx, int32_t K1, int64_t rows, const int32_t* rows_dev, float* dW1,
                           int64_t ldw1, float* db1, float* workspace, int64_t workspace_floats, const int32_t* in_ids,
-                          float* dZ, int64_t ldz, kgw_stream_t stream_, KgwGradSrc* defer, void* packed = nullptr, int flip = 0) {
-    if (!dH2 || !W2 || !H1 || !db1 || !workspace) return KGW_E_NULL;
+                          float* dZ, int64_t ldz, kgw_stream_t stream_, KgwGradSrc* defer, void* packed = nullptr, int flip = 0,
+                          const uint32_t* bits = nullptr) {
+    if (!dH2 || !W2 || (!H1 && !bits) || !db1 || !workspace) return KGW_E_NULL;
+    if (bits && (packed || ((uintptr_t)bits & 7))) return KGW_E_UNSUPPORTED;
     if (defer && K1 > 0 && ldw1 != K1) return KGW_E_UNSUPPORTED;
     if (rows <= 0 || K1 < 0) return KGW_E_RANGE;
     if (K1 > 0 && (!X || !dW1)) return KGW_E_NULL;
     if (dZ && ((ldz & 3) || !aligned16(dZ))) return KGW_E_UNSUPPORTED;
-    if (K1 > 31 || (ldd & 3) || (ldw2 & 3) || (ldh1 & 3) || !aligned16(dH2) || !aligned16(W2) || !aligned16(H1)) return KGW_E_UNSUPPORTED;
+    if (K1 > 31 || (ldd & 3) || (ldw2 & 3) || (!bits && ((ldh1 & 3) || !aligned16(H1))) || !aligned16(dH2) || !aligned16(W2)) return KGW_E_UNSUPPORTED;
     int64_t nblk = ((rows + 31) / 32 + 3) / 4;
     if (nblk > 256) nblk = 256;
     if (workspace_floats < nblk * 4096) return KGW_E_RANGE;
-    Mlp2BwdArgs a{dH2, ldd, W2, ldw2, H1, ldh1, X, ldx, workspace, rows, K1, rows_dev, in_ids, dZ, ldz, (uint4*)packed, flip};
+    Mlp2BwdArgs a{dH2, ldd, W2, ldw2, H1, ldh1, X, ldx, workspace, rows, K1, rows_dev, in_ids, dZ, ldz, (const uint2*)bits, (uint4*)packed, flip};
     const size_t lds = (size_t)(128 * WST + 4 * 32 * TST) * sizeof(float);
     static KgwPerDevice attr_once;
     if (attr_once.need()) {
-        KGW_HIP(hipFuncSetAttribute((const void*)k_mlp2_bwd_first, hipFuncAttributeMaxDynamicSharedMemorySize, (int)lds));
+        KGW_HIP(hipFuncSetAttribute((const void*)k_mlp2_bwd_first<false>, hipFuncAttributeMaxDynamicSharedMemorySize, (int)lds));
+        KGW_HIP(hipFuncSetAttribute((const void*)k_mlp2_bwd_first<true>, hipFuncAttributeMaxDynamicSharedMemorySize, (int)lds));
     }
     hipStream_t st = (hipStream_t)stream_;
     static const bool split3 = !(getenv("KGW_MLP2_SPLIT") && getenv("KGW_MLP2_SPLIT")[0] == '0');
@@ -1555,13 +1619,16 @@
         const size_t lds3 = (size_t)M3_W2_U4 * 16 + (size_t)(4 * 32 * TS2) * sizeof(float);
         static KgwPerDevice attr3_set;
         if (attr3_set.need()) {
-            KGW_HIP(hipFuncSetAttribute((const void*)k_mlp2_bwd_first3<false>, hipFuncAttributeMaxDynamicSharedMemorySize, (int)lds3));
-            KGW_HIP(hipFuncSetAttribute((const void*)k_mlp2_bwd_first3<true>, hipFuncAttributeMaxDynamicSharedMemorySize, (int)lds3));
-        }
-        if (packed) k_mlp2_bwd_first3<true><<<(int)nblk, 256, lds3, st>>>(a);
-        else k_mlp2_bwd_first3<false><<<(int)nblk, 256, lds3, st>>>(a);
+            KGW_HIP(hipFuncSetAttribute((const void*)k_mlp2_bwd_first3<false, false>, hipFuncAttributeMaxDynamicSharedMemorySize, (int)lds3));
+            KGW_HIP(hipFuncSetAttribute((const void*)k_mlp2_bwd_first3<true, false>, hipFuncAttributeMaxDynamicSharedMemorySize, (int)lds3));
+            KGW_HIP(hipFuncSetAttribute((const void*)k_mlp2_bwd_first3<false, true>, hipFuncAttributeMaxDynamicSharedMemorySize, (int)lds3));
+        }
+        if (packed) k_mlp2_bwd_first3<true, false><<<(int)nblk, 256, lds3, st>>>(a);
+        else if (bits) k_mlp2_bwd_first3<false, true><<<(int)nblk, 256, lds3, st>>>(a);
+        else k_mlp2_bwd_first3<false, false><<<(int)nblk, 256, lds3, st>>>(a);
     } else {
-        k_mlp2_bwd_first<<<(int)nblk, 256, lds, st>>>(a);
+        if (bits) k_mlp2_bwd_first<true><<<(int)nblk, 256, lds, st>>>(a);
+        else k_mlp2_bwd_first<false><<<(int)nblk, 256, lds, st>>>(a);
     }
     KGW_LAUNCH_CHECK();
     if (defer) {
@@ -1604,3 +1671,12 @@
     return mlp2_bwd_first(dH2, ldd, W2, ldw2, H1, ldh1, X, ldx, K1, rows, nullptr, dW1, ldw1, db1, workspace, workspace_floats,
                           in_ids, dZ, ldz, stream_, src, packed, flip);
 }
+
+extern "C" int kgw_mlp2_bwd_first_bits(const float* dH2, int64_t ldd, const float* W2, int64_t ldw2, const uint32_t* bits,
+                                       const float* X, int64_t ldx, int32_t K1, int64_t rows, const int32_t* rows_dev, float* dW1,
+                                       int64_t ldw1, float* db1, float* workspace, int64_t workspace_floats, KgwGradSrc* src,
+                                       kgw_stream_t stream_) {
+    if (!bits) return KGW_E_NULL;
+    return mlp2_bwd_first(dH2, ldd, W2, ldw2, nullptr, 0, X, ldx, K1, rows, rows_dev, dW1, ldw1, db1, workspace, workspace_floats,
+                          nullptr, nullptr, 0, stream_, src, nullptr, 0, bits);
+}
diff --git a/kgwas_amd/csrc/kgw_dense_tn.h b/kgwas_amd/csrc/kgw_dense_tn.h
--- a/kgwas_amd/csrc/kgw_dense_tn.h
+++ b/kgwas_amd/csrc/kgw_dense_tn.h
@@ -3,6 +3,7 @@
 namespace {
 
 typedef float f32x16 __attribute__((ext_vector_type(16)));
+typedef float f32x4 __attribute__((ext_vector_type(4)));
 
 template <int V> struct VecLoad;
 template <> struct VecLoad<1> {
@@ -138,8 +139,125 @@
     }
 }
 
-template <int MT, int NT>
-__device__ __forceinline__ void tn_gemm_block(const TnJob& T, const int bx, const int by, const int bz, float* lds) {
+struct TnH1 { const float* X; const float* W1; const float* b1; int64_t ldx, ldw1; int K1; };
+constexpr int TNH_TS = 68;
+constexpr int TNH_LDS_FLOATS = 64 * 24 + 4 * 32 * TNH_TS;
+
+__device__ __forceinline__ void tnh_tile(const TnH1& H, const float* W1l, float* Tw, const int64_t rt, const int64_t r1, const int li,
+                                         const int lk) {
+    int64_t r = rt + li;
+    if (r >= r1) r = r1 - 1;
+    const float* xp = H.X + r * H.ldx;
+    f32x4 x[3];
+#pragma unroll
+    for (int c = 0; c < 3; ++c) {
+        const int k4 = 12 * lk + 4 * c;
+        if (k4 + 4 <= H.K1) x[c] = *(const f32x4*)(xp + k4);
+        else x[c] = f32x4{k4 == H.K1 ? 1.f : 0.f, 0.f, 0.f, 0.f};
+    }
+    f32x16 acc[2];
+#pragma unroll
+    for (int t = 0; t < 2; ++t)
+#pragma unroll
+        for (int e = 0; e < 16; ++e) acc[t][e] = 0.f;
+    const float* w1p = W1l + li * 24 + 12 * lk;
+#pragma unroll
+    for (int c = 0; c < 3; ++c) {
+        f32x4 w[2];
+#pragma unroll
+        for (int t = 0; t < 2; ++t) w[t] = *(const f32x4*)(w1p + t * 32 * 24 + 4 * c);
+#define KGW_TNH_STEP(C)                                                                                   \
+        _Pragma("unroll") for (int t = 0; t < 2; ++t)                                                    \
+            acc[t] = __builtin_amdgcn_mfma_f32_32x32x2f32(w[t].C, x[c].C, acc[t], 0, 0, 0);
+        KGW_TNH_STEP(x) KGW_TNH_STEP(y) KGW_TNH_STEP(z) KGW_TNH_STEP(w)
+#undef KGW_TNH_STEP
+    }
+#pragma unroll
+    for (int t = 0; t < 2; ++t)
+#pragma unroll
+        for (int g = 0; g < 4; ++g) {
+            f32x4 v;
+            v.x = fmaxf(acc[t][4 * g + 0], 0.f); v.y = fmaxf(acc[t][4 * g + 1], 0.f);
+            v.z = fmaxf(acc[t][4 * g + 2], 0.f); v.w = fmaxf(acc[t][4 * g + 3], 0.f);
+            *(f32x4*)(Tw + li * TNH_TS + t * 32 + 8 * g + 4 * lk) = v;
+        }
+    __asm__ volatile("s_waitcnt lgkmcnt(0)" ::: "memory");
+}
+
+__device__ __forceinline__ void tn_rows_split3_h1(const float* __restrict__ A, const int64_t lda, const int cas, const TnH1& H,
+                                                  const float* W1l, float* Tw, const int64_t r0, const int64_t r1, const int kg,
+                                                  const int i, unsigned& sgn, f32x16 (&acc)[2][2], float (&sa)[2]) {
+    const int64_t nfull = (r1 - r0) / 16;
+    const float* pa = A + (r0 + 8 * kg) * lda + cas;
+    if (nfull > 0) {
+        TnStage3 cur, nxt;
+#pragma unroll
+        for (int j = 0; j < 8; ++j) cur.a[j] = *(const float2*)(pa + j * lda);
+        for (int64_t s = 0; s < nfull; ++s) {
+            const bool more = s + 1 < nfull;
+            if (more) {
+                pa += 16 * lda;
+#pragma unroll
+                for (int j = 0; j < 8; ++j) nxt.a[j] = *(const float2*)(pa + j * lda);
+            }
+            if (!(s & 1)) tnh_tile(H, W1l, Tw, r0 + 16 * s, r1, i, kg);
+            const float* tp = Tw + (16 * (int)(s & 1) + 8 * kg) * TNH_TS + 2 * i;
+#pragma unroll
+            for (int j = 0; j < 8; ++j) cur.b[j] = *(const float2*)(tp + j * TNH_TS);
+            __asm__ volatile("s_waitcnt lgkmcnt(0)" ::: "memory");
+            tn_mma3(cur, sgn, acc, sa);
+            if (more) {
+                if (((s + 1) & (TN3_FLIP - 1)) == 0) tn3_flip(sgn, acc);
+#pragma unroll
+                for (int j = 0; j < 8; ++j) cur.a[j] = nxt.a[j];
+            }
+        }
+    }
+    const int64_t rt = r0 + nfull * 16;
+    if (rt < r1) {
+        if (!(nfull & 1)) tnh_tile(H, W1l, Tw, rt, r1, i, kg);
+        const float* tp = Tw + (16 * (int)(nfull & 1) + 8 * kg) * TNH_TS + 2 * i;
+        TnStage3 t;
+#pragma unroll
+        for (int j = 0; j < 8; ++j) {
+            const int64_t row = rt + 8 * kg + j;
+            const bool ok = row < r1;
+            const int64_t rc = ok ? row : (r1 - 1);
+            const float2 va = *(const float2*)(A + rc * lda + cas), vb = *(const float2*)(tp + j * TNH_TS);
+            t.a[j] = ok ? va : make_float2(0.f, 0.f);
+            t.b[j] = ok ? vb : make_float2(0.f, 0.f);
+        }
+        __asm__ volatile("s_waitcnt lgkmcnt(0)" ::: "memory");
+        tn_mma3(t, sgn, acc, sa);
+    }
+}
+
+__device__ __forceinline__ void tn_rows_fp32_h1(const float* __restrict__ A, const int64_t lda, const int cas, const TnH1& H,
+                                                const float* W1l, float* Tw, const int64_t r0, const int64_t r1, const int k,
+                                                const int i, f32x16 (&acc)[2][2], float (&sa)[2]) {
+    constexpr int STEP = 2 * TN_U;
+    const int64_t nst = (r1 - r0 + STEP - 1) / STEP;
+    for (int64_t st = 0; st < nst; ++st) {
+        const int64_t rs = r0 + st * STEP;
+        if (!(st & 3)) tnh_tile(H, W1l, Tw, rs, r1, i, k);
+        Stage<2, 2> g;
+#pragma unroll
+        for (int u = 0; u < TN_U; ++u) {
+            const int64_t row = rs + 2 * u + k;
+            const bool ok = row < r1;
+            const int64_t rc = ok ? row : (r1 - 1);
+            VecLoad<2>::ld(A + rc * lda + cas, ok, g.a[u]);
+            const float2 vb = *(const float2*)(Tw + (STEP * (int)(st & 3) + 2 * u + k) * TNH_TS + 2 * i);
+            g.b[u][0] = ok ? vb.x : 0.f; g.b[u][1] = ok ? vb.y : 0.f;
+        }
+        __asm__ volatile("s_waitcnt lgkmcnt(0)" ::: "memory");
+        tn_mma<2, 2>(g, acc, sa);
+    }
+}
+
+template <int MT, int NT, bool H1R = false>
+__device__ __forceinline__ void tn_gemm_block(const TnJob& T, const int bx, const int by, const int bz, float* lds,
+                                              const TnH1* HH = nullptr) {
     const float* __restrict__ A = T.A;
     const float* __restrict__ B = T.B;
     const int64_t lda = T.lda, ldb = T.ldb;
@@ -173,13 +291,31 @@
 #pragma unroll
     for (int a = 0; a < MT; ++a) sa[a] = 0.f;
 
+    float* W1l = lds + 2 * MT * NT * 16 * 64 + 4 * 32 * MT;
+    float* Tw = W1l + 64 * 24 + wave * 32 * TNH_TS;
+    if constexpr (H1R) {
+        for (int idx = threadIdx.x; idx < 64 * 24; idx += 256) {
+            const int n = n0 + idx / 24, kk = idx % 24;
+            W1l[idx] = kk < HH->K1 ? HH->W1[(int64_t)n * HH->ldw1 + kk] : (kk == HH->K1 ? (HH->b1 ? HH->b1[n] : 0.f) : 0.f);
+        }
+        __syncthreads();
+    }
+
     unsigned flipm = 0u;
     bool split3 = false;
     if constexpr (MT == 2 && NT == 2) split3 = T.pad_ != 0;
     if (split3) {
         if constexpr (MT == 2 && NT == 2) {
             flipm = (wg & 1) ? 0x80000000u : 0u;
-            if (r0 < r1) tn_rows_split3(A, lda, cas, B, ldb, cbs, r0, r1, k, flipm, acc, sa);
+            if constexpr (H1R) {
+                if (r0 < r1) tn_rows_split3_h1(A, lda, cas, *HH, W1l, Tw, r0, r1, k, i, flipm, acc, sa);
+            } else {
+                if (r0 < r1) tn_rows_split3(A, lda, cas, B, ldb, cbs, r0, r1, k, flipm, acc, sa);
+            }
+        }
+    } else if (H1R) {
+        if constexpr (H1R) {
+            if (r0 < r1) tn_rows_fp32_h1(A, lda, cas, *HH, W1l, Tw, r0, r1, k, i, acc, sa);
         }
     } else if (r0 < r1) {
         constexpr int STEP = 2 * TN_U;
@@ -383,6 +519,24 @@
     tn_gemm_block<2, 2>(T, bx - T.blk0, by, bz, lds);
 }
 
+__global__ void __launch_bounds__(256, 1) k_tn_gemm_h1(TnJobs J, TnH1 H) {
+    extern __shared__ __attribute__((aligned(16))) float lds[];
+    const TnJob& T = J.j[0];
+    if ((int)blockIdx.y >= T.gy || (int)blockIdx.z >= T.gz) return;
+    tn_gemm_block<2, 2, true>(T, (int)blockIdx.x, (int)blockIdx.y, (int)blockIdx.z, lds, &H);
+}
+
+__global__ void __launch_bounds__(256, 1) k_tn_gemm_h1_ride(TnJobs J, TnJobs JR, TnRideIdx X, TnH1 H) {
+    extern __shared__ __attribute__((aligned(16))) float lds[];
+    const int b = (int)blockIdx.x;
+    if (b < X.n_rd) { tn_reduce_plan_block(JR, X.rd_gy, X.rd_gz, b, lds); return; }
+    const int l = b - X.n_rd;
+    const int bx = l % X.blk, by = (l / X.blk) % X.gy_max, bz = l / (X.blk * X.gy_max);
+    const TnJob& T = J.j[0];
+    if (by >= T.gy || bz >= T.gz) return;
+    tn_gemm_block<2, 2, true>(T, bx, by, bz, lds, &H);
+}
+
 struct TnDesc {
     const float* A; int64_t lda; int M; const float* B; int64_t ldb; int N; int64_t rows; float* C; int64_t ldc; bool c_t;
     float* colsum; int cs_rep; int64_t cs_ld; float* ws; int64_t ws_floats; const int32_t* rows_dev;
@@ -391,7 +545,7 @@
 struct TnPlan { TnJobs J; int blk, gy_max, gz_max; bool all_direct; };
 template <int MT, int NT>
 int launch_tn_jobs(const TnDesc* d, int n, hipStream_t st, KgwGradSrc* defer = nullptr, TnPlan* plan = nullptr,
-                   const TnReducePlan* ride = nullptr) {
+                   const TnReducePlan* ride = nullptr, const TnH1* h1 = nullptr) {
     constexpr int FRAG = MT * NT * 16 * 64;
     TnJobs J{};
     J.n = n;
@@ -441,6 +595,29 @@
         gz_max = gz > gz_max ? gz : gz_max;
     }
     if (plan) { plan->J = J; plan->blk = blk; plan->gy_max = gy_max; plan->gz_max = gz_max; plan->all_direct = all_direct; return KGW_OK; }
+    if constexpr (MT == 2 && NT == 2) {
+        if (h1) {
+            if (n != 1) return KGW_E_UNSUPPORTED;
+            const size_t lds_h1 = (size_t)(2 * FRAG + 4 * 32 * MT + TNH_LDS_FLOATS) * sizeof(float);
+            static KgwPerDevice attr_h1;
+            if (attr_h1.need()) {
+                KGW_HIP(hipFuncSetAttribute((const void*)k_tn_gemm_h1, hipFuncAttributeMaxDynamicSharedMemorySize, (int)lds_h1));
+                KGW_HIP(hipFuncSetAttribute((const void*)k_tn_gemm_h1_ride, hipFuncAttributeMaxDynamicSharedMemorySize, (int)lds_h1));
+            }
+            if (ride && !ride->valid) ride = nullptr;
+            if (ride) {
+                const TnRideIdx X{tn_reduce_plan_blocks(*ride), ride->gy_max, ride->gz_max, blk, gy_max, gz_max};
+                k_tn_gemm_h1_ride<<<X.n_rd + blk * gy_max * gz_max, 256, lds_h1, st>>>(J, ride->J, X, *h1);
+            } else {
+                k_tn_gemm_h1<<<dim3((unsigned)blk, gy_max, gz_max), 256, lds_h1, st>>>(J, *h1);
+            }
+            KGW_LAUNCH_CHECK();
+            if (all_direct || defer) return KGW_OK;
+            k_tn_reduce<MT, NT><<<dim3(FRAG / 64, gy_max, gz_max * n), 256, 0, st>>>(J, gz_max);
+            KGW_LAUNCH_CHECK();
+            return KGW_OK;
+        }
+    }
     const size_t lds_bytes = (size_t)(2 * FRAG + 4 * 32 * MT) * sizeof(float);
     auto kern = k_tn_gemm<MT, NT>;
     static KgwPerDevice attr_once;
@@ -478,9 +655,10 @@
 template <int MT, int NT>
 int launch_tn(const float* A, int64_t lda, int M, const float* B, int64_t ldb, int N, int64_t rows, float* C,
               int64_t ldc, bool c_t, float* colsum, int cs_rep, int64_t cs_ld, float* ws, int64_t ws_floats,
-              const int32_t* rows_dev, hipStream_t st, KgwGradSrc* defer = nullptr, const TnReducePlan* ride = nullptr) {
+              const int32_t* rows_dev, hipStream_t st, KgwGradSrc* defer = nullptr, const TnReducePlan* ride = nullptr,
+              const TnH1* h1 = nullptr) {
     const TnDesc d{A, lda, M, B, ldb, N, rows, C, ldc, c_t, colsum, cs_rep, cs_ld, ws, ws_floats, rows_dev};
-    return launch_tn_jobs<MT, NT>(&d, 1, st, defer, nullptr, ride);
+    return launch_tn_jobs<MT, NT>(&d, 1, st, defer, nullptr, ride, h1);
 }
 
 inline bool aligned16(const void* p) { return ((uintptr_t)p & 15) == 0; }
@@ -556,6 +734,19 @@
                       stream_, src, (const TnReducePlan*)ride_in);
 }
 
+extern "C" int kgw_tn_gemm_h1(const float* A, int64_t lda, int32_t M, const float* X, int64_t ldx, int32_t K1, const float* W1,
+                              int64_t ldw1, const float* b1, int64_t rows, float* C, int64_t ldc, int32_t c_transposed,
+                              float* colsum_a, float* workspace, int64_t workspace_floats, const int32_t* rows_dev, KgwGradSrc* src,
+                              const KgwTnReducePlan* ride_in, kgw_stream_t stream_) {
+    if (!A || !X || !W1 || !C || !workspace) return KGW_E_NULL;
+    if (M <= 0 || rows <= 0 || lda < M || ldc < (c_transposed ? M : 128) || K1 <= 0 || ldx < K1 || ldw1 < K1) return KGW_E_RANGE;
+    if ((M & 1) || M < 64 || (lda & 1) || ((uintptr_t)A & 7) || K1 > 20 || (K1 & 3) || (ldx & 3) || !aligned16(X))
+        return KGW_E_UNSUPPORTED;
+    const TnH1 h{X, W1, b1, ldx, ldw1, K1};
+    return launch_tn<2, 2>(A, lda, M, nullptr, 128, 128, rows, C, ldc, c_transposed != 0, colsum_a, colsum_a ? 1 : 0, M, workspace,
+                           workspace_floats, rows_dev, (hipStream_t)stream_, src, (const TnReducePlan*)ride_in, &h);
+}
+
 static int tn_gemm_multi(int32_t n_jobs, const KgwTnJob* jobs, kgw_stream_t stream_, KgwGradSrc* defer) {
     if (n_jobs == 0) return KGW_OK;
     if (!jobs) return KGW_E_NULL;
diff --git a/kgwas_amd/ops.py b/kgwas_amd/ops.py
--- a/kgwas_amd/ops.py
+++ b/kgwas_amd/ops.py
@@ -568,6 +568,29 @@
     return (out, cs) if (colsum or colsum_out is not None) else out
 
 
+def tn_gemm_h1(A: torch.Tensor, x: torch.Tensor, W1: torch.Tensor, b1: torch.Tensor, rows_dev: torch.Tensor = None):
+    rows, M = A.shape
+    K1 = x.shape[1]
+    L = _lib.lib()
+    out = torch.empty(M, KGW_C, device=A.device)
+    cs = torch.empty(M, device=A.device)
+    nws = int(L.kgw_tn_gemm_workspace_floats(rows, M, KGW_C))
+    ws = torch.empty(nws, device=A.device)
+    sink = GRAD_SINK
+    src = (_lib.KgwGradSrc * 2)() if sink is not None else None
+    ride = sink.take_reduce() if sink is not None else None
+    _lib.check(L.kgw_tn_gemm_h1(_p(A), A.stride(0), M, _p(x), x.stride(0), K1, _p(W1), W1.stride(0), _p(b1), rows, _p(out), KGW_C, 0,
+                                _p(cs), _p(ws), nws, _p(rows_dev), src, C.byref(ride[0]) if ride is not None else None,
+                                _lib.stream_ptr()), 'kgw_tn_gemm_h1')
+    _route('kgw_tn_gemm_h1')
+    if sink is not None:
+        if ride is not None:
+            sink.reduces_ridden += 1
+        sink.add(out, src[0], ws)
+        sink.add(cs, src[1], ws)
+    return out, cs
+
+
 def _tn_gemm_group(jobs) -> bool:
     if not (2 <= len(jobs) <= 4):
         return False
@@ -1164,6 +1187,9 @@
         return None, dW1, db1, dW2, db2, dW3, db3, None, None
 
 
+_MLP2_RECOMPUTE_MIN_ROWS = 32768
+
+
 class _MLP2(torch.autograd.Function):
 
     @staticmethod
@@ -1177,13 +1203,23 @@
                 and (h2 is None or (h2.stride(1) == 1 and h2.stride(0) % 4 == 0 and h2.data_ptr() % 16 == 0))):
             if h2 is None:
                 h2 = torch.empty(rows, KGW_C, device=x.device)
+            xg = torch.empty(rows, K1, device=x.device) if ids is not None else None
+            L = _lib.lib()
+            ctx.rows_dev = rows_dev
+            ctx.recompute = rows >= _MLP2_RECOMPUTE_MIN_ROWS
+            if ctx.recompute:
+                bits = torch.empty(rows, 4, dtype=torch.int32, device=x.device)
+                _lib.check(L.kgw_mlp2_fwd_bits(_p(x), x.stride(0), K1, _p(W1), W1.stride(0), _p(b1), _p(W2), W2.stride(0), _p(b2),
+                                               None, 0, _p(h2), h2.stride(0), rows, _p(rows_dev), _p(ids), _p(xg),
+                                               K1, _p(bits), _lib.stream_ptr()), 'kgw_mlp2_fwd_bits')
+                _route('kgw_mlp2_fwd_bits')
+                ctx.save_for_backward(x if ids is None else xg, W1, b1, W2, bits)
+                return h2
             h1 = torch.empty(rows, KGW_C, device=x.device)
-            xg = torch.empty(rows, K1, device=x.device) if ids is not None else None
-            _lib.check(_lib.lib().kgw_mlp2_fwd(_p(x), x.stride(0), K1, _p(W1), W1.stride(0), _p(b1), _p(W2), W2.stride(0), _p(b2),
-                                               _p(h1), h1.stride(0), _p(h2), h2.stride(0), rows, _p(rows_dev), _p(ids), _p(xg),
-                                               K1, _lib.stream_ptr()), 'kgw_mlp2_fwd')
+            _lib.check(L.kgw_mlp2_fwd(_p(x), x.stride(0), K1, _p(W1), W1.stride(0), _p(b1), _p(W2), W2.stride(0), _p(b2),
+                                      _p(h1), h1.stride(0), _p(h2), h2.stride(0), rows, _p(rows_dev), _p(ids), _p(xg),
+                                      K1, _lib.stream_ptr()), 'kgw_mlp2_fwd')
             ctx.save_for_backward(x if ids is None else xg, h1, W2)
-            ctx.rows_dev = rows_dev
             return h2
         if ids is not None:
             from .sampler import gather_rows
@@ -1192,13 +1228,33 @@
         h2 = linear(h1, W2, b2, relu=True, out=h2, rows_dev=rows_dev)
         ctx.save_for_backward(x, h1, W2)
         ctx.rows_dev = rows_dev
+        ctx.recompute = False
         return h2
 
     @staticmethod
     def backward(ctx, dh2):
-        x, h1, W2 = ctx.saved_tensors
         rd = ctx.rows_dev
         dh2 = dh2.contiguous()
+        if ctx.recompute:
+            x, W1, b1, W2, bits = ctx.saved_tensors
+            rows, K1 = x.shape
+            assert dh2.data_ptr() % 16 == 0
+            L = _lib.lib()
+            dW1 = torch.empty(KGW_C, K1, device=x.device)
+            db1 = torch.empty(KGW_C, device=x.device)
+            nws = int(L.kgw_mlp2_bwd_first_workspace_floats(rows))
+            ws = torch.empty(nws, device=x.device)
+            sink = GRAD_SINK
+            src = (_lib.KgwGradSrc * 2)() if sink is not None else None
+            _lib.check(L.kgw_mlp2_bwd_first_bits(_p(dh2), dh2.stride(0), _p(W2), W2.stride(0), _p(bits), _p(x), x.stride(0), K1, rows,
+                                                 _p(rd), _p(dW1), K1, _p(db1), _p(ws), nws, src, _lib.stream_ptr()),
+                       'kgw_mlp2_bwd_first_bits')
+            if sink is not None:
+                sink.add(dW1, src[0], ws)
+                sink.add(db1, src[1], ws)
+            dW2, db2 = tn_gemm_h1(dh2, x, W1, b1, rows_dev=rd)
+            return None, dW1, db1, dW2, db2, None, None, None
+        x, h1, W2 = ctx.saved_tensors
         rows, K1 = x.shape
         if (rows >= 16384 and K1 <= 31 and h1.shape[1] == KGW_C and W2.shape == (KGW_C, KGW_C) and x.stride(1) == 1
                 and h1.stride(1) == 1 and dh2.stride(0) % 4 == 0 and h1.stride(0) % 4 == 0 and W2.stride(0) % 4 == 0
```
